# mdolab/dafoam

Hardware: AMD Instinct MI355X
Metric: adjoint_gmres_iterations_per_sec (higher is better)
Workload: dtype f64

## Files before the change

dafoam_amd/_capi.py:

```python
from __future__ import annotations

import ctypes as C
import os

import numpy as np

from .meshgen import BC_MIXED, FoamCase

_HERE = os.path.dirname(os.path.abspath(__file__))
LIB_PATH = os.environ.get("DAFOAM_AMD_LIB") or os.path.join(_HERE, "lib", "libdafoam_amd.so")

SOLVER_IDS = {"DASimpleFoam": 0, "DAScalarTransportFoam": 1, "DARhoSimpleFoam": 2, "DATurboFoam": 3, "DAHeatTransferFoam": 4}
PATCH_TYPES = {"patch": 0, "wall": 1, "symmetry": 2, "cyclic": 3}

c_double_p = C.POINTER(C.c_double)
c_int_p = C.POINTER(C.c_int)
c_ll_p = C.POINTER(C.c_longlong)


class das_case_t(C.Structure):
    _fields_ = [
        ("solver", C.c_int),
        ("n_points", C.c_int),
        ("n_faces", C.c_int),
# ... 231 lines not shown
    "das_set_coloring": (C.c_int, [_VP, c_int_p]),
    "das_debug_factor_block": (C.c_int, [C.c_int, c_ll_p, c_int_p, c_double_p, C.c_int, c_double_p, c_ll_p, c_int_p, c_int_p]),
    "das_debug_rcb": (C.c_int, [C.c_int, c_double_p, C.c_int, C.c_int, c_int_p]),
    "das_get_n_colors": (C.c_int, [_VP, C.c_int]),
    "das_get_con_nnz": (C.c_longlong, [_VP, C.c_int]),
    "das_get_con": (C.c_int, [_VP, C.c_int, c_ll_p, c_int_p]),
    "das_get_colors": (C.c_int, [_VP, C.c_int, c_int_p]),
    "das_calc_drdwt": (C.c_int, [_VP, C.c_int, C.c_int, C.POINTER(_VP)]),
    "das_mat_rows": (C.c_longlong, [_VP]),
    "das_mat_nnz": (C.c_longlong, [_VP]),
    "das_mat_export": (C.c_int, [_VP, c_ll_p, c_int_p, c_double_p]),
    "das_mat_mult": (C.c_int, [_VP, c_double_p, c_double_p]),
    "das_mat_create_from_csr": (C.c_int, [C.c_longlong, c_ll_p, c_int_p, c_double_p, C.POINTER(_VP)]),
    "das_mat_destroy": (None, [_VP]),
    "das_initialize_drdwt_matrix_free": (C.c_int, [_VP]),
    "das_destroy_drdwt_matrix_free": (C.c_int, [_VP]),
    "das_op_nnz": (C.c_longlong, [_VP]),
    "das_op_format_bytes": (C.c_longlong, [_VP]),
    "das_op_export": (C.c_int, [_VP, c_ll_p, c_int_p, c_double_p]),
    "das_calc_drdwold_t_psi": (C.c_int, [_VP, C.c_int, c_double_p, c_double_p]),
    "das_set_old_time_fields": (C.c_int, [_VP, c_double_p, c_double_p]),
    "das_calc_jac_vec_product": (C.c_int, [_VP, c_double_p, c_double_p]),
    "das_set_patch_value": (C.c_int, [_VP, c_int_p, C.c_int, C.c_char_p, c_double_p]),
    "das_get_patch_value": (C.c_int, [_VP, C.c_int, C.c_char_p, c_double_p]),
    "das_set_field": (C.c_int, [_VP, C.c_char_p, c_double_p]),
    "das_get_field": (C.c_int, [_VP, C.c_char_p, c_double_p]),
    "das_calc_dfield_product": (C.c_int, [_VP, C.c_char_p, C.c_char_p, C.c_char_p, c_double_p, c_double_p]),
    "das_calc_dvolcoord_product": (C.c_int, [_VP, C.c_char_p, C.c_char_p, c_double_p, c_double_p, c_double_p]),
    "das_point_influence_build": (C.c_int, [_VP, C.POINTER(C.c_int), C.POINTER(C.c_longlong)]),
    "das_point_influence_get": (C.c_int, [_VP, c_int_p, c_ll_p, c_int_p, c_double_p]),
    "das_debug_device_geometry": (C.c_int, [_VP, c_double_p, c_double_p, c_double_p]),
    "das_debug_strength_aggregates": (C.c_int, [_VP, C.c_int, c_int_p, C.POINTER(C.c_int)]),
    "das_calc_dbc_product": (C.c_int, [_VP, c_int_p, C.c_int, C.c_char_p, c_double_p, C.c_char_p, C.c_char_p, c_double_p, c_double_p]),
    "das_define_force_function": (C.c_int, [_VP, C.c_char_p, c_int_p, C.c_int, c_double_p, C.c_double]),
    "das_define_face_function": (C.c_int, [_VP, C.c_char_p, C.c_char_p, c_int_p, c_int_p, C.c_int, c_double_p, c_double_p, C.c_double, C.c_double]),
    "das_define_face_function_ex": (C.c_int, [_VP, C.c_char_p, C.c_char_p, c_int_p, c_int_p, C.c_int, c_double_p, c_double_p, C.c_double, C.c_double, C.c_int, C.c_double]),
    "das_define_location_function": (C.c_int, [_VP, C.c_char_p, C.c_char_p, c_int_p, C.c_int, c_double_p, c_double_p, C.c_double, C.c_int, C.c_double]),
    "das_define_patch_field_function": (C.c_int, [_VP, C.c_char_p, C.c_char_p, c_int_p, C.c_int, C.c_char_p, c_int_p, C.c_int, c_double_p, C.c_int, C.c_double, C.c_double]),
    "das_define_cell_function": (C.c_int, [_VP, C.c_char_p, C.c_char_p, c_int_p, C.c_int, C.c_char_p, c_int_p, C.c_int, c_double_p, C.c_int, C.c_double, C.c_double]),
    "das_calc_function": (C.c_int, [_VP, C.c_char_p, c_double_p]),
    "das_define_force_coupling": (C.c_int, [_VP, C.c_char_p, c_int_p, C.c_int, C.c_double]),
    "das_calc_force_coupling": (C.c_int, [_VP, C.c_char_p, c_double_p, C.c_int]),
    "das_define_thermal_coupling": (C.c_int, [_VP, C.c_char_p, c_int_p, C.c_int, C.c_int]),
    "das_calc_thermal_coupling": (C.c_int, [_VP, C.c_char_p, c_double_p, C.c_int]),
    "das_define_thermal_coupling_input": (C.c_int, [_VP, C.c_char_p, c_int_p, C.c_int, C.c_int]),
    "das_set_thermal_coupling_input": (C.c_int, [_VP, C.c_char_p, c_double_p, C.c_int]),
    "das_get_patch_mixed": (C.c_int, [_VP, C.c_int, c_double_p, c_double_p]),
    "das_calc_dthermal_coupling_product": (C.c_int, [_VP, C.c_char_p, C.c_char_p, C.c_char_p, c_double_p, c_double_p, C.c_int]),
    "das_define_heat_source": (C.c_int, [_VP, C.c_char_p, C.c_char_p, c_double_p, C.c_double, C.c_int]),
    "das_set_heat_source_pars": (C.c_int, [_VP, C.c_char_p, c_int_p, C.c_int, c_double_p]),
    "das_get_heat_source_info": (C.c_int, [_VP, C.c_char_p, c_double_p, c_double_p, c_double_p, c_int_p]),
    "das_get_heat_source_cells": (C.c_int, [_VP, C.c_char_p, c_int_p, C.c_int]),
    "das_get_fv_source": (C.c_int, [_VP, c_double_p]),
    "das_calc_dfvsourcepar_product": (C.c_int, [_VP, C.c_char_p, c_int_p, C.c_int, C.c_char_p, C.c_char_p, c_double_p, c_double_p]),
    "das_define_actuator_disk": (C.c_int, [_VP, C.c_char_p, C.c_char_p, c_double_p, C.c_char_p, C.c_double, C.c_int]),
    "das_set_actuator_disk_pars": (C.c_int, [_VP, C.c_char_p, c_int_p, C.c_int, c_double_p]),
    "das_get_actuator_disk_info": (C.c_int, [_VP, C.c_char_p, c_double_p, c_double_p, c_int_p]),
    "das_get_actuator_disk_cells": (C.c_int, [_VP, C.c_char_p, c_int_p, C.c_int]),
    "das_get_fv_source_vector": (C.c_int, [_VP, c_double_p]),
    "das_calc_dactuatordiskpar_product": (C.c_int, [_VP, C.c_char_p, c_int_p, C.c_int, C.c_char_p, C.c_char_p, c_double_p, c_double_p]),
    "das_get_input_size": (C.c_int, [_VP, C.c_char_p, C.c_char_p]),
    "das_get_output_size": (C.c_int, [_VP, C.c_char_p, C.c_char_p]),
    "das_calc_jac_t_vec_product": (
        C.c_int,
        [_VP, C.c_char_p, C.c_char_p, c_double_p, C.c_char_p, C.c_char_p, c_double_p, c_double_p],
    ),
    "das_drdwt_mult_device": (C.c_int, [_VP, _VP, _VP]),
    "das_create_ml_rksp_matrix_free": (C.c_int, [_VP, _VP, C.POINTER(_VP)]),
    "das_solve_linear_eqn": (C.c_int, [_VP, _VP, c_double_p, c_double_p]),
    "das_solve_linear_eqn_block": (C.c_int, [_VP, _VP, C.c_int, c_double_p, c_double_p, c_double_p, c_double_p]),
    "das_ksp_apply_pc": (C.c_int, [_VP, _VP, c_double_p, c_double_p]),
    "das_ksp_get_n_blocks": (C.c_int, [_VP]),
    "das_ksp_get_factor_nnz": (C.c_longlong, [_VP]),
    "das_ksp_get_n_ext": (C.c_longlong, [_VP]),
    "das_ksp_get_blocks": (C.c_int, [_VP, c_int_p, c_ll_p]),
    "das_pc_structure_build": (C.c_int, [_VP, c_int_p, c_ll_p, c_int_p, c_int_p]),
    "das_pc_structure_get": (C.c_int, [_VP, c_int_p, c_ll_p, c_int_p, c_int_p, c_int_p]),
    "das_ksp_get_pc_structure_sizes": (C.c_int, [_VP, c_int_p, c_ll_p, c_int_p]),
    "das_ksp_get_pc_structure": (C.c_int, [_VP, c_int_p, c_ll_p, c_int_p, c_int_p, c_int_p]),
    "das_ksp_get_info": (C.c_int, [_VP, c_int_p, c_double_p, c_double_p, c_double_p]),
    "das_ksp_get_history": (C.c_int, [_VP, c_double_p, C.c_int]),
    "das_ksp_get_cycle_lengths": (C.c_int, [_VP, c_int_p, C.c_int]),
    "das_ksp_get_basis_info": (C.c_int, [_VP, c_int_p, c_double_p, c_double_p]),
    "das_ksp_get_n_refine": (C.c_int, [_VP]),
    "das_set_dense_eig_callback": (C.c_int, [_VP]),
    "das_debug_gmres_dr_host": (C.c_int, [C.c_longlong, _VP, _VP, _VP, c_double_p, c_double_p, C.c_int, C.c_int, C.c_double, C.c_double, C.c_longlong, c_double_p, C.c_int,
                                          c_double_p, c_double_p]),
    "das_ksp_get_idr_info": (C.c_int, [_VP, c_int_p, c_int_p, c_int_p, c_int_p, c_int_p, c_double_p]),
    "das_ksp_get_poly_info": (C.c_int, [_VP, c_int_p, c_int_p, C.POINTER(C.c_longlong), C.POINTER(C.c_longlong), C.POINTER(C.c_longlong), c_int_p, c_int_p, c_int_p, c_double_p,
                                        c_int_p, c_double_p, c_double_p]),
    "das_debug_poly_roots": (C.c_int, [C.c_int, c_double_p, c_double_p, c_double_p]),
    "das_debug_poly_apply_host": (C.c_int, [C.c_longlong, _VP, _VP, _VP, C.c_int, c_double_p, c_double_p, c_double_p, c_double_p]),
    "das_debug_poly_step": (C.c_int, [C.c_longlong, C.c_int, C.c_int, C.c_int, C.c_double, C.c_double, C.c_longlong, C.c_longlong, c_double_p, c_double_p, c_double_p,
                                      c_double_p, c_double_p]),
    "das_debug_ksp_poly_apply": (C.c_int, [_VP, _VP, c_double_p, c_double_p]),
    "das_debug_idrs_host": (C.c_int, [C.c_longlong, _VP, _VP, _VP, c_double_p, c_double_p, C.c_int, C.c_int, C.c_double, C.c_double, C.c_longlong, c_double_p, C.c_int,
                                      c_double_p, c_double_p]),
    "das_debug_idr_cycle_host": (C.c_int, [C.c_longlong, _VP, _VP, _VP, c_double_p, c_double_p, C.c_int, C.c_int, c_double_p, c_double_p, c_double_p, c_double_p]),
    "das_debug_idr_shadow": (C.c_int, [C.c_longlong, C.c_int, C.c_longlong, C.c_int, C.c_int, c_double_p]),
    "das_debug_idr_combine": (C.c_int, [C.c_longlong, C.c_int, C.c_double, c_double_p, c_double_p, C.c_longlong, C.c_longlong, c_double_p, C.c_longlong, c_double_p,
                                        C.c_longlong]),
    "das_debug_idr_biortho_step": (C.c_int, [C.c_longlong, C.c_int, c_double_p, c_double_p, C.c_longlong, C.c_longlong, c_double_p, c_double_p, c_double_p, C.c_longlong,
                                             c_double_p]),
    "das_debug_idr_smooth_step": (C.c_int, [C.c_longlong, C.c_int, C.c_double, c_double_p, c_double_p, c_double_p, c_double_p, C.c_longlong, c_double_p, C.c_longlong,
                                            C.c_longlong, c_double_p]),
    "das_debug_gmres_dr_restart": (C.c_int, [C.c_int, C.c_int, c_double_p, c_double_p, c_double_p, c_double_p, c_double_p]),
    "das_debug_block_chol": (C.c_int, [C.c_int, c_double_p, c_double_p, c_double_p]),
    "das_debug_block_lsq": (C.c_int, [C.c_int, C.c_int, C.c_int, c_double_p, c_double_p, c_double_p, c_double_p, c_double_p, c_double_p]),
    "das_ksp_get_status": (C.c_int, [_VP, c_int_p, c_int_p, c_int_p, c_int_p]),
    "das_ksp_get_pc_stability": (C.c_int, [_VP, C.POINTER(C.c_double), c_int_p]),
    "das_ksp_get_pc_subdomains": (C.c_int, [_VP, c_int_p, c_double_p]),
    "das_ksp_get_pc_node_out": (C.c_int, [_VP, c_int_p]),
    "das_mesh_metrics": (C.c_int, [C.c_int, c_double_p, C.c_int, C.c_int, C.c_int, c_int_p, c_int_p, c_int_p, c_int_p, c_double_p, c_double_p, c_double_p, c_double_p, c_double_p]),
    "das_ksp_get_coarse": (C.c_int, [_VP, c_int_p]),
    "das_ksp_coarse_sparse_az_active": (C.c_int, [_VP]),
    "das_ksp_set_global_coarse": (C.c_int, [_VP, _VP, C.c_int, C.c_int, c_int_p]),
    "das_ksp_run_fixed_device": (C.c_int, [_VP, _VP, _VP, _VP, C.c_int]),
    "das_ksp_begin_device": (C.c_int, [_VP, _VP, _VP, _VP, C.c_int]),
    "das_ksp_advance": (C.c_int, [_VP, _VP, C.c_int]),
    "das_ksp_end": (C.c_int, [_VP, _VP]),
    "das_ksp_destroy": (None, [_VP]),
    "das_set_owned_mask": (C.c_int, [_VP, C.POINTER(C.c_ubyte)]),
    "das_comm_load_rccl": (C.c_int, []),
    "das_comm_unique_id": (C.c_int, [C.c_char_p]),
    "das_comm_init_rccl": (C.c_int, [_VP, C.c_int, C.c_int, C.c_char_p]),
    "das_comm_set_halo": (C.c_int, [_VP, C.c_int, c_int_p, c_ll_p, c_int_p, c_ll_p, c_int_p, C.c_longlong, c_int_p]),
    "das_set_exchange_cb": (C.c_int, [_VP, _VP, _VP]),
    "das_set_pc_overlap": (C.c_int, [_VP, C.POINTER(C.c_ubyte), C.c_int, c_ll_p, c_int_p, c_ll_p, c_int_p]),
    "das_set_gather_cb": (C.c_int, [_VP, _VP, _VP]),
    "das_comm_is_native": (C.c_int, [_VP]),
    "das_comm_reset": (C.c_int, [_VP]),
    "das_set_comm": (C.c_int, [_VP, _VP, _VP, _VP]),
    "das_set_stream": (C.c_int, [_VP, _VP]),
    "das_get_elapsed_clock_time": (C.c_double, [_VP]),
    "das_get_elapsed_cpu_time": (C.c_double, [_VP]),
    "das_timer_avg_ms": (C.c_double, [_VP, C.c_char_p]),
    "das_debug_orth_bench": (C.c_int, [C.c_longlong, C.c_int, C.c_int, C.c_int, C.c_int, C.c_int, C.POINTER(C.c_double), C.POINTER(C.c_double)]),
    "das_debug_orth_bench_split": (C.c_int, [C.c_longlong, C.c_int, C.c_int, C.c_int, C.c_int, C.c_int, C.c_int, C.c_int, C.POINTER(C.c_double), C.POINTER(C.c_double)]),
    "das_debug_set_orth_wide": (C.c_int, [C.c_int, C.POINTER(C.c_int)]),
    "das_debug_krylov_wide_eligible": (C.c_int, [C.c_longlong, C.c_int, C.c_longlong, C.POINTER(C.c_int), C.POINTER(C.c_int)]),
    "das_debug_krylov_dots2": (C.c_int, [C.c_longlong, C.c_int, C.c_int, _VP, C.c_longlong, c_double_p, c_double_p]),
    "das_debug_krylov_dcgs2_update": (C.c_int, [C.c_longlong, C.c_int, C.c_int, _VP, C.c_longlong, C.c_int, c_double_p, C.c_double, C.c_double, c_double_p]),
    "das_debug_krylov_multidot": (C.c_int, [C.c_longlong, C.c_int, C.c_int, _VP, C.c_longlong, c_double_p, c_double_p]),
    "das_debug_krylov_multiaxpy": (C.c_int, [C.c_longlong, C.c_int, C.c_int, _VP, C.c_longlong, c_double_p, C.c_int, _VP, C.c_longlong]),
    "das_debug_krylov_lincomb": (C.c_int, [C.c_longlong, C.c_int, C.c_int, _VP, C.c_longlong, c_double_p, c_double_p, C.c_longlong]),
    "das_debug_krylov_scale_to": (C.c_int, [C.c_longlong, C.c_double, C.c_int, _VP, _VP, C.c_longlong]),
    "das_debug_krylov_block_tn": (C.c_int, [C.c_longlong, C.c_int, C.c_int, c_double_p, C.c_longlong, C.c_longlong, c_double_p, C.c_longlong, c_double_p]),
    "das_debug_krylov_block_nn_sub": (C.c_int, [C.c_longlong, C.c_int, C.c_int, c_double_p, C.c_longlong, c_double_p, c_double_p, C.c_longlong]),
    "das_debug_krylov_block_right_mult": (C.c_int, [C.c_longlong, C.c_int, c_double_p, C.c_longlong, c_double_p]),
    "das_debug_krylov_block_lincomb": (C.c_int, [C.c_longlong, C.c_int, C.c_int, c_double_p, C.c_longlong, c_double_p, c_double_p, C.c_longlong]),
    "das_debug_krylov_block_spmm": (C.c_int, [C.c_longlong, C.c_int, c_ll_p, c_int_p, c_double_p, c_double_p, C.c_longlong, c_double_p, C.c_longlong]),
    "das_debug_bilu_factor": (C.c_int, [C.POINTER(das_bilu_debug_t), c_ll_p, c_ll_p, c_int_p, c_int_p, _VP, _VP, c_double_p, c_int_p]),
    "das_debug_bilu_apply": (C.c_int, [C.POINTER(das_bilu_debug_t), C.c_int, C.c_longlong, c_double_p, c_double_p, C.c_int, c_double_p, c_double_p, c_int_p, c_int_p]),
    "das_debug_graph_scan": (C.c_int, [C.c_longlong, c_int_p, c_ll_p, c_ll_p]),
    "das_debug_graph_transpose": (C.c_int, [C.c_longlong, c_ll_p, c_int_p, c_ll_p, c_int_p]),
    "das_debug_graph_nets": (C.c_int, [C.c_longlong, c_ll_p, c_int_p, C.c_longlong, c_ll_p, c_ll_p, c_int_p, c_int_p, C.POINTER(C.c_ubyte), c_ll_p]),
    "das_debug_graph_rows_gather": (C.c_int, [C.c_longlong, c_ll_p, C.c_longlong, c_ll_p, c_int_p, c_ll_p, c_int_p, C.c_longlong]),
    "das_debug_compact": (C.c_int, [C.c_longlong, c_ll_p, c_int_p, c_double_p, C.c_double, C.c_int, C.POINTER(C.c_ubyte), c_ll_p, c_int_p, c_double_p, c_ll_p]),
    "das_debug_vecpack": (C.c_int, [C.c_longlong, c_ll_p, c_int_p, c_double_p, C.c_longlong, C.c_longlong, c_int_p, c_ll_p, C.POINTER(C.c_ubyte), C.c_longlong, c_ll_p,
                                    c_double_p, c_double_p, C.c_longlong]),
    "das_debug_spmv_rows": (C.c_int, [C.c_longlong, c_int_p, C.c_longlong, c_ll_p, c_int_p, c_double_p, c_double_p, c_double_p, C.c_longlong]),
    "das_debug_coarse_assemble": (C.c_int, [C.c_int, C.c_longlong, C.c_longlong, C.c_longlong, c_ll_p, c_int_p, c_double_p, c_int_p, c_int_p, C.c_int, C.c_double,
                                            c_double_p]),
    "das_debug_coarse_invert": (C.c_int, [C.c_int, c_double_p, c_double_p, c_int_p]),
    "das_debug_coarse_correct": (C.c_int, [C.c_int, C.c_longlong, C.c_longlong, C.c_longlong, c_int_p, c_double_p, c_double_p, c_double_p, c_double_p, c_double_p,
                                           C.c_longlong, C.c_int]),
    "das_debug_coarse_az": (C.c_int, [C.c_int, C.c_longlong, c_ll_p, c_int_p, c_double_p, C.c_longlong, C.c_longlong, c_int_p, c_int_p, c_ll_p, c_int_p, c_double_p,
                                      C.c_longlong, c_ll_p, c_int_p, c_double_p, c_double_p, c_double_p, C.c_longlong]),
    "das_timer_count": (C.c_longlong, [_VP, C.c_char_p]),
    "das_timer_reset": (None, [_VP]),
    "das_timer_enable": (None, [_VP, C.c_int]),
}

_lib = None


def declared_symbols():
    return sorted(_SIGS)


def lib():
    global _lib
    if _lib is None:
        if not os.path.exists(LIB_PATH):
            raise ImportError(
                f"{LIB_PATH} not found: build the HIP extension first (python -c 'import __graft_entry__ as g; g.build()'). "
                "dafoam_amd has no CPU fallback."
            )
        L = C.CDLL(LIB_PATH)
        for name, (res, args) in _SIGS.items():
            fn = getattr(L, name)
            fn.restype = res
            fn.argtypes = args
        _lib = L
        _install_dense_eig(L)
    return _lib


_DENSE_EIG_FN = C.CFUNCTYPE(C.c_int, C.c_int, c_double_p, c_double_p, c_double_p, c_double_p, c_double_p)
_dense_eig_keepalive = []


def _install_dense_eig(L):

    def eig(m, A, wr, wi, vr, vi):
        try:
            G = np.ctypeslib.as_array(A, shape=(m * m,)).reshape(m, m)
            w, v = np.linalg.eig(G)
            np.ctypeslib.as_array(wr, shape=(m,))[:] = w.real
            np.ctypeslib.as_array(wi, shape=(m,))[:] = w.imag
            np.ctypeslib.as_array(vr, shape=(m * m,))[:] = np.ascontiguousarray(v.T.real).ravel()
            np.ctypeslib.as_array(vi, shape=(m * m,))[:] = np.ascontiguousarray(v.T.imag).ravel()
            return 0
        except Exception:
            return 1

    cb = _DENSE_EIG_FN(eig)
    _dense_eig_keepalive.append(cb)
    L.das_set_dense_eig_callback(C.cast(cb, C.c_void_p))


class DASError(RuntimeError):
    pass


def check(rc):
    if rc < 0:
        raise DASError(f"dafoam_amd error {rc}: {lib().das_last_error().decode()}")
    return rc


def dptr(a: np.ndarray):
    assert a.dtype == np.float64 and a.flags["C_CONTIGUOUS"]
    return a.ctypes.data_as(c_double_p)
```

dafoam_amd/csrc/das_bilu.hpp:

```cpp
#pragma once
#include <algorithm>
#include <cstdlib>
#include <numeric>

#include <omp.h>

#include "das_common.hpp"
#include "das_jaccon.hpp"

namespace das {

constexpr int BILU_NB = 8;
constexpr int BILU_NB2 = 64;
constexpr unsigned long long BILU_SENTINEL = 0xFFF7A5A5FFF7A5A5ull;
#ifndef BILU_WG
#define BILU_WG 512
#endif
#ifndef BILU_OCC
#define BILU_OCC 4
#endif
#ifndef BILU_XCD_TICKETS
#define BILU_XCD_TICKETS 1
#endif
constexpr int BILU_CTRL_STRIDE = 32;
// ... 283 lines not shown

__global__ __launch_bounds__(256) void k_bilu_scatter(long long n, const long long* __restrict__ rp, const int* __restrict__ ci,
                                                      const double* __restrict__ v, const int* __restrict__ unkNode,
                                                      const unsigned char* __restrict__ unkSlot, const long long* __restrict__ bptr,
                                                      const int* __restrict__ bcol, const unsigned char* __restrict__ late, double* __restrict__ bval,
                                                      unsigned long long* dropped, int transpose, double diagScale, long long shiftExLo,
                                                      long long shiftExHi, long long shiftEnd) {
    const long long row = (long long)blockIdx.x * 16 + (threadIdx.x >> 4);
    const int l16 = threadIdx.x & 15;
    if (row >= n) return;
    const int I0 = unkNode[row];
    if (I0 < 0) return;
    const int r0 = unkSlot[row];
    for (long long k = rp[row] + l16; k < rp[row + 1]; k += 16) {
        const int j = ci[k];
        const int J0 = unkNode[j];
        if (J0 < 0) continue;
        const int I = transpose ? J0 : I0, J = transpose ? I0 : J0;
        const int r = transpose ? unkSlot[j] : r0, c = transpose ? r0 : unkSlot[j];
        long long lo = bptr[I], hi = bptr[I + 1] - 1, e = -1;
        while (lo <= hi) {
            const long long mid = (lo + hi) >> 1;
            const int cm = bcol[mid];
            if (cm == J) { e = mid; break; }
            if (cm < J) lo = mid + 1; else hi = mid - 1;
        }
        if (e < 0) { if (!(late[I] && late[J])) atomicAdd(dropped, 1ull); continue; }
        const bool shifted = row < shiftEnd && !(row >= shiftExLo && row < shiftExHi);
        bval[e * BILU_NB2 + r * 8 + c] = (j == row && shifted) ? v[k] * diagScale : v[k];
    }
}
__global__ void k_bilu_pad_diag(int nNodes, const int* __restrict__ nodeUnk, const long long* __restrict__ bdiag, double* __restrict__ bval) {
    const long long i = (long long)blockIdx.x * blockDim.x + threadIdx.x;
    if (i >= (long long)nNodes * BILU_NB) return;
    if (nodeUnk[i] < 0) { const int k = (int)(i & 7); bval[bdiag[i >> 3] * BILU_NB2 + k * 8 + k] = 1.0; }
}

__device__ __forceinline__ double bilu_inverse8(double a, int lane, int* nshift) {
    const int r = lane >> 3, c = lane & 7;
    double b = (r == c) ? 1.0 : 0.0;
    for (int k = 0; k < 8; k++) {
        int pr = k;
        double best = -1.0;
        for (int rr = k; rr < 8; rr++) {
            const double t = fabs(__shfl(a, rr * 8 + k, 64));
            if (t > best) { best = t; pr = rr; }
        }
        const int src = (r == k) ? pr * 8 + c : (r == pr ? k * 8 + c : lane);
        a = __shfl(a, src, 64);
        b = __shfl(b, src, 64);
        double pv = __shfl(a, k * 8 + k, 64);
        if (!(fabs(pv) > 1e-300)) {
            pv = (pv < 0.0 ? -1.0 : 1.0) * 1e-12;
            if (lane == k * 9) a = pv;
            if (lane == 0) (*nshift)++;
        }
        const double rk = __shfl(a, k * 8 + c, 64) / pv;
        const double rkb = __shfl(b, k * 8 + c, 64) / pv;
        const double f = __shfl(a, r * 8 + k, 64);
        if (r == k) { a = rk; b = rkb; }
        else { a -= f * rk; b -= f * rkb; }
    }
    return b;
}

__global__ __launch_bounds__(256) void k_bilu_factor(int node0, int node1, const long long* __restrict__ bptr, const long long* __restrict__ bdiag,
                                                     const int* __restrict__ bcol, double* bval, double* invD, int* nshift) {
    const int lane = threadIdx.x & 63;
    const int p = node0 + blockIdx.x * 4 + (threadIdx.x >> 6);
    if (p >= node1) return;
    const int r = lane >> 3, c = lane & 7;
    const long long rb = bptr[p], rd = bdiag[p], re = bptr[p + 1];
    for (long long e = rb; e < rd; e++) {
        const int J = bcol[e];
        const double a = bval[e * BILU_NB2 + lane];
        double Lv = 0.0;
#pragma unroll
        for (int k = 0; k < 8; k++) Lv += __shfl(a, r * 8 + k, 64) * invD[(long long)J * BILU_NB2 + k * 8 + c];
        bval[e * BILU_NB2 + lane] = Lv;
        double Lrow[8];
#pragma unroll
        for (int k = 0; k < 8; k++) Lrow[k] = __shfl(Lv, r * 8 + k, 64);
        const long long je = bptr[J + 1];
        long long from = e + 1;
        for (long long f = bdiag[J] + 1; f < je; f++) {
            const int M = bcol[f];
            long long lo = from, hi = re - 1, pos = -1;
            while (lo <= hi) {
                const long long mid = (lo + hi) >> 1;
                const int cm = bcol[mid];
                if (cm == M) { pos = mid; break; }
                if (cm < M) lo = mid + 1; else hi = mid - 1;
            }
            if (pos < 0) { from = lo; continue; }
            from = pos + 1;
            double s = 0.0;
#pragma unroll
            for (int k = 0; k < 8; k++) s += Lrow[k] * bval[f * BILU_NB2 + k * 8 + c];
            bval[pos * BILU_NB2 + lane] -= s;
        }
    }
    int ns = 0;
    const double inv = bilu_inverse8(bval[rd * BILU_NB2 + lane], lane, &ns);
    invD[(long long)p * BILU_NB2 + lane] = inv;
    if (lane == 0 && ns) atomicAdd(nshift, ns);
}

template <class VT>
__global__ __launch_bounds__(256) void k_bilu_pack(int nNodes, const long long* __restrict__ bptr, const long long* __restrict__ bdiag,
                                                   const int* __restrict__ bcol, const double* __restrict__ bval, const long long* __restrict__ Lptr,
                                                   const long long* __restrict__ Uptr, int* __restrict__ Lcol, int* __restrict__ Ucol,
                                                   VT* __restrict__ Lval, VT* __restrict__ Uval) {
    const int lane = threadIdx.x & 63;
    const long long p = (long long)blockIdx.x * 4 + (threadIdx.x >> 6);
    if (p >= nNodes) return;
    const int r = lane >> 3, k = lane & 7;
    for (int t = 0; t < 2; t++) {
        const long long s0 = t == 0 ? bptr[p] : bdiag[p] + 1;
        const long long s1 = t == 0 ? bdiag[p] : bptr[p + 1];
        const int nE = (int)(s1 - s0);
        const long long d0 = t == 0 ? Lptr[p] : Uptr[nNodes - 1 - p];
        int* dcol = t == 0 ? Lcol : Ucol;
        VT* dval = t == 0 ? Lval : Uval;
        for (int a = 0; a < nE; a++) {
            const int pass = a >> 3, g = a & 7;
            const int nb = min(8, nE - 8 * pass);
            dval[(d0 + 8 * pass) * BILU_NB2 + (((r >> 1) * nb + g) * 8 + k) * 2 + (r & 1)] = (VT)bval[(s0 + a) * BILU_NB2 + lane];
            if (lane == 0) dcol[d0 + a] = bcol[s0 + a];
        }
    }
}

struct NodeILU {
    bool ready = false;
    long long n = 0;
    int nNodes = 0, nPrimary = 0, nLevels = 0, nshift = 0, maxRow = 0;
    std::vector<unsigned char> h_late;
    long long nnzB = 0, nL = 0, nU = 0;
    bool fp32 = false;
    double windowLevels = 3.0;
    int launchGrid = 0, launchSleep = 0, launchPerXcd = 0;
    std::vector<int> h_nodeUnk, h_bcol, h_lvlPtr, h_natural;
    std::vector<long long> h_bptr;
    DevBuf<int> nodeUnk, nodeOut, Lcol, Ucol;
    std::vector<int> h_nodeOut;
    DevBuf<long long> Lptr, Uptr;
    DevBuf<double> Lval, Uval, invD, y, z;
    DevBuf<float> Lvalf, Uvalf;
    DevBuf<unsigned> ctrl;
    DevBuf<double> ym, zm;
    int mS = 0;
    BiluView view;
    double t_struct = 0, t_scatter = 0, t_factor = 0, t_pack = 0;
    long long factor_bytes() const { return (nL + nU) * BILU_NB2 * (fp32 ? 4 : 8) + (long long)nNodes * BILU_NB2 * 8; }
};

inline std::vector<int> bilu_rcm_cells(const Mesh& m, const std::vector<char>& cellOwned, const double* startDir = nullptr) {
    const int nC = m.nC;
    std::vector<int> order, deg(nC, 0), queue;
    std::vector<char> seen(nC, 0);
    order.reserve(nC);
    for (int c = 0; c < nC; c++) for (int q = m.cc_ptr[c]; q < m.cc_ptr[c + 1]; q++) deg[c] += cellOwned[m.cc[q]] ? 1 : 0;
    auto bfs = [&](int start, std::vector<int>& out, std::vector<char>& mark) {
        const size_t first = out.size();
        out.push_back(start);
        mark[start] = 1;
        std::vector<int> nb;
        for (size_t head = first; head < out.size(); head++) {
            const int c = out[head];
            nb.clear();
            for (int q = m.cc_ptr[c]; q < m.cc_ptr[c + 1]; q++) { const int d = m.cc[q]; if (cellOwned[d] && !mark[d]) { mark[d] = 1; nb.push_back(d); } }
            std::sort(nb.begin(), nb.end(), [&](int a, int b) { return deg[a] < deg[b] || (deg[a] == deg[b] && a < b); });
            out.insert(out.end(), nb.begin(), nb.end());
        }
    };
    std::vector<char> tmpMark(nC, 0);
    std::vector<int> tmp;
    for (int c0 = 0; c0 < nC; c0++) {
        if (!cellOwned[c0] || seen[c0]) continue;
        int start = c0;
        if (startDir) {
            tmp.clear();
            bfs(c0, tmp, tmpMark);
            double best = 1e300;
            for (int c : tmp) {
                tmpMark[c] = 0;
                const double key = m.cg[c].C[0] * startDir[0] + m.cg[c].C[1] * startDir[1] + m.cg[c].C[2] * startDir[2];
                if (key < best) { best = key; start = c; }
            }
        } else {
            for (int sweep = 0; sweep < 2; sweep++) {
                tmp.clear();
                bfs(start, tmp, tmpMark);
                start = tmp.back();
                for (int c : tmp) tmpMark[c] = 0;
            }
        }
        bfs(start, order, seen);
    }
    std::reverse(order.begin(), order.end());
    return order;
}

inline void bilu_build_structure(const Mesh& m, const std::vector<StateDef>& states, long long n, const std::vector<unsigned char>& owned,
                                 const std::vector<char>& cellOwned, int reach, NodeILU& P, std::vector<int>& unkNode,
                                 std::vector<unsigned char>& unkSlot, std::vector<long long>& bptr, std::vector<long long>& bdiag,
                                 std::vector<int>& bcol, int nthr, int order = 0, const double* dir = nullptr) {
    const int nC = m.nC;
    std::vector<std::vector<int>> ownedFaces;
    bool hasFace = false;
    for (const StateDef& sd : states) if (sd.kind == KIND_FACE) hasFace = true;
    std::vector<int> of_ptr(nC + 1, 0), of;
    if (hasFace) {
        for (int f = 0; f < m.nF; f++) of_ptr[m.owner[f] + 1]++;
        for (int c = 0; c < nC; c++) of_ptr[c + 1] += of_ptr[c];
        of.resize(m.nF);
        std::vector<int> fill(of_ptr.begin(), of_ptr.end() - 1);
        for (int f = 0; f < m.nF; f++) of[fill[m.owner[f]]++] = f;
    }
    std::vector<int> nodeUnk0;
    std::vector<int> nodeCell_ptr{0}, nodeCell;
    std::vector<int> cellNode_ptr(nC + 1, 0), cellNode;
    nodeUnk0.reserve((size_t)nC * 9);
    std::vector<long long> tmp;
    int fillSlots = BILU_NB;
    auto is_owned = [&](long long g) { return owned.empty() || owned[g]; };
    std::vector<int> cellOrder;
    if (order == 1 || order == 2) cellOrder = bilu_rcm_cells(m, cellOwned);
    else { cellOrder.reserve(nC); for (int c = 0; c < nC; c++) if (cellOwned[c]) cellOrder.push_back(c); }
    if (order == 2 || order == 3) std::reverse(cellOrder.begin(), cellOrder.end());
    if (order == 6 || order == 7) {
        const double xdir[3] = {1.0, 0.0, 0.0};
        cellOrder = bilu_rcm_cells(m, cellOwned, dir ? dir : xdir);
        if (order == 6) std::reverse(cellOrder.begin(), cellOrder.end());
    }
    if (order == 4 || order == 5) {
        const double d0 = dir ? dir[0] : 1.0, d1 = dir ? dir[1] : 0.0, d2 = dir ? dir[2] : 0.0, sgn = order == 4 ? 1.0 : -1.0;
        std::vector<double> key(nC);
        for (int c = 0; c < nC; c++) key[c] = sgn * (m.cg[c].C[0] * d0 + m.cg[c].C[1] * d1 + m.cg[c].C[2] * d2);
        std::sort(cellOrder.begin(), cellOrder.end(), [&](int a, int b) { return key[a] < key[b] || (key[a] == key[b] && a < b); });
    }
    std::vector<std::pair<int, int>> cellNodePairs;
    std::vector<int> lateUnk, lateCell;
    for (int c : cellOrder) {
        tmp.clear();
        for (const StateDef& sd : states) {
            if (sd.kind == KIND_VEC) { for (int k = 0; k < 3; k++) if (is_owned(sd.offset + 3LL * c + k)) tmp.push_back(sd.offset + 3LL * c + k); }
            else if (sd.kind == KIND_SCL) { if (is_owned(sd.offset + c)) tmp.push_back(sd.offset + c); }
        }
        for (const StateDef& sd : states)
            if (sd.kind == KIND_FACE) for (int q = of_ptr[c]; q < of_ptr[c + 1]; q++) if (is_owned(sd.offset + of[q])) tmp.push_back(sd.offset + of[q]);
        const size_t mc = tmp.size();
        if (mc == 0) continue;
        const size_t mp = std::min<size_t>(mc, BILU_NB);
        if ((size_t)(BILU_NB - fillSlots) < mp) fillSlots = BILU_NB;
        if (fillSlots == BILU_NB) {
            nodeUnk0.insert(nodeUnk0.end(), BILU_NB, -1);
            nodeCell_ptr.push_back(nodeCell_ptr.back());
            fillSlots = 0;
        }
        const int node = (int)nodeCell_ptr.size() - 2;
        nodeCell.push_back(c);
        nodeCell_ptr[node + 1]++;
        cellNodePairs.push_back({c, node});
        for (size_t k = 0; k < mp; k++) nodeUnk0[(size_t)node * BILU_NB + fillSlots++] = (int)tmp[k];
        for (size_t k = mp; k < mc; k++) { lateUnk.push_back((int)tmp[k]); lateCell.push_back(c); }
    }
    const int nPrimary = (int)nodeCell_ptr.size() - 1;
    for (size_t k = 0; k < lateUnk.size();) {
        const int c = lateCell[k];
        nodeUnk0.insert(nodeUnk0.end(), BILU_NB, -1);
        nodeCell_ptr.push_back(nodeCell_ptr.back());
        const int node = (int)nodeCell_ptr.size() - 2;
        nodeCell.push_back(c);
        nodeCell_ptr[node + 1]++;
        cellNodePairs.push_back({c, node});
        for (int slot = 0; slot < BILU_NB && k < lateUnk.size() && lateCell[k] == c; slot++, k++) nodeUnk0[(size_t)node * BILU_NB + slot] = lateUnk[k];
    }
    const int nN = (int)nodeCell_ptr.size() - 1;
    DAS_CHECK(nN > 0, DAS_ERR_INTERNAL, "preconditioner: no owned unknowns");
    for (const auto& pr : cellNodePairs) cellNode_ptr[pr.first + 1]++;
    for (int c = 0; c < nC; c++) cellNode_ptr[c + 1] += cellNode_ptr[c];
    cellNode.resize(cellNodePairs.size());
    {
        std::vector<int> fill(cellNode_ptr.begin(), cellNode_ptr.end() - 1);
        for (const auto& pr : cellNodePairs) cellNode[fill[pr.first]++] = pr.second;
    }
    std::vector<long long> rptr(nN + 1, 0);
    std::vector<std::vector<int>> rows(nN);
#pragma omp parallel num_threads(nthr)
    {
        std::vector<int> cmark(nC, -1), nmark(nN, -1), cur, nxt;
#pragma omp for schedule(dynamic, 256)
        for (int I = 0; I < nN; I++) {
            std::vector<int>& row = rows[I];
            cur.clear();
            for (int q = nodeCell_ptr[I]; q < nodeCell_ptr[I + 1]; q++) { const int c = nodeCell[q]; cmark[c] = I; cur.push_back(c); }
            const bool lateI = I >= nPrimary;
            auto add_cell = [&](int c) {
                for (int q = cellNode_ptr[c]; q < cellNode_ptr[c + 1]; q++) {
                    const int J = cellNode[q];
                    if (lateI && J >= nPrimary && J != I) continue;
                    if (nmark[J] != I) { nmark[J] = I; row.push_back(J); }
                }
            };
            for (int c : cur) add_cell(c);
            for (int ring = 0; ring < reach; ring++) {
                nxt.clear();
                for (int c : cur)
                    for (int q = m.cc_ptr[c]; q < m.cc_ptr[c + 1]; q++) {
                        const int d = m.cc[q];
                        if (cmark[d] != I) { cmark[d] = I; nxt.push_back(d); if (cellOwned[d]) add_cell(d); }
                    }
                cur.swap(nxt);
            }
            std::sort(row.begin(), row.end());
        }
    }
    std::vector<int> level(nN, 0);
    int nLv = 0;
    for (int I = 0; I < nN; I++) {
        int l = 0;
        for (int J : rows[I]) { if (J >= I) break; l = std::max(l, level[J] + 1); }
        level[I] = l;
        nLv = std::max(nLv, l + 1);
    }
    std::vector<int> lvlPtr(nLv + 1, 0), pos(nN);
    for (int I = 0; I < nN; I++) lvlPtr[level[I] + 1]++;
    for (int l = 0; l < nLv; l++) lvlPtr[l + 1] += lvlPtr[l];
    {
        std::vector<int> fill(lvlPtr.begin(), lvlPtr.end() - 1);
        for (int I = 0; I < nN; I++) pos[I] = fill[level[I]]++;
    }
    std::vector<int> inv(nN);
    for (int I = 0; I < nN; I++) inv[pos[I]] = I;
    bptr.assign(nN + 1, 0);
    for (int p = 0; p < nN; p++) bptr[p + 1] = bptr[p] + (long long)rows[inv[p]].size();
    bcol.resize((size_t)bptr[nN]);
    bdiag.assign(nN, -1);
    int maxRow = 0;
#pragma omp parallel for schedule(static) reduction(max : maxRow) num_threads(nthr)
    for (int p = 0; p < nN; p++) {
        const std::vector<int>& row = rows[inv[p]];
        int* dst = bcol.data() + bptr[p];
        for (size_t k = 0; k < row.size(); k++) dst[k] = pos[row[k]];
        std::sort(dst, dst + row.size());
        bdiag[p] = bptr[p] + (std::lower_bound(dst, dst + row.size(), p) - dst);
        maxRow = std::max(maxRow, (int)row.size());
    }
    P.h_nodeUnk.assign((size_t)nN * BILU_NB, -1);
    unkNode.assign(n, -1);
    unkSlot.assign(n, 0);
    for (int p = 0; p < nN; p++)
        for (int k = 0; k < BILU_NB; k++) {
            const int gidx = nodeUnk0[(size_t)inv[p] * BILU_NB + k];
            P.h_nodeUnk[(size_t)p * BILU_NB + k] = gidx;
            if (gidx >= 0) { unkNode[gidx] = p; unkSlot[gidx] = (unsigned char)k; }
        }
    P.n = n; P.nNodes = nN; P.nLevels = nLv; P.nnzB = bptr[nN]; P.maxRow = maxRow; P.nPrimary = nPrimary;
    P.h_late.assign(nN, 0);
    for (int p = 0; p < nN; p++) P.h_late[p] = inv[p] >= nPrimary ? 1 : 0;
    P.h_bptr = bptr; P.h_bcol = bcol; P.h_lvlPtr = lvlPtr; P.h_natural = inv;
}

struct NodeILU;
inline void bilu_launch_shape(NodeILU& P, hipStream_t st);

struct BiluStructRef {
    const std::vector<long long>* bptr;
    const std::vector<long long>* bdiag;
    const std::vector<int>* bcol;
    std::vector<const std::vector<int>*> unkNode;
    std::vector<const std::vector<unsigned char>*> unkSlot;
};
inline void bilu_numeric(long long n, const BiluStructRef& S, bool fp32, long long An, const long long* d_rp, const int* d_ci, const double* d_av, hipStream_t st, NodeILU& P,
                         bool debug, bool transpose, double diagScale, long long shiftExLo, long long shiftExHi, long long shiftEnd, double t0);

inline std::vector<char> cells_of_mask(const Mesh& m, const std::vector<StateDef>& states, const std::vector<unsigned char>& mask) {
    std::vector<char> in(m.nC, 1);
    if (mask.empty()) return in;
    const StateDef& s0 = states[0];
    const int stride = s0.kind == KIND_VEC ? 3 : 1;
    for (int c = 0; c < m.nC; c++) in[c] = mask[s0.offset + (long long)stride * c] ? 1 : 0;
    return in;
}

inline void bilu_setup(const Mesh& m, const std::vector<StateDef>& states, long long n, const std::vector<unsigned char>& owned, int reach,
                       bool fp32, long long An, const long long* d_rp, const int* d_ci, const double* d_av, hipStream_t st, NodeILU& P,
                       bool debug, int nthr, int order, bool transpose = false, double diagScale = 1.0, long long shiftExLo = 0,
                       long long shiftExHi = 0, long long shiftEnd = (long long)1 << 62, const double* dir = nullptr) {
    const double t0 = wall_seconds();
    const std::vector<char> cellOwned = cells_of_mask(m, states, owned);
    std::vector<int> unkNode, bcol;
    std::vector<unsigned char> unkSlot;
    std::vector<long long> bptr, bdiag;
    bilu_build_structure(m, states, n, owned, cellOwned, reach, P, unkNode, unkSlot, bptr, bdiag, bcol, std::max(1, nthr), order, dir);
    BiluStructRef S{&bptr, &bdiag, &bcol, {&unkNode}, {&unkSlot}};
    bilu_numeric(n, S, fp32, An, d_rp, d_ci, d_av, st, P, debug, transpose, diagScale, shiftExLo, shiftExHi, shiftEnd, t0);
}

inline void bilu_numeric(long long n, const BiluStructRef& S, bool fp32, long long An, const long long* d_rp, const int* d_ci, const double* d_av, hipStream_t st, NodeILU& P,
                         bool debug, bool transpose, double diagScale, long long shiftExLo, long long shiftExHi, long long shiftEnd, double t0) {
    const int nN = P.nNodes;
    P.fp32 = fp32;
    P.nodeUnk.upload(P.h_nodeUnk);
    DevBuf<int> d_unkNode, d_bcol;
    DevBuf<unsigned char> d_unkSlot;
    DevBuf<long long> d_bptr, d_bdiag;
    const std::vector<int>& bcol = *S.bcol;
    const std::vector<long long>&bptr = *S.bptr, &bdiag = *S.bdiag;
    DevBuf<unsigned char> d_late;
    d_late.upload(P.h_late);
    d_bptr.upload(bptr); d_bdiag.upload(bdiag); d_bcol.upload(bcol);
    DevBuf<double> bval((size_t)P.nnzB * BILU_NB2);
    DevBuf<unsigned long long> d_dropped(1);
    DevBuf<int> d_nshift(1);
    DAS_HIP(hipMemsetAsync(bval.p, 0, bval.n * sizeof(double), st));
    DAS_HIP(hipMemsetAsync(d_dropped.p, 0, sizeof(unsigned long long), st));
    DAS_HIP(hipMemsetAsync(d_nshift.p, 0, sizeof(int), st));
    P.t_struct = wall_seconds() - t0;
    double t1 = wall_seconds();
    for (size_t q = 0; q < S.unkNode.size(); q++) {
        d_unkNode.upload(*S.unkNode[q]); d_unkSlot.upload(*S.unkSlot[q]);
        hipLaunchKernelGGL(k_bilu_scatter, dim3((unsigned)((An + 15) / 16)), dim3(256), 0, st, An, d_rp, d_ci, d_av, d_unkNode.p, d_unkSlot.p, d_bptr.p,
                           d_bcol.p, d_late.p, bval.p, d_dropped.p, transpose ? 1 : 0, diagScale, shiftExLo, shiftExHi, shiftEnd);
        DAS_HIP(hipStreamSynchronize(st));
    }
    hipLaunchKernelGGL(k_bilu_pad_diag, dim3((unsigned)(((long long)nN * BILU_NB + 255) / 256)), dim3(256), 0, st, nN, P.nodeUnk.p, d_bdiag.p, bval.p);
    DAS_HIP(hipGetLastError());
    unsigned long long dropped = 0;
    DAS_HIP(hipMemcpyAsync(&dropped, d_dropped.p, sizeof(dropped), hipMemcpyDeviceToHost, st));
    DAS_HIP(hipStreamSynchronize(st));
    DAS_CHECK(dropped == 0, DAS_ERR_INTERNAL, "preconditioner: " + std::to_string(dropped) + " matrix entries fall outside the node pattern (stencil reach too small)");
    P.t_scatter = wall_seconds() - t1;
    t1 = wall_seconds();
    P.invD.alloc((size_t)nN * BILU_NB2);
    for (int l = 0; l < P.nLevels; l++) {
        const int a = P.h_lvlPtr[l], bnd = P.h_lvlPtr[l + 1];
        if (bnd > a)
            hipLaunchKernelGGL(k_bilu_factor, dim3((unsigned)((bnd - a + 3) / 4)), dim3(256), 0, st, a, bnd, d_bptr.p, d_bdiag.p, d_bcol.p, bval.p, P.invD.p,
                               d_nshift.p);
    }
    DAS_HIP(hipGetLastError());
    DAS_HIP(hipMemcpyAsync(&P.nshift, d_nshift.p, sizeof(int), hipMemcpyDeviceToHost, st));
    DAS_HIP(hipStreamSynchronize(st));
    P.t_factor = wall_seconds() - t1;
    t1 = wall_seconds();
    std::vector<long long> Lptr(nN + 1, 0), Uptr(nN + 1, 0);
    for (int p = 0; p < nN; p++) Lptr[p + 1] = Lptr[p] + (bdiag[p] - bptr[p]);
    for (int q = 0; q < nN; q++) { const int p = nN - 1 - q; Uptr[q + 1] = Uptr[q] + (bptr[p + 1] - bdiag[p] - 1); }
    P.nL = Lptr[nN]; P.nU = Uptr[nN];
    P.Lptr.upload(Lptr); P.Uptr.upload(Uptr);
    P.Lcol.alloc(std::max<long long>(P.nL, 1)); P.Ucol.alloc(std::max<long long>(P.nU, 1));
    if (fp32) {
        P.Lvalf.alloc((size_t)std::max<long long>(P.nL, 1) * BILU_NB2); P.Uvalf.alloc((size_t)std::max<long long>(P.nU, 1) * BILU_NB2);
        P.Lval.release(); P.Uval.release();
        hipLaunchKernelGGL(k_bilu_pack<float>, dim3((unsigned)((nN + 3) / 4)), dim3(256), 0, st, nN, d_bptr.p, d_bdiag.p, d_bcol.p, bval.p, P.Lptr.p,
                           P.Uptr.p, P.Lcol.p, P.Ucol.p, P.Lvalf.p, P.Uvalf.p);
    } else {
        P.Lval.alloc((size_t)std::max<long long>(P.nL, 1) * BILU_NB2); P.Uval.alloc((size_t)std::max<long long>(P.nU, 1) * BILU_NB2);
        P.Lvalf.release(); P.Uvalf.release();
        hipLaunchKernelGGL(k_bilu_pack<double>, dim3((unsigned)((nN + 3) / 4)), dim3(256), 0, st, nN, d_bptr.p, d_bdiag.p, d_bcol.p, bval.p, P.Lptr.p,
                           P.Uptr.p, P.Lcol.p, P.Ucol.p, P.Lval.p, P.Uval.p);
    }
    DAS_HIP(hipGetLastError());
    P.y.alloc((size_t)nN * BILU_NB); P.z.alloc((size_t)nN * BILU_NB);
    P.ctrl.alloc(BILU_CTRL_SIZE);
    DAS_HIP(hipMemsetAsync(P.ctrl.p, 0, BILU_CTRL_SIZE * sizeof(unsigned), st));
    DAS_HIP(hipStreamSynchronize(st));
    P.t_pack = wall_seconds() - t1;
    P.view.nNodes = nN; P.view.nodeUnk = P.nodeUnk.p;
    if (!P.h_nodeOut.empty()) P.nodeOut.upload(P.h_nodeOut);
    P.view.nodeOut = P.h_nodeOut.empty() ? P.nodeUnk.p : P.nodeOut.p;
    P.view.ptr[0] = P.Lptr.p; P.view.ptr[1] = P.Uptr.p; P.view.col[0] = P.Lcol.p; P.view.col[1] = P.Ucol.p;
    P.view.val[0] = P.Lval.p; P.view.val[1] = P.Uval.p; P.view.valf[0] = P.Lvalf.p; P.view.valf[1] = P.Uvalf.p;
    P.view.invD = P.invD.p; P.view.y = P.y.p; P.view.z = P.z.p; P.view.ctrl = P.ctrl.p;
    bilu_launch_shape(P, st);
    P.ready = true;
    if (debug)
        fprintf(stderr, "[dafoam_amd] node-block ILU(0): %d nodes (%.3f slots/unknown), %lld blocks (%.1f per node, max %d), %d levels, %d shifted pivots, "
                        "factor %.2f GB%s; structure %.2f s, scatter %.3f s, factorise %.3f s, pack %.3f s\n", nN, (double)nN * BILU_NB / (double)n, P.nnzB,
                (double)P.nnzB / nN, P.maxRow, P.nLevels, P.nshift, P.factor_bytes() / 1e9, fp32 ? " (fp32)" : "", P.t_struct, P.t_scatter, P.t_factor,
                P.t_pack);
}

inline void bilu_setup_multi(const Mesh& m, const std::vector<StateDef>& states, long long n, const std::vector<const std::vector<unsigned char>*>& masks,
                             const std::vector<int>& orders, const std::vector<unsigned char>& subOf, int reach, bool fp32, long long An, const long long* d_rp,
                             const int* d_ci, const double* d_av, hipStream_t st, NodeILU& P, bool debug, int nthr, const double* dir) {
    const double t0 = wall_seconds();
    const int K = (int)masks.size();
    struct Blk { NodeILU S; std::vector<int> unkNode, bcol, newPos; std::vector<unsigned char> unkSlot; std::vector<long long> bptr, bdiag; };
    std::vector<Blk> B(K);
    int nLv = 0;
    long long nN = 0, nnzB = 0;
    for (int b = 0; b < K; b++) {
        const std::vector<unsigned char>& mask = *masks[b];
        const std::vector<char> cellOwned = cells_of_mask(m, states, mask);
        bilu_build_structure(m, states, n, mask, cellOwned, reach, B[b].S, B[b].unkNode, B[b].unkSlot, B[b].bptr, B[b].bdiag, B[b].bcol, std::max(1, nthr), orders[b], dir);
        nLv = std::max(nLv, B[b].S.nLevels);
        nN += B[b].S.nNodes;
        nnzB += B[b].S.nnzB;
    }
    DAS_CHECK(nN < (1LL << 31) && nnzB < (1LL << 40), DAS_ERR_INTERNAL, "multi-block preconditioner too large");
    std::vector<int> lvlPtr(nLv + 1, 0);
    for (int b = 0; b < K; b++) for (int l = 0; l < B[b].S.nLevels; l++) lvlPtr[l + 1] += B[b].S.h_lvlPtr[l + 1] - B[b].S.h_lvlPtr[l];
    for (int l = 0; l < nLv; l++) lvlPtr[l + 1] += lvlPtr[l];
    {
        std::vector<int> cursor(lvlPtr.begin(), lvlPtr.end() - 1);
        for (int b = 0; b < K; b++) {
            B[b].newPos.resize(B[b].S.nNodes);
            for (int l = 0; l < B[b].S.nLevels; l++) for (int p = B[b].S.h_lvlPtr[l]; p < B[b].S.h_lvlPtr[l + 1]; p++) B[b].newPos[p] = cursor[l]++;
        }
    }
    std::vector<long long> bptr(nN + 1, 0), bdiag(nN, -1);
    for (int b = 0; b < K; b++) for (int p = 0; p < B[b].S.nNodes; p++) bptr[B[b].newPos[p] + 1] = B[b].bptr[p + 1] - B[b].bptr[p];
    for (long long p = 0; p < nN; p++) bptr[p + 1] += bptr[p];
    std::vector<int> bcol((size_t)bptr[nN]);
    P = NodeILU();
    P.h_nodeUnk.assign((size_t)nN * BILU_NB, -1);
    P.h_nodeOut.assign((size_t)nN * BILU_NB, -1);
    P.h_late.assign(nN, 0);
    P.h_natural.assign(nN, 0);
    int maxRow = 0, nPrimary = 0;
    long long natOff = 0;
    for (int b = 0; b < K; b++) {
        Blk& Q = B[b];
#pragma omp parallel for schedule(static) num_threads(std::max(1, nthr))
        for (int p = 0; p < Q.S.nNodes; p++) {
            const long long np = Q.newPos[p];
            int* dst = bcol.data() + bptr[np];
            const long long r0 = Q.bptr[p], len = Q.bptr[p + 1] - r0;
            for (long long q = 0; q < len; q++) dst[q] = Q.newPos[Q.bcol[r0 + q]];
            bdiag[np] = bptr[np] + (Q.bdiag[p] - r0);
            for (int k = 0; k < BILU_NB; k++) {
                const int gi = Q.S.h_nodeUnk[(size_t)p * BILU_NB + k];
                P.h_nodeUnk[(size_t)np * BILU_NB + k] = gi;
                P.h_nodeOut[(size_t)np * BILU_NB + k] = (gi >= 0 && subOf[gi] == (unsigned char)b) ? gi : -1;
            }
            P.h_late[np] = Q.S.h_late[p];
            P.h_natural[np] = (int)(natOff + Q.S.h_natural[p]);
        }
        for (long long g = 0; g < n; g++) if (Q.unkNode[g] >= 0) Q.unkNode[g] = Q.newPos[Q.unkNode[g]];
        maxRow = std::max(maxRow, Q.S.maxRow);
        nPrimary += Q.S.nPrimary;
        natOff += Q.S.nNodes;
        Q.S = NodeILU();
        std::vector<int>().swap(Q.bcol);
        std::vector<long long>().swap(Q.bptr);
        std::vector<long long>().swap(Q.bdiag);
    }
    P.n = n; P.nNodes = (int)nN; P.nLevels = nLv; P.nnzB = bptr[nN]; P.maxRow = maxRow; P.nPrimary = nPrimary;
    P.h_bptr = bptr; P.h_bcol = bcol; P.h_lvlPtr = lvlPtr;
    BiluStructRef S{&bptr, &bdiag, &bcol, {}, {}};
    for (int b = 0; b < K; b++) { S.unkNode.push_back(&B[b].unkNode); S.unkSlot.push_back(&B[b].unkSlot); }
    bilu_numeric(n, S, fp32, An, d_rp, d_ci, d_av, st, P, debug, false, 1.0, 0, 0, (long long)1 << 62, t0);
}

__global__ void k_bilu_xcd_probe(unsigned* mask) {
    if (threadIdx.x == 0) atomicOr(mask, 1u << (__builtin_amdgcn_s_getreg((3 << 11) | 20) & 15u));
}
inline int bilu_xcd_probe(hipStream_t st) {
    static int cached = -1;
    if (cached >= 0) return cached;
    DevBuf<unsigned> mask(1);
    DAS_HIP(hipMemsetAsync(mask.p, 0, sizeof(unsigned), st));
    hipLaunchKernelGGL(k_bilu_xcd_probe, dim3(256), dim3(64), 0, st, mask.p);
    unsigned h = 0u;
    DAS_HIP(hipMemcpyAsync(&h, mask.p, sizeof(h), hipMemcpyDeviceToHost, st));
    DAS_HIP(hipStreamSynchronize(st));
    cached = (h == 0xFFu) ? 8 : 0;
    return cached;
}

inline void bilu_launch_shape(NodeILU& P, hipStream_t st) {
    int dev = 0, cus = 256;
    if (hipGetDevice(&dev) == hipSuccess) (void)hipDeviceGetAttribute(&cus, hipDeviceAttributeMultiprocessorCount, dev);
    const int waves = BILU_WG / 64;
    const double perLevel = (double)P.nNodes / std::max(1, P.nLevels);
    int grid = (int)std::min<double>(cus * 2.0 * (BILU_OCC * 4 / waves), std::max(8.0, P.windowLevels * perLevel / waves));
    int sleepReps = 0;
    if (const char* e = getenv("DAS_BILU_WGS")) grid = std::max(1, atoi(e));
    if (const char* e = getenv("DAS_BILU_SLEEP")) sleepReps = std::max(0, atoi(e));
    const long long tickets = ((long long)P.nNodes + waves - 1) / waves;
    grid = (int)std::min<long long>(grid, tickets + 1);
    int perXcd = (BILU_XCD_TICKETS && grid >= 64 && bilu_xcd_probe(st) == 8) ? 1 : 0;
    if (const char* e = getenv("DAS_BILU_XCD")) perXcd = (atoi(e) != 0 && grid >= 64 && bilu_xcd_probe(st) == 8) ? 1 : 0;
    P.launchGrid = grid; P.launchSleep = sleepReps; P.launchPerXcd = perXcd;
}

inline void bilu_apply(NodeILU& P, const double* b, double* out, hipStream_t st) {
    const long long nslots = (long long)P.nNodes * BILU_NB;
    hipLaunchKernelGGL(k_bilu_reset, dim3((unsigned)((nslots + 255) / 256)), dim3(256), 0, st, nslots, P.y.p, P.z.p, P.ctrl.p);
    const int grid = P.launchGrid, sl = P.launchSleep, px = P.launchPerXcd;
    if (P.fp32) {
        hipLaunchKernelGGL((k_bilu_sweep<float, false>), dim3(grid), dim3(BILU_WG), 0, st, P.view, b, out, sl, px);
        hipLaunchKernelGGL((k_bilu_sweep<float, true>), dim3(grid), dim3(BILU_WG), 0, st, P.view, b, out, sl, px);
    } else {
        hipLaunchKernelGGL((k_bilu_sweep<double, false>), dim3(grid), dim3(BILU_WG), 0, st, P.view, b, out, sl, px);
        hipLaunchKernelGGL((k_bilu_sweep<double, true>), dim3(grid), dim3(BILU_WG), 0, st, P.view, b, out, sl, px);
    }
}

template <int S>
inline void bilu_apply_multi_s(NodeILU& P, const double* b, double* out, long long ld, hipStream_t st) {
    const long long nslots = (long long)P.nNodes * BILU_NB * S;
    if (P.mS < S || P.ym.n < (size_t)nslots) { P.ym.alloc((size_t)P.nNodes * BILU_NB * 4); P.zm.alloc((size_t)P.nNodes * BILU_NB * 4); P.mS = 4; }
    hipLaunchKernelGGL(k_bilu_reset, dim3((unsigned)((nslots + 255) / 256)), dim3(256), 0, st, nslots, P.ym.p, P.zm.p, P.ctrl.p);
    const int grid = P.launchGrid, sl = P.launchSleep, px = P.launchPerXcd;
    if (P.fp32) {
        hipLaunchKernelGGL((k_bilu_sweep_m<float, false, S>), dim3(grid), dim3(BILU_WG), 0, st, P.view, P.ym.p, P.zm.p, b, out, ld, sl, px);
        hipLaunchKernelGGL((k_bilu_sweep_m<float, true, S>), dim3(grid), dim3(BILU_WG), 0, st, P.view, P.ym.p, P.zm.p, b, out, ld, sl, px);
    } else {
        hipLaunchKernelGGL((k_bilu_sweep_m<double, false, S>), dim3(grid), dim3(BILU_WG), 0, st, P.view, P.ym.p, P.zm.p, b, out, ld, sl, px);
        hipLaunchKernelGGL((k_bilu_sweep_m<double, true, S>), dim3(grid), dim3(BILU_WG), 0, st, P.view, P.ym.p, P.zm.p, b, out, ld, sl, px);
    }
}
inline void bilu_apply_multi(NodeILU& P, const double* b, double* out, long long ld, int nrhs, hipStream_t st) {
    int r = 0;
    for (; r + 4 <= nrhs; r += 4) bilu_apply_multi_s<4>(P, b + (long long)r * ld, out + (long long)r * ld, ld, st);
    for (; r + 2 <= nrhs; r += 2) bilu_apply_multi_s<2>(P, b + (long long)r * ld, out + (long long)r * ld, ld, st);
    for (; r < nrhs; r++) bilu_apply(P, b + (long long)r * ld, out + (long long)r * ld, st);
}

inline bool bilu_aborted(NodeILU& P, hipStream_t st) {
    unsigned c = 0u;
    DAS_HIP(hipMemcpyAsync(&c, P.ctrl.p + BILU_CTRL_ABORT, sizeof(c), hipMemcpyDeviceToHost, st));
    DAS_HIP(hipStreamSynchronize(st));
    return c != 0u;
}

inline void bilu_clear_abort(NodeILU& P, hipStream_t st) { DAS_HIP(hipMemsetAsync(P.ctrl.p + BILU_CTRL_ABORT, 0, sizeof(unsigned), st)); }

}
```

dafoam_amd/csrc/das_bilu_debug.hpp:

```cpp
#pragma once
#include "das_bilu.hpp"

namespace das {

static void bilu_debug_validate(const std::string& who, const das_bilu_debug_t& d) {
    const int nN = d.nNodes;
    auto bad = [&](bool cond, const char* what) { DAS_CHECK(!cond, DAS_ERR_ARG, who + ": " + what); };
    bad(d.bptr[0] != 0, "bptr[0] must be 0");
    for (int p = 0; p < nN; p++) bad(d.bptr[p + 1] < d.bptr[p], "bptr decreases");
    bad(d.bptr[nN] >= (1LL << 40), "too many blocks");
    bad(d.lvlPtr[0] != 0 || d.lvlPtr[d.nLevels] != nN, "lvlPtr must cover [0, nNodes]");
    for (int l = 0; l < d.nLevels; l++) bad(d.lvlPtr[l + 1] < d.lvlPtr[l], "lvlPtr decreases");
    std::vector<int> level(nN);
    for (int l = 0; l < d.nLevels; l++) for (int p = d.lvlPtr[l]; p < d.lvlPtr[l + 1]; p++) level[p] = l;
    for (int p = 0; p < nN; p++) {
        const long long rb = d.bptr[p], re = d.bptr[p + 1], rd = d.bdiag[p];
        bad(rd < rb || rd >= re, "bdiag outside its row");
        for (long long e = rb; e < re; e++) {
            const int J = d.bcol[e];
            bad(J < 0 || J >= nN, "block column out of range");
            bad(e > rb && d.bcol[e - 1] >= J, "block columns of a row must ascend");
        }
        bad(d.bcol[rd] != p, "bdiag does not point at the diagonal block");
    }
    for (int p = 0; p < nN; p++)
        for (long long e = d.bptr[p]; e < d.bptr[p + 1]; e++) {
            const int J = d.bcol[e];
            if (J == p) continue;
            const int* jb = d.bcol + d.bptr[J];
            const int* je = d.bcol + d.bptr[J + 1];
            bad(!std::binary_search(jb, je, p), "the node pattern is not symmetric");
            bad(J < p && level[J] >= level[p], "a dependency does not lie in an earlier level");
        }
    for (long long i = 0; i < (long long)nN * BILU_NB; i++) {
        bad(d.nodeUnk[i] < -1 || d.nodeUnk[i] >= d.n, "nodeUnk out of range");
        if (d.nodeOut) bad(d.nodeOut[i] < -1 || d.nodeOut[i] >= d.n, "nodeOut out of range");
    }
    for (long long i = 0; i < (long long)d.nMaps * d.An; i++) {
        bad(d.unkNode[i] < -1 || d.unkNode[i] >= nN, "unkNode out of range");
        bad(d.unkSlot[i] >= BILU_NB, "unkSlot must be below 8");
    }
    bad(d.rp[0] != 0, "rowptr[0] must be 0");
    for (long long i = 0; i < d.An; i++) bad(d.rp[i + 1] < d.rp[i], "rowptr decreases");
    const long long nnz = d.rp[d.An];
    bad(nnz > 0 && !(d.ci && d.val), "null pointer");
    for (long long k = 0; k < nnz; k++) bad(d.ci[k] < 0 || d.ci[k] >= d.An, "CSR column out of range");
}

static void bilu_debug_check(const std::string& who, const das_bilu_debug_t* d) {
    DAS_CHECK(d, DAS_ERR_ARG, who + ": null pointer");
    DAS_CHECK(d->nNodes > 0 && d->nLevels > 0 && d->nMaps > 0 && d->n > 0 && d->An > 0, DAS_ERR_ARG, who + ": sizes must be positive");
    DAS_CHECK(d->nNodes < (1 << 27) && d->An <= d->n && d->n < (1LL << 31), DAS_ERR_ARG, who + ": sizes out of range (An <= n < 2^31)");
    DAS_CHECK(d->nodeUnk && d->late && d->bptr && d->bdiag && d->bcol && d->lvlPtr && d->unkNode && d->unkSlot && d->rp, DAS_ERR_ARG, who + ": null pointer");
    DAS_CHECK((d->fp32 == 0 || d->fp32 == 1) && (d->transpose == 0 || d->transpose == 1), DAS_ERR_ARG, who + ": fp32 and transpose are 0 or 1");
    bilu_debug_validate(who, *d);
}

static void bilu_debug_setup(const das_bilu_debug_t& d, NodeILU& P) {
    const int nN = d.nNodes;
    const std::vector<long long> bptr(d.bptr, d.bptr + nN + 1), bdiag(d.bdiag, d.bdiag + nN);
    const std::vector<int> bcol(d.bcol, d.bcol + bptr[nN]);
    std::vector<std::vector<int>> unkNode(d.nMaps);
    std::vector<std::vector<unsigned char>> unkSlot(d.nMaps);
    BiluStructRef S{&bptr, &bdiag, &bcol, {}, {}};
    for (int q = 0; q < d.nMaps; q++) {
        unkNode[q].assign(d.unkNode + q * d.An, d.unkNode + (q + 1) * d.An);
        unkSlot[q].assign(d.unkSlot + q * d.An, d.unkSlot + (q + 1) * d.An);
    }
    for (int q = 0; q < d.nMaps; q++) { S.unkNode.push_back(&unkNode[q]); S.unkSlot.push_back(&unkSlot[q]); }
    P.n = d.n; P.nNodes = nN; P.nLevels = d.nLevels; P.nnzB = bptr[nN]; P.nPrimary = nN;
    for (int p = 0; p < nN; p++) P.maxRow = std::max(P.maxRow, (int)(bptr[p + 1] - bptr[p]));
    P.h_nodeUnk.assign(d.nodeUnk, d.nodeUnk + (size_t)nN * BILU_NB);
    if (d.nodeOut) P.h_nodeOut.assign(d.nodeOut, d.nodeOut + (size_t)nN * BILU_NB);
    P.h_late.assign(d.late, d.late + nN);
    P.h_lvlPtr.assign(d.lvlPtr, d.lvlPtr + d.nLevels + 1);
    P.h_bptr = bptr; P.h_bcol = bcol;
    const size_t nnz = (size_t)d.rp[d.An];
    DevBuf<long long> d_rp(d.An + 1);
    DevBuf<int> d_ci(std::max<size_t>(nnz, 1));
    DevBuf<double> d_av(std::max<size_t>(nnz, 1));
    d_rp.upload(d.rp, (size_t)d.An + 1); d_ci.upload(d.ci, nnz); d_av.upload(d.val, nnz);
    bilu_numeric(d.n, S, d.fp32 != 0, d.An, d_rp.p, d_ci.p, d_av.p, 0, P, false, d.transpose != 0, d.diagScale, d.shiftExLo, d.shiftExHi, d.shiftEnd, wall_seconds());
}

static void debug_bilu_factor(const das_bilu_debug_t& d, long long* Lptr, long long* Uptr, int* Lcol, int* Ucol, void* Lval, void* Uval, double* invD, int* nshift) {
    NodeILU P;
    bilu_debug_setup(d, P);
    const size_t nN = (size_t)d.nNodes;
    P.Lptr.download(Lptr, nN + 1); P.Uptr.download(Uptr, nN + 1);
    P.Lcol.download(Lcol, (size_t)P.nL); P.Ucol.download(Ucol, (size_t)P.nU);
    if (d.fp32) { P.Lvalf.download((float*)Lval, (size_t)P.nL * BILU_NB2); P.Uvalf.download((float*)Uval, (size_t)P.nU * BILU_NB2); }
    else { P.Lval.download((double*)Lval, (size_t)P.nL * BILU_NB2); P.Uval.download((double*)Uval, (size_t)P.nU * BILU_NB2); }
    P.invD.download(invD, nN * BILU_NB2);
    *nshift = P.nshift;
}

static int bilu_debug_last_group(int nrhs) { return (nrhs & 1) ? 1 : ((nrhs & 3) == 2 ? 2 : 4); }

static void debug_bilu_apply(const das_bilu_debug_t& d, int nrhs, long long ld, const double* b, double* out, int twice, double* y, double* z, int* abortFlag,
                             int* info) {
    NodeILU P;
    bilu_debug_setup(d, P);
    const size_t len = (size_t)nrhs * ld;
    DevBuf<double> db(len), dout(len);
    db.upload(b, len);
    for (int rep = 0; rep < (twice ? 2 : 1); rep++) {
        dout.upload(out, len);
        if (nrhs == 1) bilu_apply(P, db.p, dout.p, 0);
        else bilu_apply_multi(P, db.p, dout.p, ld, nrhs, 0);
        DAS_HIP(hipGetLastError());
        DAS_HIP(hipStreamSynchronize(0));
    }
    dout.download(out, len);
    const int S = bilu_debug_last_group(nrhs);
    const size_t nw = (size_t)d.nNodes * BILU_NB * S;
    (S == 1 ? P.y : P.ym).download(y, nw);
    (S == 1 ? P.z : P.zm).download(z, nw);
    *abortFlag = bilu_aborted(P, 0) ? 1 : 0;
    info[0] = P.launchGrid; info[1] = P.launchSleep; info[2] = P.launchPerXcd; info[3] = bilu_xcd_probe(0);
}

}
```

dafoam_amd/csrc/das_device.hip:

```cpp
#include <algorithm>
#include <cmath>
#include <ctime>
#include <functional>
#include <numeric>
#include <thread>

#include "das_case.hpp"
#include "das_jaccon.hpp"
#include "das_bilu.hpp"
#include "das_rcb.hpp"
#include "das_comm.hpp"
#include "das_krylov.hpp"
#include "das_gmres_host.hpp"
#include "das_block.hpp"
#include "das_krylov_debug.hpp"
#include "das_idr.hpp"
#include "das_idr_debug.hpp"
#include "das_poly.hpp"
#include "das_poly_debug.hpp"
#include "das_bilu_debug.hpp"
#include "das_graph_debug.hpp"
#include "das_coarse.hpp"
#include "das_coarse_debug.hpp"
#include "das_color.hpp"
// ... 467 lines not shown
            sok[d] = ee < lvl[lq + 1];
            const int ec = ee < eend ? ee : eend - 1;
            sv[d].load(bv, ec);
            sr[d] = br[ec];
#ifndef PC_EXP_NOBARRIER
            __syncthreads();
#endif
        }
    }
}

template <bool USE_LDS>
__global__ __launch_bounds__(PC_THREADS) void k_ras_apply(PCView P, const double* __restrict__ b, double* __restrict__ out, int maxLev) {
    extern __shared__ double xs[];
    const int blk = blockIdx.x;
    const long long o0 = P.boff[blk];
    const int nloc = (int)(P.boff[blk + 1] - o0);
    int* lvl = (int*)xs;
    double* xlds = xs + ((maxLev + 2 * PC_PF + 4) >> 1);
    double* xw = USE_LDS ? xlds : P.xglob + o0;
    for (int i = threadIdx.x; i < nloc; i += PC_THREADS) xw[i] = b[P.gidx[o0 + i]];
    __syncthreads();
    if (P.factor32) ras_sweep<USE_LDS, float>(P.svalf[0], P.srowcol[0], P.slev[0], P.slevOff[0][blk], P.slevOff[0][blk + 1], xw, lvl);
    else ras_sweep<USE_LDS, double>(P.sval[0], P.srowcol[0], P.slev[0], P.slevOff[0][blk], P.slevOff[0][blk + 1], xw, lvl);
    for (int i = threadIdx.x; i < nloc; i += PC_THREADS) xw[i] *= P.invd[o0 + i];
    __syncthreads();
    if (P.factor32) ras_sweep<USE_LDS, float>(P.svalf[1], P.srowcol[1], P.slev[1], P.slevOff[1][blk], P.slevOff[1][blk + 1], xw, lvl);
    else ras_sweep<USE_LDS, double>(P.sval[1], P.srowcol[1], P.slev[1], P.slevOff[1][blk], P.slevOff[1][blk + 1], xw, lvl);
    for (int i = threadIdx.x; i < nloc; i += PC_THREADS) {
        int g = P.gout[o0 + i];
        if (g >= 0) out[g] = xw[i];
    }
}

struct Mat {
    long long n = 0, nnz = 0;
    DevBuf<long long> rowptr;
    DevBuf<int> col;
    DevBuf<double> val;
    VecPack vp;
};

struct KernelTimer {
    struct Rec { double ms = 0; long long cnt = 0; std::vector<std::pair<hipEvent_t, hipEvent_t>> pending; };
    std::map<std::string, Rec> recs;
    bool on = false;
    std::vector<hipEvent_t> pool;
    hipEvent_t get() {
        if (!pool.empty()) { hipEvent_t e = pool.back(); pool.pop_back(); return e; }
        hipEvent_t e;
        DAS_HIP(hipEventCreate(&e));
        return e;
    }
    void begin(const char* name, hipStream_t st, hipEvent_t& a) {
        if (!on) return;
        a = get();
        DAS_HIP(hipEventRecord(a, st));
    }
    void end(const char* name, hipStream_t st, hipEvent_t a) {
        if (!on) return;
        hipEvent_t b = get();
        DAS_HIP(hipEventRecord(b, st));
        recs[name].pending.push_back({a, b});
    }
    void resolve() {
        for (auto& kv : recs) {
            for (auto& pr : kv.second.pending) {
                DAS_HIP(hipEventSynchronize(pr.second));
                float ms = 0;
                DAS_HIP(hipEventElapsedTime(&ms, pr.first, pr.second));
                kv.second.ms += ms;
                kv.second.cnt++;
                pool.push_back(pr.first);
                pool.push_back(pr.second);
            }
            kv.second.pending.clear();
        }
    }
    void reset() { resolve(); for (auto& kv : recs) { kv.second.ms = 0; kv.second.cnt = 0; } }
};

struct ConDev {
    bool ready = false;
    bool onDevice = false;
    DevBuf<long long> t_rowptr;
    DevBuf<int> cl_cols;
    DevBuf<int> t_col;
};

struct BlockILU {
    long long n = 0, next = 0;
    int nBlocks = 0;
    long long fnnz = 0;
    int maxLocal = 0;
    DevBuf<long long> boff, slev[2], slevOff[2];
    DevBuf<int> gidx, gout;
    DevBuf<unsigned> srowcol[2];
    DevBuf<double> sval[2], invd, xw;
    DevBuf<float> svalf[2];
    bool factor32 = false;
    PCView view;
    int maxLevels = 0;
    bool useLDS = false;
    double setup_seconds = 0;
    std::vector<int> h_core_perm;
    std::vector<long long> h_core_off;
};

}

using namespace das;

struct das_mat {
    Mat m;
};

struct das_ksp {
    das_mat* pcmat = nullptr;
    BlockILU pc;
    NodeILU bilu;
    bool useBilu = false;
    bool pcTranspose = false;
    double pcDiagScale = 1.0;
    long long shiftExLo = 0, shiftExHi = 0, shiftEnd = (long long)1 << 62;
    struct CoarsePC {
        bool active = false, deflated = false;
        bool global = false;
        int nagg = 0;
        int naggG = 0, aggOff = 0;
        long long off = 0, N = 0;
        DevBuf<int> agg;
        DevBuf<int> aggRow;
        DevBuf<int> cells, cellsAll;
        DevBuf<long long> aptr, aptrAll;
        DevBuf<double> Einv, t, u, c, rr;
        std::vector<int> h_agg;
        DevBuf<long long> azPtr;
        DevBuf<int> azAgg;
        DevBuf<double> azVal;
        long long azOpId = -1;
        long long azEpoch = -1, azNnz = 0;
        bool azReady = false, azFailed = false;
    } coarse;
    int restart = 0;
    VmBuf<double> V;
    long long Vn = 0;
    bool vf32 = false;
    bool split = false;
    DevBuf<double> ustage;
    DevBuf<double> w, z, r, xdev, bdev, partial, hdev, rich_r, rich_d;
    int nSub = 1;
    std::vector<int> subOrder;
    std::vector<double> subEst;
    int pcOrder = -1;
    int pcOrderUsed = -1;
    double pcStability = -1.0;
    bool rasOverlap = false;
    DevBuf<double> pcin;
    std::unique_ptr<struct GmresRun> run;
    std::unique_ptr<struct BlockWork> block;
    int polyD = 0;
    std::unique_ptr<struct PolyWork> poly;
    std::unique_ptr<struct IdrWork> idr;
    std::vector<double> block_res0, block_res;
    int iters = 0, nrefine = 0, reason = 0, nBreakdown = 0;
    double res0 = 0, res = 0, seconds = 0;
    std::vector<double> hist;
    std::vector<int> cycleLens;
};

struct das_solver {
    Mesh mesh;
    CaseParams cp;
    Options opt;
    int device = -1;
    bool inited = false;
    long long n = 0;
    Stencil st_full, st_pc;
    JacCon con_full, con_pc;
    std::vector<int> colors;
    int nColors = 0;
    bool colored = false;
    DevBuf<FaceGeom> d_fg;
    DevBuf<CellGeom> d_cg;
    DevBuf<int> d_cf_ptr, d_cf_face, d_cf_other, d_owner, d_neigh, d_bpatch, d_cyc;
    DevBuf<PatchBC> d_bc;
    DevBuf<double> d_mixed;
    DevBuf<double> d_phiF, d_Told;
    DevMesh dm;
    DevBuf<double> d_W, d_R, d_R0, d_Wp, d_scale, d_tmp1, d_tmp2;
    DevBuf<int> d_colors;
    std::vector<double> h_W, h_scale;
    ResWork<double> wk;
    ResWork<Dual<1>> wk1;
    DevBuf<Dual<1>> d_Wd, d_Rd;
    ConDev cd[2];
    std::unique_ptr<das_mat> op;
    std::vector<double> op_states;
    long long op_geom = -1;
    struct FaceFn {
        int kind = DAS_FN_FORCE;
        bool ratio = false;
        double gammaFn = 1.4, RFn = 287.0;
        std::vector<int> faces;
        std::vector<unsigned char> group;
        std::vector<double> w0, dir;
        DevBuf<int> d_faces;
        DevBuf<unsigned char> d_group;
        DevBuf<double> d_w0, d_weff, d_dir, d_fv;
        bool uploaded = false;
        bool isMoment = false;
        double vecA[3] = {0, 0, 0}, vecB[3] = {0, 0, 0}, scale = 1.0;
        long long geomVersion = -1;
        bool refVar = false, geoWeight = false, hasData = true;
        double ref = 0.0;
        int ncomp = 1;
        bool byUnitArea = true, ks = false;
        double coeffKS = 1.0, loc[6] = {1, 0, 0, 0, 0, 0};
        DevBuf<double> d_ks, d_kpart;
        double pRef = 0.0;
        FaceFnView view(const double* w) const {
            return FaceFnView{d_faces.p, d_group.p, w, dir.empty() ? nullptr : d_dir.p, (int)faces.size(), kind, gammaFn, RFn,
                              {loc[0], loc[1], loc[2], loc[3], loc[4], loc[5]}, pRef};
        }
    };
    std::map<std::string, FaceFn> functions;
    struct ForceCoupling {
        std::vector<int> patches;
        int nOut = 0;
        std::vector<int> ptPtr, ptSlot;
        std::vector<int> fcPtr, fcPt;
        DevBuf<int> d_ptPtr, d_ptSlot, d_fcPtr, d_fcPt;
        DevBuf<double> d_ff, d_out, d_seeds;
        FaceFn fn;
        bool uploaded = false;
    };
    std::map<std::string, ForceCoupling> forceCouplings;
    struct ThermalCoupling {
        std::vector<int> patches;
        DevBuf<double> d_out, d_seeds;
        FaceFn fn;
        bool uploaded = false;
        std::vector<double> in;
    };
    std::map<std::string, ThermalCoupling> thermalCouplings, thermalInputs;
    struct CellFn {
        bool variance = false, square = false, multiplyVol = true, divByTotalVol = false, refVar = false, geoWeight = false, hasData = true;
        bool field = false;
        double scale = 1.0, ref = 0.0;
        double coef = 0.0, totalVol = 1.0;
        long long geomVersion = -1;
        std::vector<int> cell;
        std::vector<long long> idx;
        std::vector<double> data;
        DevBuf<int> d_cell;
        DevBuf<long long> d_idx;
        DevBuf<double> d_data, d_part, d_unit;
        bool uploaded = false;
        CellFnView view() const {
            return CellFnView{(long long)cell.size(), d_cell.p, d_idx.p, data.empty() ? nullptr : d_data.p, (int)square, (int)multiplyVol};
        }
    };
    std::map<std::string, CellFn> cellFunctions;
    struct HeatSource {
        int kind = DAS_HS_CYLINDERSMOOTH;
        double pars[9] = {0, 0, 0, 0, 0, 0, 0, 0, 0};
        double eps = 0.0;
        int snapCell = -1;
        std::vector<int> members;
        DevBuf<unsigned char> d_member;
        double volumeTotal = 0.0;
    };
    std::map<std::string, HeatSource> heatSources;
    DevBuf<double> d_src, d_hsVt;
    DevBuf<Dual<1>> d_hsPart, d_hsVtD;
    double hsSourceTotal = 0.0;
    struct ActuatorDisk {
        int smooth = 1, adjustThrust = 0;
        double pars[13] = {0, 0, 0, 0, 0, 0, 0, 0, 0, 0, 0, 0, 0};
        double eps = 0.0, rotSign = 1.0;
        std::vector<int> members;
        DevBuf<unsigned char> d_member;
        double scale = 0.0, thrustSum = 0.0, torqueSum = 0.0, unitThrust = 0.0;
    };
    std::map<std::string, ActuatorDisk> actuatorDisks;
    DevBuf<double> d_src3, d_adSums;
    DevBuf<Dual<1>> d_adPart, d_adD;
    DevBuf<int> d_adBad;
    int colorRounds = 0;
    DevBuf<double> d_betaFI, d_dBetaFI;
    long long geomVersion = 0;
    struct VolCoord {
        PointInfluence inf;
        bool built = false, uploaded = false;
        double relStep = 0.0;
        long long hGeom = -1;
        DevBuf<long long> d_ptr;
        DevBuf<int> d_cells, d_cpoints, d_face_ptr, d_face_pts, d_bad, d_fnPtr, d_fnIdx;
        DevBuf<double> d_h, d_X0, d_X, d_Rp, d_Rm, d_seeds, d_tc, d_out, d_fvp, d_fvm;
        DevBuf<FaceGeom> d_fg0;
        DevBuf<CellGeom> d_cg0;
        double buildSeconds = 0.0, seconds = 0.0;
    } vc;
    long long opEpoch = 0, op_epoch = -1;
    long long nGlobalCells = 0;
    hipStream_t stream = nullptr;
// ... 422 lines not shown
                lrp.assign(nl + 1, 0);
                lci.clear();
                lv.clear();
                for (int p = 0; p < nl; p++) {
                    int g = F.gidx[p];
                    row.clear();
                    for (long long q = rp[g]; q < rp[g + 1]; q++) {
                        int lc = loc[ci[q]];
                        if (lc >= 0) row.push_back({lc, av[q]});
                    }
                    std::sort(row.begin(), row.end());
                    for (auto& e : row) { lci.push_back(e.first); lv.push_back(e.second); }
                    lrp[p + 1] = (long long)lci.size();
                }
                for (int p = 0; p < nl; p++) loc[F.gidx[p]] = -1;
                factor_local(nl, lrp, lci, lv, lfill, F, where, lev, nullptr);
                F.nnzLU = (long long)F.fci.size();
                std::vector<long long>().swap(F.frp); std::vector<long long>().swap(F.fdiag); std::vector<int>().swap(F.fci);
                std::vector<double>().swap(F.fv); std::vector<int>().swap(F.Lrows); std::vector<int>().swap(F.Urows);
            } catch (const std::exception& e) {
#pragma omp critical
                err = e.what();
            }
        }
    }
    DAS_CHECK(err.empty(), DAS_ERR_INTERNAL, "block ILU setup failed: " + err);
    const double t_fact = wall_seconds();
    BlockILU& P = k->pc;
    std::vector<long long> boff(nB + 1, 0), eoff[2], loff[2], slev[2], slevOff[2];
    long long next = 0, fnnz = 0;
    int maxLocal = 0, maxLv = 0, nshift = 0;
    for (int t = 0; t < 2; t++) { eoff[t].assign(nB + 1, 0); loff[t].assign(nB + 1, 0); }
    P.h_core_off.assign(1, 0);
    for (int b = 0; b < nB; b++) {
        const BlockFactor& F = BF[b];
        const int nl = (int)F.gidx.size();
        boff[b + 1] = boff[b] + nl;
        maxLocal = std::max(maxLocal, nl);
        nshift += F.nshift;
        fnnz += F.nnzLU;
        long long ncore = 0;
        for (int g : F.gout) ncore += g >= 0 ? 1 : 0;
        P.h_core_off.push_back(P.h_core_off.back() + ncore);
        for (int t = 0; t < 2; t++) {
            eoff[t][b + 1] = eoff[t][b] + (long long)F.sval[t].size();
            loff[t][b + 1] = loff[t][b] + (long long)F.slev[t].size();
            maxLv = std::max<int>(maxLv, (int)F.slev[t].size() - 1);
        }
    }
    next = boff[nB];
    std::vector<int> gidx(next), gout(next);
    std::vector<double> invd(next);
    P.h_core_perm.assign(P.h_core_off.back(), 0);
    for (int t = 0; t < 2; t++) { slev[t].resize(loff[t][nB]); slevOff[t] = loff[t]; }
#pragma omp parallel for schedule(dynamic, 1) num_threads(das::host_threads())
    for (int b = 0; b < nB; b++) {
        BlockFactor& F = BF[b];
        std::copy(F.gidx.begin(), F.gidx.end(), gidx.begin() + boff[b]);
        std::copy(F.gout.begin(), F.gout.end(), gout.begin() + boff[b]);
        std::copy(F.invd.begin(), F.invd.end(), invd.begin() + boff[b]);
        long long pc = P.h_core_off[b];
        for (int g : F.gout) if (g >= 0) P.h_core_perm[pc++] = g;
        for (int t = 0; t < 2; t++)
            for (size_t q = 0; q < F.slev[t].size(); q++) slev[t][loff[t][b] + q] = eoff[t][b] + F.slev[t][q];
    }
    DAS_CHECK((long long)P.h_core_perm.size() == nOwnedStates, DAS_ERR_INTERNAL, "block cores do not cover all owned states exactly once");
    P.n = n; P.next = next; P.nBlocks = nB; P.fnnz = fnnz; P.maxLevels = maxLv; P.maxLocal = maxLocal;
    P.boff.upload(boff); P.gidx.upload(gidx); P.gout.upload(gout); P.invd.upload(invd);
    P.factor32 = s->opt.geti("amd.pcFactorFP32") != 0;
    for (int t = 0; t < 2; t++) {
        const size_t tot = (size_t)eoff[t][nB];
        if (P.factor32) { P.svalf[t].alloc(tot); P.sval[t].release(); }
        else { P.sval[t].alloc(tot); P.svalf[t].release(); }
        P.srowcol[t].alloc(tot);
        P.slev[t].upload(slev[t]); P.slevOff[t].upload(slevOff[t]);
    }
    {
        std::vector<float> f32;
        for (int b = 0; b < nB; b++) {
            BlockFactor& F = BF[b];
            for (int t = 0; t < 2; t++) {
                const size_t cnt = F.sval[t].size();
                if (!cnt) continue;
                if (P.factor32) {
                    f32.assign(F.sval[t].begin(), F.sval[t].end());
                    DAS_HIP(hipMemcpy(P.svalf[t].p + eoff[t][b], f32.data(), cnt * sizeof(float), hipMemcpyHostToDevice));
                } else {
                    DAS_HIP(hipMemcpy(P.sval[t].p + eoff[t][b], F.sval[t].data(), cnt * sizeof(double), hipMemcpyHostToDevice));
                }
                DAS_HIP(hipMemcpy(P.srowcol[t].p + eoff[t][b], F.src[t].data(), cnt * sizeof(unsigned), hipMemcpyHostToDevice));
            }
            F = BlockFactor();
        }
    }
    P.useLDS = (size_t)maxLocal * sizeof(double) + (size_t)(maxLv + 2 * PC_PF + 8) * sizeof(int) + 16 <= 160 * 1024;
    if (!P.useLDS) P.xw.alloc(next);
    else DAS_HIP(hipFuncSetAttribute((const void*)k_ras_apply<true>, hipFuncAttributeMaxDynamicSharedMemorySize, 160 * 1024));
    P.view.nBlocks = nB; P.view.boff = P.boff.p; P.view.gidx = P.gidx.p; P.view.gout = P.gout.p; P.view.invd = P.invd.p;
    P.view.factor32 = P.factor32 ? 1 : 0;
    for (int t = 0; t < 2; t++) { P.view.sval[t] = P.sval[t].p; P.view.svalf[t] = P.svalf[t].p; P.view.srowcol[t] = P.srowcol[t].p; P.view.slev[t] = P.slev[t].p; P.view.slevOff[t] = P.slevOff[t].p; }
    P.view.xglob = P.xw.p;
    P.setup_seconds = wall_seconds() - t0;
    if (s->opt.geti("debug"))
        fprintf(stderr, "[dafoam_amd] RAS(overlap %d)+ILU(%d): %d blocks, n_ext=%lld (%.2fx), nnz(LU)=%lld, max block %d unknowns (%s), max levels %d, "
                        "%d shifted pivots, %.2f s (download+partition %.2f, factorise %.2f, streams+upload %.2f)\n", overlap, lfill, nB, next,
                (double)next / n, fnnz, maxLocal, P.useLDS ? "LDS" : "global", maxLv, nshift, P.setup_seconds, t_prep - t0, t_fact - t_prep,
                wall_seconds() - t_fact);
}

static int pc_stencil_reach(das_solver* s) {
    ensure_coloring(s);
    int reach = 0;
    for (size_t b = 0; b < s->st_pc.states.size(); b++)
        for (size_t lv = 0; lv < s->st_pc.levels[b].size(); lv++) {
            const unsigned mask = s->st_pc.levels[b][lv];
            if (!mask) continue;
            bool faceState = false;
            for (size_t q = 0; q < s->st_pc.states.size(); q++) if ((mask >> q & 1u) && s->st_pc.states[q].kind == KIND_FACE) faceState = true;
            reach = std::max<int>(reach, (int)lv + (faceState ? 1 : 0) + (s->st_pc.states[b].kind == KIND_FACE ? 1 : 0));
        }
    return reach;
}

static bool pc_ordering_rcm(das_solver* s) {
    const std::string& o = s->opt.gets("adjEqnOption.jacMatReOrdering");
    DAS_CHECK(o == "natural" || o == "rcm", DAS_ERR_ARG, "adjEqnOption.jacMatReOrdering \"" + o + "\" is not implemented (natural | rcm)");
    return o == "rcm";
}

static void pc_flow_direction(das_solver* s, double* dir) {
    dir[0] = 1.0; dir[1] = 0.0; dir[2] = 0.0;
    if (!s->st_full.states.empty() && s->st_full.states[0].kind == KIND_VEC && s->h_W.size() == (size_t)s->n) {
        const StateDef& u = s->st_full.states[0];
        double m[3] = {0, 0, 0};
        for (long long c = 0; c < u.size / 3; c++) for (int q = 0; q < 3; q++) m[q] += s->h_W[u.offset + 3 * c + q];
        const double nm = std::sqrt(m[0] * m[0] + m[1] * m[1] + m[2] * m[2]);
        if (nm > 0.0) for (int q = 0; q < 3; q++) dir[q] = m[q] / nm;
    }
}

static const std::vector<unsigned char>& pc_mask(das_solver* s, das_ksp* k) { return (s->pcMask.empty() || k->pcTranspose) ? s->owned : s->pcMask; }
static int pc_configured_order(das_solver* s, das_ksp* k) { return k->pcOrder >= 0 ? k->pcOrder : (pc_ordering_rcm(s) ? 1 : 0); }
static bool pc_order_is_deep(int levels, int nodes) { return (double)levels > 30.0 * std::cbrt((double)std::max(1, nodes)); }
static const char* rank_label() { return getenv("RANK") ? getenv("RANK") : "0"; }

struct BiluInputs {
    const Mat& A;
    int reach, nthr;
    bool fp32, debug;
    double dir[3];
    BiluInputs(das_solver* s, das_ksp* k)
        : A(k->pcmat->m), reach(pc_stencil_reach(s)), nthr(pc_setup_threads(s)), fp32(s->opt.geti("amd.pcFactorFP32") != 0), debug(s->opt.geti("debug") != 0) { pc_flow_direction(s, dir); }
};
static void factorise_node_ilu(das_solver* s, das_ksp* k, NodeILU& P, const std::vector<unsigned char>& mask, int order) {
    const BiluInputs in(s, k);
    bilu_setup(s->mesh, s->st_full.states, s->n, mask, in.reach, in.fp32, in.A.n, in.A.rowptr.p, in.A.col.p, in.A.val.p, s->stream,
               P, in.debug, in.nthr, order, k->pcTranspose, k->pcDiagScale, k->shiftExLo, k->shiftExHi, k->shiftEnd, in.dir);
}
static void pc_finish_bilu(das_solver* s, das_ksp* k, double t0, int nBlocks, bool rasOverlap) {
    k->useBilu = true;
    k->rasOverlap = rasOverlap;
    if (k->rasOverlap && k->pcin.n != (size_t)s->n) k->pcin.alloc(s->n);
    k->pc.setup_seconds = wall_seconds() - t0;
    k->pc.nBlocks = nBlocks;
    k->pc.fnnz = (k->bilu.nL + k->bilu.nU + k->bilu.nNodes) * (long long)BILU_NB2;
    k->pc.next = (long long)k->bilu.nNodes * BILU_NB;
}

static double pc_stability_estimate(das_solver* s, das_ksp* k, NodeILU& F, const std::vector<unsigned char>& mask) {
    const long long n = s->n;
    const Mat& P = k->pcmat->m;
    std::vector<double> e(n), z(n);
    DevBuf<double> de(n), dw(n), dz(n);
    double est = 0.0;
    long long worst = -1;
    for (int trial = 0; trial < 2; trial++) {
        for (long long i = 0; i < n; i++) {
            const bool in = mask.empty() || mask[i];
            unsigned long long hsh = (unsigned long long)i * 0x9E3779B97F4A7C15ull;
            hsh ^= hsh >> 29;
            e[i] = !in ? 0.0 : (trial == 0 ? 1.0 : ((hsh & 1ull) ? 1.0 : -1.0));
        }
        de.upload(e);
        hipLaunchKernelGGL(k_spmv_wave, SPMV_GRID(P.n), dim3(256), 0, s->stream, P.n, P.rowptr.p, P.col.p, P.val.p, (const double*)de.p, dw.p);
        dz.zero();
        bilu_apply(F, dw.p, dz.p, s->stream);
        DAS_HIP(hipStreamSynchronize(s->stream));
        z = dz.to_host();
        const int* nu = F.h_nodeUnk.data();
        for (size_t q = 0; q < F.h_nodeUnk.size(); q++) {
            const int gi = nu[q];
            if (gi < 0) continue;
            const double d = std::fabs(z[gi] - e[gi]);
            if (d > est || d != d) worst = gi;
            est = (d > est || d != d) ? (d != d ? 1e300 : d) : est;
        }
    }
    if (worst >= 0 && getenv("DAS_PC_STAB")) {
        for (const StateDef& sd : s->st_full.states) {
            if (worst < sd.offset || worst >= sd.offset + sd.size) continue;
            const long long ent = (worst - sd.offset) / (sd.kind == KIND_VEC ? 3 : 1);
            const double* C = sd.kind == KIND_FACE ? s->mesh.fg[ent].Cf : s->mesh.cg[ent].C;
            fprintf(stderr, "[dafoam_amd] rank %s: worst entry of the stability test: state %s entity %lld at (%.4g %.4g %.4g)%s\n", rank_label(),
                    sd.name.c_str(), ent, C[0], C[1], C[2], (!s->owned.empty() && !s->owned[worst]) ? " (overlap ring)" : "");
        }
    }
    return est;
}

static void choose_order_and_factorise(das_solver* s, das_ksp* k, NodeILU& F, const std::vector<unsigned char>& mask, bool pickMin, int& orderUsed, double& estimate,
                                       bool earlyAccept = true) {
    const int configured = pc_configured_order(s, k);
    const double limit = s->opt.getd("amd.pcStabilityLimit");
    if (!(limit > 0.0)) {
        F = NodeILU();
        factorise_node_ilu(s, k, F, mask, configured);
        orderUsed = -1; estimate = -1.0;
        return;
    }
    std::vector<int> cand{configured};
    {
        std::string lst = s->opt.gets("amd.pcOrderCandidates");
        if (getenv("DAS_BILU_ORDER_LIST")) { lst = getenv("DAS_BILU_ORDER_LIST"); cand.clear(); }
        for (size_t q = 0; q < lst.size(); q++)
            if (lst[q] >= '0' && lst[q] <= '7') { const int o = lst[q] - '0'; if (std::find(cand.begin(), cand.end(), o) == cand.end()) cand.push_back(o); }
        if (cand.empty()) cand.push_back(configured);
    }
    if (getenv("DAS_BILU_PICK_MIN")) pickMin = atoi(getenv("DAS_BILU_PICK_MIN")) != 0;
    const double good = s->opt.getd("amd.pcStabilityGood");
    struct Cand { int o; double est; int levels; };
    std::vector<Cand> seen;
    int last = -1;
    for (size_t attempt = 0; attempt < cand.size(); attempt++) {
        const int o = cand[attempt];
        F = NodeILU();
        factorise_node_ilu(s, k, F, mask, o);
        const double est = pc_stability_estimate(s, k, F, mask);
        last = o;
        seen.push_back({o, est, F.nLevels});
        if (s->opt.geti("debug") || getenv("DAS_PC_STAB") || (est > limit && !pickMin))
            fprintf(stderr, "[dafoam_amd] rank %s: preconditioner stability estimate max|(LU)^-1 P e - e| = %.3e with elimination order %d, %d levels (limit %.1e)%s\n",
                    rank_label(), est, o, F.nLevels, limit, (est > limit && !pickMin) ? ": unstable, trying another order" : "");
        const bool deep = pc_order_is_deep(F.nLevels, F.nNodes);
        if (est <= limit && (!pickMin || (earlyAccept && est <= good && !deep))) break;
    }
    bool anyOk = false;
    for (const Cand& c : seen) anyOk = anyOk || c.est <= limit;
    int minLv = 1 << 30;
    for (const Cand& c : seen) if (!anyOk || c.est <= limit) minLv = std::min(minLv, c.levels);
    int best = seen.back().o;
    double bestEst = 1e300;
    if (!pickMin && seen.back().est <= limit) bestEst = seen.back().est;
    else
        for (const Cand& c : seen)
            if ((!anyOk || c.est <= limit) && (double)c.levels <= 1.5 * minLv && c.est < bestEst) { best = c.o; bestEst = c.est; }
    if (last != best) {
        F = NodeILU();
        factorise_node_ilu(s, k, F, mask, best);
    }
    if (bestEst > limit)
        fprintf(stderr, "[dafoam_amd] rank %s: no elimination order passes the stability limit; keeping order %d (estimate %.3e)\n", rank_label(), best, bestEst);
    orderUsed = best; estimate = bestEst;
}

static void setup_node_ilu(das_solver* s, das_ksp* k, bool byEstimate) {
    const double t0 = wall_seconds();
    if (byEstimate) {
        choose_order_and_factorise(s, k, k->bilu, pc_mask(s, k), !s->owned.empty(), k->pcOrderUsed, k->pcStability,  s->owned.empty());
        if (k->pcOrderUsed >= 0) k->pcOrder = k->pcOrderUsed;
    } else {
        factorise_node_ilu(s, k, k->bilu, pc_mask(s, k), pc_configured_order(s, k));
    }
    pc_finish_bilu(s, k, t0, 1, !s->pcMask.empty() && !k->pcTranspose && s->halo.ovActive);
}

static long long pc_subdomain_count(das_solver* s) {
    long long K = s->opt.geti("amd.pcSubdomains");
    if (!s->owned.empty()) return 1;
    if (K < 0) K = s->mesh.nC >= 1000000 ? 4 : 1;
    return std::max<long long>(1, std::min<long long>(K, 16));
}

template <class Fn>
static void for_each_unknown_with_cell(das_solver* s, Fn fn) {
    const Mesh& m = s->mesh;
    for (const StateDef& sd : s->st_full.states) {
        if (sd.kind == KIND_VEC) { for (int c = 0; c < m.nC; c++) for (int q = 0; q < 3; q++) fn(sd.offset + 3LL * c + q, c); }
        else if (sd.kind == KIND_SCL) { for (int c = 0; c < m.nC; c++) fn(sd.offset + c, c); }
        else { for (long long f = 0; f < m.nF; f++) fn(sd.offset + f, m.owner[f]); }
    }
}

static bool setup_subdomain_ilus(das_solver* s, das_ksp* k, int K) {
    const double t0 = wall_seconds();
    const Mesh& m = s->mesh;
    const long long N = m.nC, n = s->n;
    std::vector<int> cells(N), blockOf(N, 0);
    std::iota(cells.begin(), cells.end(), 0);
    rcb_parts(cells, [&](int c, int d) { return m.cg[c].C[d]; }, K, blockOf);
    std::vector<unsigned char> subOf(n, 0);
    for_each_unknown_with_cell(s, [&](long long g, int c) { subOf[g] = (unsigned char)blockOf[c]; });
    const int overlap = (int)std::max<long long>(0, s->opt.geti("adjEqnOption.asmOverlap"));
    std::vector<std::vector<unsigned char>> masks(K);
    k->subOrder.assign(K, -1);
    k->subEst.assign(K, -1.0);
    for (int b = 0; b < K; b++) {
        std::vector<unsigned char> cellIn(N, 0), grown;
        for (long long c = 0; c < N; c++) cellIn[c] = blockOf[c] == b;
        for (int ring = 0; ring < overlap; ring++) {
            grown = cellIn;
            for (long long c = 0; c < N; c++) if (cellIn[c]) for (int q = m.cc_ptr[c]; q < m.cc_ptr[c + 1]; q++) grown[m.cc[q]] = 1;
            cellIn.swap(grown);
        }
        masks[b].assign(n, 0);
        for_each_unknown_with_cell(s, [&](long long g, int c) { masks[b][g] = cellIn[c]; });
        NodeILU F;
        choose_order_and_factorise(s, k, F, masks[b], true, k->subOrder[b], k->subEst[b]);
        if (k->subOrder[b] < 0) k->subOrder[b] = pc_configured_order(s, k);
        if (s->opt.geti("debug") || getenv("DAS_PC_STAB"))
            fprintf(stderr, "[dafoam_amd] sub-domain %d of %d: %d nodes, %d levels, elimination order %d, stability estimate %.3e\n", b, K, F.nNodes, F.nLevels, k->subOrder[b], k->subEst[b]);
        if (pc_order_is_deep(F.nLevels, F.nNodes) && s->opt.geti("amd.pcSubdomains") < 0) {
            fprintf(stderr, "[dafoam_amd] sub-domain %d of %d needs %d dependency levels for %d nodes: the blocks do not suit this mesh, one factorisation instead "
                            "(amd.pcSubdomains K > 1 forces the blocks)\n", b, K, F.nLevels, F.nNodes);
            k->subOrder.clear(); k->subEst.clear();
            return false;
        }
    }
    {
        const BiluInputs in(s, k);
        std::vector<const std::vector<unsigned char>*> mp;
        for (int b = 0; b < K; b++) mp.push_back(&masks[b]);
        k->bilu = NodeILU();
        bilu_setup_multi(s->mesh, s->st_full.states, n, mp, k->subOrder, subOf, in.reach, in.fp32, in.A.n, in.A.rowptr.p, in.A.col.p, in.A.val.p, s->stream, k->bilu,
                         in.debug, in.nthr, in.dir);
    }
    k->nSub = K;
    k->pcOrderUsed = k->subOrder[0];
    k->pcStability = 0.0;
    for (double e : k->subEst) k->pcStability = std::max(k->pcStability, e);
    pc_finish_bilu(s, k, t0, K, false);
    if (s->opt.geti("debug") || getenv("DAS_PC_STAB"))
        fprintf(stderr, "[dafoam_amd] %d sub-domains merged: %d nodes, %d levels (%.0f nodes per level)\n", K, k->bilu.nNodes, k->bilu.nLevels, (double)k->bilu.nNodes / std::max(1, k->bilu.nLevels));
    return true;
}

static void coarse_build_operator(das_solver* s, das_ksp* k, int naggG, int aggOff, const std::vector<int>& aggRowG) {
    das_ksp::CoarsePC& C = k->coarse;
    C.active = false;
    DAS_CHECK(naggG >= C.nagg && naggG <= 2048, DAS_ERR_ARG, "coarse space: at most 2048 aggregates in total (dense inverse)");
    const long long N = C.N;
    std::vector<int> aggOwn(N, -1);
    for (long long c = 0; c < N; c++) if (C.h_agg[c] >= 0) aggOwn[c] = aggOff + C.h_agg[c];
    std::vector<long long> aptrAll;
    std::vector<int> cellsAll;
    coarse_sort_cells(N, naggG, aggRowG.data(), aptrAll, cellsAll);
    C.naggG = naggG; C.aggOff = aggOff; C.global = naggG > C.nagg;
    C.azOpId = -1; C.azReady = false;
    C.agg.upload(aggOwn); C.aggRow.upload(aggRowG); C.cellsAll.upload(cellsAll); C.aptrAll.upload(aptrAll);
    DevBuf<double> E((size_t)naggG * naggG);
    const Mat& P = k->pcmat->m;
    coarse_assemble(naggG, C.aptrAll.p, C.cellsAll.p, N, C.off, P.rowptr.p, P.col.p, P.val.p, k->pcTranspose ? C.aggRow.p : C.agg.p, E.p, k->pcTranspose ? 1 : 0,
                    (C.off < k->shiftEnd && !(C.off >= k->shiftExLo && C.off < k->shiftExHi)) ? k->pcDiagScale : 1.0, s->stream);
    if (C.global) {
        DAS_CHECK(!k->pcTranspose, DAS_ERR_ARG, "global coarse space: adjoint preconditioner only");
        rank_allreduce(s, E.p, naggG * naggG, s->stream);
    }
    {
        if (C.Einv.n < (size_t)naggG * naggG) C.Einv.alloc((size_t)naggG * naggG);
        DevBuf<int> sing(1);
        if (coarse_invert(naggG, E.p, C.Einv.p, sing.p, s->stream)) return;
    }
    C.t.alloc(naggG); C.u.alloc(naggG);
    C.active = true;
}

static void setup_coarse(das_solver* s, das_ksp* k) {
    das_ksp::CoarsePC& C = k->coarse;
    C.active = false;
    long long want = s->opt.geti("amd.pcCoarseAggregates");
    if (want == 0) return;
    const std::string field = s->opt.gets("amd.pcCoarseField");
    const StateDef* sd = nullptr;
    for (const StateDef& q : s->st_full.states) if (q.name == field && q.kind == KIND_SCL) sd = &q;
    if (!sd) return;
    const Mesh& m = s->mesh;
    const long long N = m.nC;
    std::vector<int> owned;
    owned.reserve(N);
    for (long long c = 0; c < N; c++) if (s->owned.empty() || s->owned[sd->offset + c]) owned.push_back((int)c);
    if (owned.size() < 64) return;
    if (want < 0) want = std::min<long long>(1024, std::max<long long>(16, (long long)owned.size() / 2048));
    int nagg = (int)std::min<long long>(want, std::min<long long>(2048, (long long)owned.size() / 4));
    if (nagg < 2) return;
    std::vector<int> agg(N, -1);
    const bool byStrength = s->opt.gets("amd.pcCoarseAggregation") == "strength";
    DAS_CHECK(byStrength || s->opt.gets("amd.pcCoarseAggregation") == "rcb", DAS_ERR_ARG, "amd.pcCoarseAggregation: rcb | strength");
    if (byStrength) {
        std::vector<unsigned char> mask;
        if (!s->owned.empty()) { mask.resize(N); for (long long c = 0; c < N; c++) mask[c] = s->owned[sd->offset + c]; }
        nagg = strength_aggregates(m, s->owned.empty() ? nullptr : &mask, nagg, agg);
        if (nagg < 2) return;
    } else {
        rcb_parts(owned, [&](int c, int d) { return m.cg[c].C[d]; }, nagg, agg);
    }
    std::vector<long long> aptr;
    std::vector<int> cells;
    coarse_sort_cells(N, nagg, agg.data(), aptr, cells);
    C.nagg = nagg; C.off = sd->offset; C.N = N; C.h_agg = agg;
    C.cells.upload(cells); C.aptr.upload(aptr);
    C.deflated = s->opt.gets("amd.pcCoarseMode") == "deflated";
    if (C.deflated) { C.c.alloc(s->n); C.rr.alloc(s->n); }
    coarse_build_operator(s, k, nagg, 0, agg);
    if (C.active && s->opt.geti("debug")) fprintf(stderr, "[dafoam_amd] coarse space: %d aggregates on field %s (%s)\n", nagg, field.c_str(), C.deflated ? "deflated" : "additive");
}
static void coarse_solve(das_solver* s, das_ksp* k, const double* r) {
    das_ksp::CoarsePC& C = k->coarse;
    if (C.global) DAS_HIP(hipMemsetAsync(C.t.p, 0, (size_t)C.naggG * sizeof(double), s->stream));
    coarse_restrict_solve(C.nagg, C.aptr.p, C.cells.p, C.off, r, C.naggG, C.aggOff, C.Einv.p, C.t.p, C.u.p, s->stream,
                          [&] { if (C.global) rank_allreduce(s, C.t.p, C.naggG, s->stream); });
}

static void pc_apply(das_solver* s, das_ksp* k, const double* b, double* x) {
    hipEvent_t ev = nullptr;
    s->timer.begin("pc", s->stream, ev);
    if (k->useBilu) {
        if (k->rasOverlap) {
            DAS_HIP(hipMemcpyAsync(k->pcin.p, b, (size_t)s->n * sizeof(double), hipMemcpyDeviceToDevice, s->stream));
            s->halo.gather_overlap(k->pcin.p, s->stream);
            bilu_apply(k->bilu, k->pcin.p, x, s->stream);
            s->halo.zero_overlap(x, s->stream);
        } else {
            bilu_apply(k->bilu, b, x, s->stream);
        }
        s->timer.end("pc", s->stream, ev);
        return;
    }
    const int mlv = k->pc.maxLevels;
    const size_t lvlBytes = (size_t)((mlv + 2 * PC_PF + 4) >> 1) * sizeof(double);
    if (k->pc.useLDS)
        hipLaunchKernelGGL(k_ras_apply<true>, dim3(k->pc.nBlocks), dim3(PC_THREADS), lvlBytes + (size_t)k->pc.maxLocal * sizeof(double), s->stream,
                           k->pc.view, b, x, mlv);
    else
        hipLaunchKernelGGL(k_ras_apply<false>, dim3(k->pc.nBlocks), dim3(PC_THREADS), lvlBytes, s->stream, k->pc.view, b, x, mlv);
    s->timer.end("pc", s->stream, ev);
}

static void gmres_ws(das_solver* s, das_ksp* k, int polyD = 0) {
    const long long n = s->n;
    long long restart = std::min<long long>(s->opt.geti("adjEqnOption.gmresRestart"), s->opt.geti("adjEqnOption.gmresMaxIters"));
    k->polyD = polyD;
    if (polyD > 0) restart = std::min<long long>(s->opt.geti("adjEqnOption.gmresRestart"), (std::max<long long>(s->opt.geti("adjEqnOption.gmresMaxIters"), 1) + polyD - 1) / polyD + polyD);
    const long long budget = s->opt.geti_or("amd.maxKrylovBytes", (long long)(32.0 * 1024 * 1024 * 1024));
    const long long nr = (n + 3) / 4 * 4;
    const long long maxVec = std::max<long long>(3, budget / (8 * nr));
    restart = std::max<long long>(1, std::min<long long>(restart, maxVec - 2));
    long long wantVec = std::max<long long>(restart + 2, std::min<long long>(maxVec, 1002));
    if ((size_t)wantVec * (size_t)nr * sizeof(double) < ((size_t)4 << 30) || getenv("DAS_NO_VMM") || polyD > 0) wantVec = restart + 2;
    if (k->V.n < (size_t)((restart + 2) * nr) || k->Vn != n) {
        k->V.reserve((size_t)(wantVec * nr));
        k->Vn = n;
    }
    {
        const std::string prec = s->opt.gets_or("amd.krylovBasisPrecision", "auto");
        DAS_CHECK(prec == "auto" || prec == "fp64" || prec == "fp32" || prec == "split", DAS_ERR_ARG, "amd.krylovBasisPrecision: auto | fp64 | split | fp32");
        const bool eligible = s->opt.geti("adjEqnOption.useMGSO") == 0 && !s->fwd.on;
        const bool dcgs2 = s->opt.gets("amd.gmresOrthogonalization") == "dcgs2" && s->opt.geti("adjEqnOption.useMGSO") == 0;
        bool big = (size_t)(restart + 2) * (size_t)n * 8 >= ((size_t)1 << 30);
        big = rank_any(s, big);
        k->split = eligible && (prec == "split" || (prec == "auto" && dcgs2 && big));
        k->vf32 = k->split || (eligible && prec == "fp32");
        if (k->vf32 && k->ustage.n != (size_t)n) k->ustage.alloc(n);
    }
    if (k->restart != restart || k->w.n != (size_t)n) {
        k->restart = (int)restart;
        k->w.alloc(n); k->z.alloc(n); k->r.alloc(n); k->xdev.alloc(n); k->bdev.alloc(n);
        k->z.zero();
        k->partial.alloc(std::max<size_t>(multidot_partial_size(n, (int)restart + 1), multidot2_partial_size(n, (int)restart + 2)));
        k->hdev.alloc(4 * (restart + 3));
    }
}
static inline long long basis_n4(das_solver* s) { return (s->n + 3) / 4 * 4; }
static inline long long basis_ld(das_solver* s, das_ksp* k) { return k->split ? 2 * basis_n4(s) : (k->vf32 ? basis_n4(s) : s->n); }
static inline bool gmres_map_basis(das_solver* s, das_ksp* k, long long nvec) {
    const long long per = basis_ld(s, k) / (k->vf32 ? 2 : 1);
    const long long ahead = k->polyD > 0 ? std::min<long long>(nvec + 64, (long long)k->restart + 2) : nvec + 64;
    k->V.request((size_t)(ahead * per));
    return k->V.try_ensure((size_t)(nvec * per));
}
template <class VT>
static inline VT* basis_slot(das_solver* s, das_ksp* k, long long j) { return reinterpret_cast<VT*>(k->V.p) + j * basis_ld(s, k); }
static inline float* basis_lo(das_solver* s, das_ksp* k, long long j) { return k->split ? reinterpret_cast<float*>(k->V.p) + j * basis_ld(s, k) + basis_n4(s) : nullptr; }

template <class VT>
static void multidot_dev(das_solver* s, das_ksp* k, const VT* Vbase, int m, const double* w, double* dev_out) {
    launch_multidot<VT>(s->stream, s->n, m, Vbase, basis_ld(s, k), w, k->partial.p, dev_out);
// ... 4330 lines not shown
    g_orth_wide = on ? 1 : 0;
    return DAS_OK;
}
int das_debug_krylov_wide_eligible(long long n, int fmt, long long ld, int* dots, int* update) {
    DAS_TRY
    DAS_CHECK(dots && update, DAS_ERR_ARG, "das_debug_krylov_wide_eligible: null pointer");
    const float* base = reinterpret_cast<const float*>((uintptr_t)1 << 20);
    const bool f = fmt == KRY_FP32 || fmt == KRY_SPLIT;
    *dots = (f && g_orth_wide && orth_wide_ok(n, base, nullptr, ld, base + ld, base)) ? 1 : 0;
    *update = (f && g_orth_wide && orth_wide_ok(n, base, fmt == KRY_SPLIT ? base + n : nullptr, ld, nullptr, base)) ? 1 : 0;
    return DAS_OK;
    DAS_CATCH
}

int das_debug_krylov_dots2(long long n, int K, int fmt, const void* V, long long ld, const double* v, double* out) {
    DAS_TRY
    krylov_check_basis("das_debug_krylov_dots2", n, K, fmt, V, ld);
    DAS_CHECK(v && out, DAS_ERR_ARG, "das_debug_krylov_dots2: null pointer");
    if (fmt == KRY_FP64) debug_krylov_dots2<double>(n, K, V, ld, v, out);
    else debug_krylov_dots2<float>(n, K, V, ld, v, out);
    return DAS_OK;
    DAS_CATCH
}
int das_debug_krylov_dcgs2_update(long long n, int j, int fmt, void* V, long long ld, int nslots, const double* sc, double gamma, double ralpha,
                                  const double* v) {
    DAS_TRY
    DAS_CHECK(j >= 0, DAS_ERR_ARG, "das_debug_krylov_dcgs2_update: j must not be negative");
    krylov_check_basis("das_debug_krylov_dcgs2_update", n, nslots, fmt, V, ld);
    DAS_CHECK(nslots >= j + 2, DAS_ERR_ARG, "das_debug_krylov_dcgs2_update: the basis needs slots 0 .. j + 1");
    DAS_CHECK(v && (sc || j == 0), DAS_ERR_ARG, "das_debug_krylov_dcgs2_update: null pointer");
    if (fmt == KRY_FP64) debug_krylov_dcgs2_update<double>(n, j, false, V, ld, nslots, sc, gamma, ralpha, v);
    else debug_krylov_dcgs2_update<float>(n, j, fmt == KRY_SPLIT, V, ld, nslots, sc, gamma, ralpha, v);
    return DAS_OK;
    DAS_CATCH
}
int das_debug_krylov_multidot(long long n, int m, int fmt, const void* V, long long ld, const double* w, double* out) {
    DAS_TRY
    DAS_CHECK(m >= 0, DAS_ERR_ARG, "das_debug_krylov_multidot: m must not be negative");
    krylov_check_basis("das_debug_krylov_multidot", n, std::max(m, 1), fmt, m > 0 ? V : (const void*)w, ld);
    DAS_CHECK(w && out, DAS_ERR_ARG, "das_debug_krylov_multidot: null pointer");
    if (fmt == KRY_FP64) debug_krylov_multidot<double>(n, m, V, ld, w, out);
    else debug_krylov_multidot<float>(n, m, V, ld, w, out);
    return DAS_OK;
    DAS_CATCH
}
int das_debug_krylov_multiaxpy(long long n, int m, int fmt, const void* V, long long ld, const double* h, int wfloat, void* w, long long wlen) {
    DAS_TRY
    krylov_check_basis("das_debug_krylov_multiaxpy", n, m, fmt, V, ld);
    DAS_CHECK(h && w, DAS_ERR_ARG, "das_debug_krylov_multiaxpy: null pointer");
    DAS_CHECK(wlen >= n, DAS_ERR_ARG, "das_debug_krylov_multiaxpy: w shorter than n");
    DAS_CHECK(!wfloat || fmt == KRY_FP32, DAS_ERR_ARG, "das_debug_krylov_multiaxpy: a float w goes with the fp32 basis only");
    if (fmt == KRY_FP64) debug_krylov_multiaxpy<double, double>(n, m, false, V, ld, h, w, wlen);
    else if (wfloat) debug_krylov_multiaxpy<float, float>(n, m, false, V, ld, h, w, wlen);
    else debug_krylov_multiaxpy<float, double>(n, m, fmt == KRY_SPLIT, V, ld, h, w, wlen);
    return DAS_OK;
    DAS_CATCH
}
int das_debug_krylov_lincomb(long long n, int m, int fmt, const void* V, long long ld, const double* c, double* y, long long ylen) {
    DAS_TRY
    krylov_check_basis("das_debug_krylov_lincomb", n, m, fmt, V, ld);
    DAS_CHECK(c && y, DAS_ERR_ARG, "das_debug_krylov_lincomb: null pointer");
    DAS_CHECK(ylen >= n, DAS_ERR_ARG, "das_debug_krylov_lincomb: y shorter than n");
    if (fmt == KRY_FP64) debug_krylov_lincomb<double>(n, m, false, V, ld, c, y, ylen);
    else debug_krylov_lincomb<float>(n, m, fmt == KRY_SPLIT, V, ld, c, y, ylen);
    return DAS_OK;
    DAS_CATCH
}
int das_debug_krylov_scale_to(long long n, double a, int use, const void* x, void* y, long long ylen) {
    DAS_TRY
    DAS_CHECK(n > 0, DAS_ERR_ARG, "das_debug_krylov_scale_to: n must be positive");
    DAS_CHECK(use >= 0 && use <= 4, DAS_ERR_ARG, "das_debug_krylov_scale_to: use is 0 (double -> double), 1 (double -> float), 2 (double -> split), 3 (split -> double) or 4 (float -> double)");
    DAS_CHECK(x && y, DAS_ERR_ARG, "das_debug_krylov_scale_to: null pointer");
    DAS_CHECK(ylen >= (use == 2 ? 2 * n : n), DAS_ERR_ARG, "das_debug_krylov_scale_to: y shorter than n (split: 2 n)");
    if (use == 0) debug_krylov_scale_to<double, double>(n, a, false, false, x, y, ylen);
    else if (use == 1) debug_krylov_scale_to<double, float>(n, a, false, false, x, y, ylen);
    else if (use == 2) debug_krylov_scale_to<double, float>(n, a, false, true, x, y, ylen);
    else if (use == 3) debug_krylov_scale_to<float, double>(n, a, true, false, x, y, ylen);
    else debug_krylov_scale_to<float, double>(n, a, false, false, x, y, ylen);
    return DAS_OK;
    DAS_CATCH
}
int das_debug_krylov_block_tn(long long n, int K, int s, const double* V, long long ldv, long long voff, const double* W, long long ldw, double* C) {
    DAS_TRY
    krylov_check_block("das_debug_krylov_block_tn", n, K, s);
    DAS_CHECK(V && W && C, DAS_ERR_ARG, "das_debug_krylov_block_tn: null pointer");
    DAS_CHECK(ldv >= n && ldw >= n && voff >= 0, DAS_ERR_ARG, "das_debug_krylov_block_tn: leading dimension below n or negative offset");
    debug_krylov_block_tn(n, K, s, V, ldv, voff, W, ldw, C);
    return DAS_OK;
    DAS_CATCH
}
int das_debug_krylov_block_nn_sub(long long n, int K, int s, const double* V, long long ldv, const double* C, double* W, long long ldw) {
    DAS_TRY
    krylov_check_block("das_debug_krylov_block_nn_sub", n, K, s);
    DAS_CHECK(V && W && C, DAS_ERR_ARG, "das_debug_krylov_block_nn_sub: null pointer");
    DAS_CHECK(ldv >= n && ldw >= n, DAS_ERR_ARG, "das_debug_krylov_block_nn_sub: leading dimension below n");
    debug_krylov_block_nn_sub(n, K, s, V, ldv, C, W, ldw);
    return DAS_OK;
    DAS_CATCH
}
int das_debug_krylov_block_right_mult(long long n, int s, double* W, long long ldw, const double* T) {
    DAS_TRY
    krylov_check_block("das_debug_krylov_block_right_mult", n, 1, s);
    DAS_CHECK(W && T, DAS_ERR_ARG, "das_debug_krylov_block_right_mult: null pointer");
    DAS_CHECK(ldw >= n, DAS_ERR_ARG, "das_debug_krylov_block_right_mult: leading dimension below n");
    debug_krylov_block_right_mult(n, s, W, ldw, T);
    return DAS_OK;
    DAS_CATCH
}
int das_debug_krylov_block_lincomb(long long n, int K, int s, const double* V, long long ldv, const double* C, double* Y, long long ldy) {
    DAS_TRY
    krylov_check_block("das_debug_krylov_block_lincomb", n, K, s);
    DAS_CHECK(V && C && Y, DAS_ERR_ARG, "das_debug_krylov_block_lincomb: null pointer");
    DAS_CHECK(ldv >= n && ldy >= n, DAS_ERR_ARG, "das_debug_krylov_block_lincomb: leading dimension below n");
    debug_krylov_block_lincomb(n, K, s, V, ldv, C, Y, ldy);
    return DAS_OK;
    DAS_CATCH
}
int das_debug_krylov_block_spmm(long long n, int s, const long long* rp, const int* ci, const double* val, const double* X, long long ldx, double* Y,
                                long long ldy) {
    DAS_TRY
    krylov_check_block("das_debug_krylov_block_spmm", n, 1, s);
    DAS_CHECK(rp && X && Y, DAS_ERR_ARG, "das_debug_krylov_block_spmm: null pointer");
    DAS_CHECK(ldx >= n && ldy >= n, DAS_ERR_ARG, "das_debug_krylov_block_spmm: leading dimension below n");
    DAS_CHECK(rp[0] == 0, DAS_ERR_ARG, "das_debug_krylov_block_spmm: rowptr[0] must be 0");
    for (long long i = 0; i < n; i++) DAS_CHECK(rp[i + 1] >= rp[i], DAS_ERR_ARG, "das_debug_krylov_block_spmm: rowptr decreases");
    const long long nnz = rp[n];
    DAS_CHECK(nnz == 0 || (ci && val), DAS_ERR_ARG, "das_debug_krylov_block_spmm: null pointer");
    for (long long k = 0; k < nnz; k++) DAS_CHECK(ci[k] >= 0 && ci[k] < n, DAS_ERR_ARG, "das_debug_krylov_block_spmm: column index out of range");
    debug_krylov_block_spmm(n, s, rp, ci, val, X, ldx, Y, ldy);
    return DAS_OK;
    DAS_CATCH
}

int das_debug_bilu_factor(const das_bilu_debug_t* in, long long* Lptr, long long* Uptr, int* Lcol, int* Ucol, void* Lval, void* Uval, double* invD,
                          int* nshift) {
    DAS_TRY
    bilu_debug_check("das_debug_bilu_factor", in);
    DAS_CHECK(Lptr && Uptr && Lcol && Ucol && Lval && Uval && invD && nshift, DAS_ERR_ARG, "das_debug_bilu_factor: null pointer");
    debug_bilu_factor(*in, Lptr, Uptr, Lcol, Ucol, Lval, Uval, invD, nshift);
    return DAS_OK;
    DAS_CATCH
}
int das_debug_bilu_apply(const das_bilu_debug_t* in, int nrhs, long long ld, const double* b, double* out, int twice, double* y, double* z,
                         int* abortFlag, int* info) {
    DAS_TRY
    bilu_debug_check("das_debug_bilu_apply", in);
    DAS_CHECK(nrhs >= 1 && nrhs <= 8, DAS_ERR_ARG, "das_debug_bilu_apply: 1 to 8 right-hand sides");
    DAS_CHECK(ld >= in->n, DAS_ERR_ARG, "das_debug_bilu_apply: leading dimension below n");
    DAS_CHECK(b && out && y && z && abortFlag && info, DAS_ERR_ARG, "das_debug_bilu_apply: null pointer");
    debug_bilu_apply(*in, nrhs, ld, b, out, twice, y, z, abortFlag, info);
    return DAS_OK;
    DAS_CATCH
}

#define DAS_GRAPH_DEVICE(who) DAS_CHECK(das_device_count() > 0, DAS_ERR_NO_DEVICE, std::string(who) + ": no HIP device visible")
int das_debug_graph_scan(long long n, const int* cnt, long long* out, long long* total) {
    DAS_TRY
    const std::string who = "das_debug_graph_scan";
    graph_check_sizes(who, n);
    DAS_CHECK(cnt && out && total, DAS_ERR_ARG, who + ": null pointer");
    for (long long i = 0; i < n; i++) DAS_CHECK(cnt[i] >= 0, DAS_ERR_ARG, who + ": negative count");
    DAS_GRAPH_DEVICE(who);
    debug_graph_scan(n, cnt, out, total);
    return DAS_OK;
    DAS_CATCH
}
int das_debug_graph_transpose(long long n, const long long* rowptr, const int* col, long long* trp, int* tcol) {
    DAS_TRY
    const std::string who = "das_debug_graph_transpose";
    graph_check_sizes(who, n);
    DAS_CHECK(rowptr && col && trp && tcol, DAS_ERR_ARG, who + ": null pointer");
    graph_check_csr(who, n, rowptr, col, n, true);
    DAS_CHECK(rowptr[n] > 0, DAS_ERR_ARG, who + ": a pattern without entries");
    DAS_GRAPH_DEVICE(who);
    debug_graph_transpose(n, rowptr, col, trp, tcol);
    return DAS_OK;
    DAS_CATCH
}
int das_debug_graph_nets(long long n, const long long* rowptr, const int* col, long long nKeep, const long long* keep, long long* cptr, int* crow, int* cpos,
                         unsigned char* isStart, long long* total) {
    DAS_TRY
    const std::string who = "das_debug_graph_nets";
    graph_check_sizes(who, n);
    DAS_CHECK(rowptr && col && cptr && crow && cpos && isStart && total && (keep || nKeep == 0), DAS_ERR_ARG, who + ": null pointer");
    graph_check_csr(who, n, rowptr, col, n, true);
    DAS_CHECK(rowptr[n] > 0, DAS_ERR_ARG, who + ": a pattern without entries");
    DAS_CHECK(nKeep >= 0 && nKeep <= n, DAS_ERR_ARG, who + ": nKeep outside [0, n]");
    {
        std::vector<unsigned char> seen((size_t)n, 0);
        for (long long q = 0; q < nKeep; q++) {
            DAS_CHECK(keep[q] >= 0 && keep[q] < n, DAS_ERR_ARG, who + ": kept row out of range");
            DAS_CHECK(!seen[keep[q]], DAS_ERR_ARG, who + ": kept row repeated");
            seen[keep[q]] = 1;
        }
    }
    DAS_GRAPH_DEVICE(who);
    debug_graph_nets(n, rowptr, col, nKeep, keep, cptr, crow, cpos, isStart, total);
    return DAS_OK;
    DAS_CATCH
}
int das_debug_graph_rows_gather(long long nSel, const long long* rows, long long n, const long long* rowptr, const int* col, const long long* dst, int* out,
                                long long outLen) {
    DAS_TRY
    const std::string who = "das_debug_graph_rows_gather";
    graph_check_sizes(who, n);
    DAS_CHECK(nSel > 0 && outLen > 0, DAS_ERR_ARG, who + ": sizes must be positive");
    DAS_CHECK(rows && rowptr && dst && out, DAS_ERR_ARG, who + ": null pointer");
    graph_check_csr(who, n, rowptr, col, n, false);
    for (long long q = 0; q < nSel; q++) {
        DAS_CHECK(rows[q] >= 0 && rows[q] < n, DAS_ERR_ARG, who + ": row index out of range");
        DAS_CHECK(dst[q] >= 0 && dst[q] <= outLen - (rowptr[rows[q] + 1] - rowptr[rows[q]]), DAS_ERR_ARG, who + ": a gathered row does not fit into out");
    }
    DAS_GRAPH_DEVICE(who);
    debug_graph_rows_gather(nSel, rows, n, rowptr, col, dst, out, outLen);
    return DAS_OK;
    DAS_CATCH
}
int das_debug_compact(long long n, const long long* rowptr, const int* col, const double* vals, double bound, int useBound, const unsigned char* owned,
                      long long* nrp, int* nci, double* nv, long long* nnzOut) {
    DAS_TRY
    const std::string who = "das_debug_compact";
    graph_check_sizes(who, n);
    DAS_CHECK(rowptr && nrp && nci && nv && nnzOut, DAS_ERR_ARG, who + ": null pointer");
    DAS_CHECK(useBound == 0 || useBound == 1, DAS_ERR_ARG, who + ": useBound is 0 or 1");
    graph_check_csr(who, n, rowptr, col, n, false);
    DAS_CHECK(rowptr[n] == 0 || vals, DAS_ERR_ARG, who + ": null pointer");
    DAS_GRAPH_DEVICE(who);
    debug_compact(n, rowptr, col, vals, bound, useBound != 0, owned, nrp, nci, nv, nnzOut);
    return DAS_OK;
    DAS_CATCH
}
int das_debug_vecpack(long long n, const long long* rowptr, const int* col, const double* vals, long long row0, long long nG, int* built, long long* cptr,
                      unsigned char* data, long long dataCap, long long* nChunks, const double* x, double* y, long long ylen) {
    DAS_TRY
    const std::string who = "das_debug_vecpack";
    graph_check_sizes(who, n);
    DAS_CHECK(nG > 0, DAS_ERR_ARG, who + ": sizes must be positive");
    DAS_CHECK(rowptr && built && cptr && data && nChunks && (!x || y), DAS_ERR_ARG, who + ": null pointer");
    DAS_CHECK(row0 >= 0 && nG <= n && row0 <= n - 3 * nG, DAS_ERR_ARG, who + ": the group rows [row0, row0 + 3 nG) do not lie in [0, n)");
    DAS_CHECK(!x || ylen >= n, DAS_ERR_ARG, who + ": y shorter than n");
    graph_check_csr(who, n, rowptr, col, n, false);
    DAS_CHECK(rowptr[n] == 0 || vals, DAS_ERR_ARG, who + ": null pointer");
    long long need = 0;
    for (long long g = 0; g < nG; g++) need += (rowptr[row0 + 3 * g + 1] - rowptr[row0 + 3 * g] + VP_CHUNK - 1) / VP_CHUNK;
    DAS_CHECK(dataCap >= need * VP_CHUNK_BYTES, DAS_ERR_ARG, who + ": data holds fewer bytes than the chunks of the group rows");
    DAS_GRAPH_DEVICE(who);
    debug_vecpack(n, rowptr, col, vals, row0, nG, built, cptr, data, nChunks, x, y, ylen);
    return DAS_OK;
    DAS_CATCH
}
int das_debug_spmv_rows(long long nrows, const int* rows, long long n, const long long* rowptr, const int* col, const double* vals, const double* x, double* buf,
                        long long buflen) {
    DAS_TRY
    const std::string who = "das_debug_spmv_rows";
    graph_check_sizes(who, n);
    DAS_CHECK(nrows > 0, DAS_ERR_ARG, who + ": sizes must be positive");
    DAS_CHECK(rows && rowptr && x && buf, DAS_ERR_ARG, who + ": null pointer");
    DAS_CHECK(buflen >= nrows, DAS_ERR_ARG, who + ": buf shorter than nrows");
    graph_check_csr(who, n, rowptr, col, n, false);
    DAS_CHECK(rowptr[n] == 0 || vals, DAS_ERR_ARG, who + ": null pointer");
    for (long long k = 0; k < nrows; k++) DAS_CHECK(rows[k] >= 0 && rows[k] < n, DAS_ERR_ARG, who + ": row index out of range");
    DAS_GRAPH_DEVICE(who);
    debug_spmv_rows(nrows, rows, n, rowptr, col, vals, x, buf, buflen);
    return DAS_OK;
    DAS_CATCH
}
int das_debug_coarse_assemble(int nagg, long long N, long long off, long long n, const long long* rowptr, const int* col, const double* vals, const int* aggRow,
                              const int* aggCol, int transpose, double diagScale, double* E) {
    DAS_TRY
    const std::string who = "das_debug_coarse_assemble";
    coarse_check_nagg(who, nagg);
    coarse_check_field(who, N, off, n);
    DAS_CHECK(rowptr && aggRow && aggCol && E, DAS_ERR_ARG, who + ": null pointer");
    DAS_CHECK(transpose == 0 || transpose == 1, DAS_ERR_ARG, who + ": transpose is 0 or 1");
    graph_check_csr(who, n, rowptr, col, n, false);
    DAS_CHECK(rowptr[n] == 0 || vals, DAS_ERR_ARG, who + ": null pointer");
    coarse_check_agg(who, N, nagg, aggRow);
    coarse_check_agg(who, N, nagg, aggCol);
    DAS_GRAPH_DEVICE(who);
    debug_coarse_assemble(nagg, N, off, n, rowptr, col, vals, aggRow, aggCol, transpose, diagScale, E);
    return DAS_OK;
    DAS_CATCH
}
int das_debug_coarse_invert(int n, const double* Ein, double* Inv, int* singular) {
    DAS_TRY
    const std::string who = "das_debug_coarse_invert";
    DAS_CHECK(n >= 1 && n <= COARSE_MAX_AGG, DAS_ERR_ARG, who + ": n outside 1 .. 2048");
    DAS_CHECK(Ein && Inv && singular, DAS_ERR_ARG, who + ": null pointer");
    DAS_GRAPH_DEVICE(who);
    debug_coarse_invert(n, Ein, Inv, singular);
    return DAS_OK;
    DAS_CATCH
}
int das_debug_coarse_correct(int nagg, long long N, long long off, long long n, const int* agg, const double* Einv, const double* r, double* t, double* u, double* y,
                             long long ylen, int set) {
    DAS_TRY
    const std::string who = "das_debug_coarse_correct";
    coarse_check_nagg(who, nagg);
    coarse_check_field(who, N, off, n);
    DAS_CHECK(Einv && r && t && u && y, DAS_ERR_ARG, who + ": null pointer");
    DAS_CHECK(ylen >= n && ylen < (1LL << 31), DAS_ERR_ARG, who + ": y shorter than n");
    DAS_CHECK(set == 0 || set == 1, DAS_ERR_ARG, who + ": set is 0 or 1");
    coarse_check_agg(who, N, nagg, agg);
    DAS_GRAPH_DEVICE(who);
    debug_coarse_correct(nagg, N, off, n, agg, Einv, r, t, u, y, ylen, set);
    return DAS_OK;
// ... 48 lines not shown
```

include/dafoam_amd.h:

```cpp
#ifndef DAFOAM_AMD_H
#define DAFOAM_AMD_H

#ifdef __cplusplus
extern "C" {
#endif

#define DAS_OK 0
#define DAS_ERR_ARG -1
#define DAS_ERR_NO_DEVICE -2
#define DAS_ERR_HIP -3
#define DAS_ERR_STATE -4
#define DAS_ERR_INTERNAL -5

#define DAS_SOLVER_SIMPLEFOAM 0
#define DAS_SOLVER_SCALARTRANSPORTFOAM 1
#define DAS_SOLVER_RHOSIMPLEFOAM 2
#define DAS_SOLVER_TURBOFOAM 3
#define DAS_SOLVER_HEATTRANSFERFOAM 4
#define DAS_IS_COMPRESSIBLE(s) ((s) == DAS_SOLVER_RHOSIMPLEFOAM || (s) == DAS_SOLVER_TURBOFOAM)

#define DAS_PATCH_PATCH 0
#define DAS_PATCH_WALL 1
#define DAS_PATCH_SYMMETRY 2
#define DAS_PATCH_CYCLIC 3
// ... 145 lines not shown
int das_define_patch_field_function(das_solver_t* s, const char* name, const char* type, const int* patch_ids, int npatch, const char* var,
                                    const int* comps, int ncomp, const double* data, int flags, double scale, double ref);
int das_define_cell_function(das_solver_t* s, const char* name, const char* type, const int* cells, int ncells, const char* var, const int* comps,
                             int ncomp, const double* data, int flags, double scale, double ref);
int das_calc_function(das_solver_t* s, const char* name, double* value);
int das_define_force_coupling(das_solver_t* s, const char* name, const int* patch_ids, int npatch, double pRef);
int das_calc_force_coupling(das_solver_t* s, const char* name, double* out, int n);
int das_define_thermal_coupling(das_solver_t* s, const char* name, const int* patch_ids, int npatch, int flags);
int das_calc_thermal_coupling(das_solver_t* s, const char* name, double* out, int n);
int das_define_thermal_coupling_input(das_solver_t* s, const char* name, const int* patch_ids, int npatch, int flags);
int das_set_thermal_coupling_input(das_solver_t* s, const char* name, const double* in, int n);
int das_get_patch_mixed(das_solver_t* s, int patch, double* refValue, double* valueFraction);
int das_calc_dthermal_coupling_product(das_solver_t* s, const char* inputName, const char* outputName, const char* outputType, const double* seeds,
                                       double* product, int n);

int das_define_heat_source(das_solver_t* s, const char* name, const char* kind, const double* pars, double eps, int snapCenter2Cell);
int das_set_heat_source_pars(das_solver_t* s, const char* name, const int* indices, int n, const double* values);
int das_get_heat_source_info(das_solver_t* s, const char* name, double* pars9, double* volumeTotal, double* sourceTotal, int* snappedCell);
int das_get_heat_source_cells(das_solver_t* s, const char* name, int* cells, int cap);
int das_get_fv_source(das_solver_t* s, double* out);
int das_calc_dfvsourcepar_product(das_solver_t* s, const char* name, const int* indices, int n, const char* outputName, const char* outputType,
                                  const double* seeds, double* product);

int das_define_actuator_disk(das_solver_t* s, const char* name, const char* kind, const double* pars, const char* rotDir, double eps, int adjustThrust);
int das_set_actuator_disk_pars(das_solver_t* s, const char* name, const int* indices, int n, const double* values);
int das_get_actuator_disk_info(das_solver_t* s, const char* name, double* pars13, double* info4, int* nCells);
int das_get_actuator_disk_cells(das_solver_t* s, const char* name, int* cells, int cap);
int das_get_fv_source_vector(das_solver_t* s, double* out);
int das_calc_dactuatordiskpar_product(das_solver_t* s, const char* name, const int* indices, int n, const char* outputName, const char* outputType,
                                      const double* seeds, double* product);

int das_get_input_size(das_solver_t* s, const char* inputName, const char* inputType);
int das_get_output_size(das_solver_t* s, const char* outputName, const char* outputType);
int das_calc_jac_t_vec_product(das_solver_t* s, const char* inputName, const char* inputType, const double* inputs,
                               const char* outputName, const char* outputType, const double* seeds, double* product);
int das_drdwt_mult_device(das_solver_t* s, const double* d_x, double* d_y);

int das_create_ml_rksp_matrix_free(das_solver_t* s, das_mat_t* pc, das_ksp_t** ksp);
int das_solve_linear_eqn(das_solver_t* s, das_ksp_t* ksp, const double* rhs, double* sol);
int das_solve_linear_eqn_block(das_solver_t* s, das_ksp_t* ksp, int nrhs, const double* rhs, double* sol, double* res0, double* res);
int das_ksp_apply_pc(das_solver_t* s, das_ksp_t* ksp, const double* x, double* y);
int das_ksp_get_n_blocks(das_ksp_t* ksp);
long long das_ksp_get_factor_nnz(das_ksp_t* ksp);
long long das_ksp_get_n_ext(das_ksp_t* ksp);
int das_ksp_get_blocks(das_ksp_t* ksp, int* perm, long long* block_off);
int das_pc_structure_build(das_solver_t* s, int* nNodes, long long* nBlocks, int* nLevels, int* reach);
int das_pc_structure_get(das_solver_t* s, int* nodeUnk, long long* bptr, int* bcol, int* lvlPtr, int* natural);
int das_ksp_get_pc_structure_sizes(das_ksp_t* ksp, int* nNodes, long long* nBlocks, int* nLevels);
int das_ksp_get_pc_structure(das_ksp_t* ksp, int* nodeUnk, long long* bptr, int* bcol, int* lvlPtr, int* natural);
int das_ksp_get_pc_node_out(das_ksp_t* ksp, int* nodeOut);
int das_ksp_get_info(das_ksp_t* ksp, int* iters, double* res0, double* res, double* seconds);
int das_ksp_get_history(das_ksp_t* ksp, double* hist, int cap);
int das_ksp_get_basis_info(das_ksp_t* ksp, int* fp32, double* mappedBytes, double* bytesPerVector);
int das_ksp_get_cycle_lengths(das_ksp_t* ksp, int* lens, int cap);
int das_ksp_get_n_refine(das_ksp_t* ksp);
int das_set_dense_eig_callback(void* fn);
int das_debug_gmres_dr_restart(int m, int kwant, const double* Hbar, const double* rvec, double* P1, double* Hnew, double* cnew);
int das_debug_block_chol(int sv, const double* G, double* L, double* T);
int das_debug_block_lsq(int sv, int m, int ncols, const double* S0, const double* Hc, const double* Hc2, const double* S, double* Y, double* res);
int das_debug_gmres_dr_host(long long n, void* A, void* M, void* user, const double* b, double* x, int m, int kdef, double rtol, double atol,
                            long long maxIts, double* hist, int histCap, double* info4, double* res2);
int das_ksp_get_idr_info(das_ksp_t* ksp, int* s, int* cycles, int* restarts, int* breakdowns, int* workVectors, double* workBytes);
int das_debug_idrs_host(long long n, void* A, void* M, void* user, const double* b, double* x, int s, int seed, double rtol, double atol, long long maxIts,
                        double* hist, int histCap, double* info4, double* res2);
int das_debug_idr_cycle_host(long long n, void* A, void* M, void* user, const double* b, double* x, int s, int seed, double* r, double* P, double* G,
                             double* U);
int das_debug_idr_shadow(long long n, int s, long long ld, int seed, int device, double* P);
int das_debug_idr_combine(long long n, int m, double a, const double* x, double* V, long long ld, long long vlen, const double* c, long long yoff, double* y,
                          long long ylen);
int das_debug_idr_biortho_step(long long n, int k, double* G, double* U, long long ld, long long glen, const double* coef, double* r, double* x,
                               long long vlen, double* rr);
int das_debug_idr_smooth_step(long long n, int s, double omega, double* r, const double* t, double* x, const double* z, long long vlen, double* P,
                              long long ld, long long plen, double* out);
int das_ksp_get_poly_info(das_ksp_t* ksp, int* degree, int* nComplexPairs, long long* products, long long* columns, long long* generatingColumns, int* generated,
                          int* fallback, int* workVectors, double* workBytes, int* nRoots, double* re, double* im);
int das_debug_poly_roots(int d, const double* Hbar, double* re, double* im);
int das_debug_poly_apply_host(long long n, void* A, void* M, void* user, int nroots, const double* re, const double* im, const double* v, double* out);
int das_debug_poly_step(long long n, int kind, int first, int last, double re, double im, long long off, long long len, double* v, double* w, double* prod, double* poly,
                        double* tmp);
int das_debug_ksp_poly_apply(das_solver_t* s, das_ksp_t* ksp, const double* v, double* out);
int das_ksp_get_status(das_ksp_t* ksp, int* reason, int* nBreakdown, int* nSweepGrid, int* sweepPerXcd);
int das_ksp_get_pc_stability(das_ksp_t* ksp, double* estimate, int* orderUsed);
int das_ksp_get_pc_subdomains(das_ksp_t* ksp, int* orders, double* estimates);
int das_ksp_get_coarse(das_ksp_t* ksp, int* aggOfCell);
int das_ksp_coarse_sparse_az_active(das_ksp_t* ksp);
int das_ksp_set_global_coarse(das_solver_t* s, das_ksp_t* ksp, int naggGlobal, int aggOffset, const int* aggRowGlobal);
int das_ksp_run_fixed_device(das_solver_t* s, das_ksp_t* ksp, const double* d_rhs, double* d_sol, int iters);
int das_ksp_begin_device(das_solver_t* s, das_ksp_t* ksp, const double* d_rhs, double* d_sol, int fixed);
int das_ksp_advance(das_solver_t* s, das_ksp_t* ksp, int iters);
int das_ksp_end(das_solver_t* s, das_ksp_t* ksp);
void das_ksp_destroy(das_ksp_t* k);

typedef void (*das_halo_cb)(double* d_vec, void* user);
typedef void (*das_allreduce_cb)(double* d_buf, int n, void* user);
int das_set_owned_mask(das_solver_t* s, const unsigned char* owned );
int das_set_comm(das_solver_t* s, das_halo_cb halo, das_allreduce_cb allreduce, void* user);
int das_comm_load_rccl(void);
typedef void (*das_exchange_cb)(double* d_send, double* d_recv, void* user);
int das_comm_unique_id(char* out128);
int das_comm_init_rccl(das_solver_t* s, int rank, int world, const char* id128);
int das_comm_set_halo(das_solver_t* s, int npeers, const int* peers, const long long* sendOff, const int* sendIdx, const long long* recvOff,
                      const int* recvIdx, long long nGhost, const int* ghostIdx);
int das_set_exchange_cb(das_solver_t* s, das_exchange_cb cb, void* user);
int das_set_pc_overlap(das_solver_t* s, const unsigned char* pcMask , int npeers, const long long* ovSendOff, const int* ovSendIdx,
                       const long long* ovRecvOff, const int* ovRecvIdx);
int das_set_gather_cb(das_solver_t* s, das_exchange_cb cb, void* user);
int das_comm_is_native(das_solver_t* s);
int das_comm_reset(das_solver_t* s);
int das_set_stream(das_solver_t* s, void* hip_stream);

double das_get_elapsed_clock_time(das_solver_t* s);
double das_get_elapsed_cpu_time(das_solver_t* s);
double das_timer_avg_ms(das_solver_t* s, const char* name);
int das_debug_orth_bench(long long n, int K, int reps, int rows, int unroll, int rpt, double* ms_dots, double* ms_update);
int das_debug_orth_bench_split(long long n, int K, int reps, int fmt, int variant, int rows, int unroll, int rpt, double* ms_dots, double* ms_update);
int das_debug_set_orth_wide(int on, int* previous);
int das_debug_krylov_wide_eligible(long long n, int fmt, long long ld, int* dots, int* update);
int das_debug_krylov_dots2(long long n, int K, int fmt, const void* V, long long ld, const double* v, double* out);
int das_debug_krylov_dcgs2_update(long long n, int j, int fmt, void* V, long long ld, int nslots, const double* sc, double gamma, double ralpha,
                                  const double* v);
int das_debug_krylov_multidot(long long n, int m, int fmt, const void* V, long long ld, const double* w, double* out);
int das_debug_krylov_multiaxpy(long long n, int m, int fmt, const void* V, long long ld, const double* h, int wfloat, void* w, long long wlen);
int das_debug_krylov_lincomb(long long n, int m, int fmt, const void* V, long long ld, const double* c, double* y, long long ylen);
int das_debug_krylov_scale_to(long long n, double a, int use, const void* x, void* y, long long ylen);
int das_debug_krylov_block_tn(long long n, int K, int s, const double* V, long long ldv, long long voff, const double* W, long long ldw, double* C);
int das_debug_krylov_block_nn_sub(long long n, int K, int s, const double* V, long long ldv, const double* C, double* W, long long ldw);
int das_debug_krylov_block_right_mult(long long n, int s, double* W, long long ldw, const double* T);
int das_debug_krylov_block_lincomb(long long n, int K, int s, const double* V, long long ldv, const double* C, double* Y, long long ldy);
int das_debug_krylov_block_spmm(long long n, int s, const long long* rowptr, const int* colidx, const double* vals, const double* X, long long ldx,
                                double* Y, long long ldy);
typedef struct {
    int nNodes, nLevels, nMaps;
    int fp32, transpose;
    long long n, An;
    const int* nodeUnk;
    const int* nodeOut;
    const unsigned char* late;
    const long long* bptr;
    const long long* bdiag;
    const int* bcol;
    const int* lvlPtr;
    const int* unkNode;
    const unsigned char* unkSlot;
    const long long* rp;
    const int* ci;
    const double* val;
    double diagScale;
    long long shiftExLo, shiftExHi, shiftEnd;
} das_bilu_debug_t;
int das_debug_bilu_factor(const das_bilu_debug_t* in, long long* Lptr, long long* Uptr, int* Lcol, int* Ucol, void* Lval, void* Uval, double* invD,
                          int* nshift);
int das_debug_bilu_apply(const das_bilu_debug_t* in, int nrhs, long long ld, const double* b, double* out, int twice, double* y, double* z,
                         int* abortFlag, int* info);
int das_debug_graph_scan(long long n, const int* cnt, long long* out, long long* total);
int das_debug_graph_transpose(long long n, const long long* rowptr, const int* col, long long* trp, int* tcol);
int das_debug_graph_nets(long long n, const long long* rowptr, const int* col, long long nKeep, const long long* keep, long long* cptr, int* crow, int* cpos,
                         unsigned char* isStart, long long* total);
int das_debug_graph_rows_gather(long long nSel, const long long* rows, long long n, const long long* rowptr, const int* col, const long long* dst, int* out,
                                long long outLen);
int das_debug_compact(long long n, const long long* rowptr, const int* col, const double* vals, double bound, int useBound, const unsigned char* owned,
                      long long* nrp, int* nci, double* nv, long long* nnzOut);
int das_debug_vecpack(long long n, const long long* rowptr, const int* col, const double* vals, long long row0, long long nG, int* built, long long* cptr,
                      unsigned char* data, long long dataCap, long long* nChunks, const double* x, double* y, long long ylen);
int das_debug_spmv_rows(long long nrows, const int* rows, long long n, const long long* rowptr, const int* col, const double* vals, const double* x, double* buf,
                        long long buflen);
int das_debug_coarse_assemble(int nagg, long long N, long long off, long long n, const long long* rowptr, const int* col, const double* vals, const int* aggRow,
                              const int* aggCol, int transpose, double diagScale, double* E);
int das_debug_coarse_invert(int n, const double* Ein, double* Inv, int* singular);
int das_debug_coarse_correct(int nagg, long long N, long long off, long long n, const int* agg, const double* Einv, const double* r, double* t, double* u, double* y,
                             long long ylen, int set);
int das_debug_coarse_az(int nagg, long long n, const long long* rowptr, const int* col, const double* vals, long long N, long long off, const int* agg, int* cnt,
                        long long* ptr, int* oa, double* ov, long long cap, long long* nnz, int* overflow, const double* u, const double* v, double* out,
                        long long outlen);
long long das_timer_count(das_solver_t* s, const char* name);
void das_timer_reset(das_solver_t* s);
void das_timer_enable(das_solver_t* s, int on);

#ifdef __cplusplus
}
#endif
#endif
```

Measured before the change: 43.91.

## Reuse sub-domain ILU factors in merge instead of refactorising the whole matrix

The multi-subdomain block ILU set-up now keeps each sub-domain's factorisation and merges the packed factors on the device with copy kernels (rows, columns, inverse diagonals), instead of rebuilding structure and refactorising the merged matrix. Scratch buffers for scatter and the stability estimate are reused across order candidates, and the best candidate factor is kept so it need not be refactorised. An environment switch restores the old rebuild path, and per-phase timing and memory diagnostics are added. This targets preconditioner set-up cost, not the per-iteration GMRES kernels, so it affects the iteration rate only if set-up time is counted; holding several factors at once raises peak device memory.

After: 43.84. About the same (-0.2%).

```diff
diff --git a/dafoam_amd/_capi.py b/dafoam_amd/_capi.py
--- a/dafoam_amd/_capi.py
+++ b/dafoam_amd/_capi.py
@@ -407,6 +407,7 @@
     "das_debug_krylov_block_spmm": (C.c_int, [C.c_longlong, C.c_int, c_ll_p, c_int_p, c_double_p, c_double_p, C.c_longlong, c_double_p, C.c_longlong]),
     "das_debug_bilu_factor": (C.c_int, [C.POINTER(das_bilu_debug_t), c_ll_p, c_ll_p, c_int_p, c_int_p, _VP, _VP, c_double_p, c_int_p]),
     "das_debug_bilu_apply": (C.c_int, [C.POINTER(das_bilu_debug_t), C.c_int, C.c_longlong, c_double_p, c_double_p, C.c_int, c_double_p, c_double_p, c_int_p, c_int_p]),
+    "das_debug_bilu_stab_max": (C.c_int, [C.c_longlong, C.c_longlong, c_int_p, c_double_p, c_double_p, c_double_p, c_ll_p]),
     "das_debug_graph_scan": (C.c_int, [C.c_longlong, c_int_p, c_ll_p, c_ll_p]),
     "das_debug_graph_transpose": (C.c_int, [C.c_longlong, c_ll_p, c_int_p, c_ll_p, c_int_p]),
     "das_debug_graph_nets": (C.c_int, [C.c_longlong, c_ll_p, c_int_p, C.c_longlong, c_ll_p, c_ll_p, c_int_p, c_int_p, C.POINTER(C.c_ubyte), c_ll_p]),
diff --git a/dafoam_amd/csrc/das_bilu.hpp b/dafoam_amd/csrc/das_bilu.hpp
--- a/dafoam_amd/csrc/das_bilu.hpp
+++ b/dafoam_amd/csrc/das_bilu.hpp
@@ -459,6 +459,7 @@
     int mS = 0;
     BiluView view;
     double t_struct = 0, t_scatter = 0, t_factor = 0, t_pack = 0;
+    double gbPeak = 0;
     long long factor_bytes() const { return (nL + nU) * BILU_NB2 * (fp32 ? 4 : 8) + (long long)nNodes * BILU_NB2 * 8; }
 };
 
@@ -673,6 +674,19 @@
 struct NodeILU;
 inline void bilu_launch_shape(NodeILU& P, hipStream_t st);
 
+struct BiluStabPart { double val; long long q, nanq; };
+
+struct BiluSetupWork {
+    DevBuf<double> bval, e, w, z;
+    DevBuf<unsigned char> mask;
+    DevBuf<BiluStabPart> part;
+};
+inline double bilu_device_gb_in_use() {
+    size_t fr = 0, tot = 0;
+    if (hipMemGetInfo(&fr, &tot) != hipSuccess) { (void)hipGetLastError(); return -1.0; }
+    return (double)(tot - fr) / 1e9;
+}
+
 struct BiluStructRef {
     const std::vector<long long>* bptr;
     const std::vector<long long>* bdiag;
@@ -681,7 +695,8 @@
     std::vector<const std::vector<unsigned char>*> unkSlot;
 };
 inline void bilu_numeric(long long n, const BiluStructRef& S, bool fp32, long long An, const long long* d_rp, const int* d_ci, const double* d_av, hipStream_t st, NodeILU& P,
-                         bool debug, bool transpose, double diagScale, long long shiftExLo, long long shiftExHi, long long shiftEnd, double t0);
+                         bool debug, bool transpose, double diagScale, long long shiftExLo, long long shiftExHi, long long shiftEnd, double t0,
+                         BiluSetupWork* W = nullptr);
 
 inline std::vector<char> cells_of_mask(const Mesh& m, const std::vector<StateDef>& states, const std::vector<unsigned char>& mask) {
     std::vector<char> in(m.nC, 1);
@@ -695,7 +710,7 @@
 inline void bilu_setup(const Mesh& m, const std::vector<StateDef>& states, long long n, const std::vector<unsigned char>& owned, int reach,
                        bool fp32, long long An, const long long* d_rp, const int* d_ci, const double* d_av, hipStream_t st, NodeILU& P,
                        bool debug, int nthr, int order, bool transpose = false, double diagScale = 1.0, long long shiftExLo = 0,
-                       long long shiftExHi = 0, long long shiftEnd = (long long)1 << 62, const double* dir = nullptr) {
+                       long long shiftExHi = 0, long long shiftEnd = (long long)1 << 62, const double* dir = nullptr, BiluSetupWork* W = nullptr) {
     const double t0 = wall_seconds();
     const std::vector<char> cellOwned = cells_of_mask(m, states, owned);
     std::vector<int> unkNode, bcol;
@@ -703,11 +718,27 @@
     std::vector<long long> bptr, bdiag;
     bilu_build_structure(m, states, n, owned, cellOwned, reach, P, unkNode, unkSlot, bptr, bdiag, bcol, std::max(1, nthr), order, dir);
     BiluStructRef S{&bptr, &bdiag, &bcol, {&unkNode}, {&unkSlot}};
-    bilu_numeric(n, S, fp32, An, d_rp, d_ci, d_av, st, P, debug, transpose, diagScale, shiftExLo, shiftExHi, shiftEnd, t0);
+    bilu_numeric(n, S, fp32, An, d_rp, d_ci, d_av, st, P, debug, transpose, diagScale, shiftExLo, shiftExHi, shiftEnd, t0, W);
+}
+
+inline void bilu_finish(NodeILU& P, hipStream_t st) {
+    const int nN = P.nNodes;
+    P.y.alloc((size_t)nN * BILU_NB); P.z.alloc((size_t)nN * BILU_NB);
+    P.ctrl.alloc(BILU_CTRL_SIZE);
+    DAS_HIP(hipMemsetAsync(P.ctrl.p, 0, BILU_CTRL_SIZE * sizeof(unsigned), st));
+    DAS_HIP(hipStreamSynchronize(st));
+    P.view.nNodes = nN; P.view.nodeUnk = P.nodeUnk.p;
+    if (!P.h_nodeOut.empty()) P.nodeOut.upload(P.h_nodeOut);
+    P.view.nodeOut = P.h_nodeOut.empty() ? P.nodeUnk.p : P.nodeOut.p;
+    P.view.ptr[0] = P.Lptr.p; P.view.ptr[1] = P.Uptr.p; P.view.col[0] = P.Lcol.p; P.view.col[1] = P.Ucol.p;
+    P.view.val[0] = P.Lval.p; P.view.val[1] = P.Uval.p; P.view.valf[0] = P.Lvalf.p; P.view.valf[1] = P.Uvalf.p;
+    P.view.invD = P.invD.p; P.view.y = P.y.p; P.view.z = P.z.p; P.view.ctrl = P.ctrl.p;
+    bilu_launch_shape(P, st);
+    P.ready = true;
 }
 
 inline void bilu_numeric(long long n, const BiluStructRef& S, bool fp32, long long An, const long long* d_rp, const int* d_ci, const double* d_av, hipStream_t st, NodeILU& P,
-                         bool debug, bool transpose, double diagScale, long long shiftExLo, long long shiftExHi, long long shiftEnd, double t0) {
+                         bool debug, bool transpose, double diagScale, long long shiftExLo, long long shiftExHi, long long shiftEnd, double t0, BiluSetupWork* W) {
     const int nN = P.nNodes;
     P.fp32 = fp32;
     P.nodeUnk.upload(P.h_nodeUnk);
@@ -719,10 +750,14 @@
     DevBuf<unsigned char> d_late;
     d_late.upload(P.h_late);
     d_bptr.upload(bptr); d_bdiag.upload(bdiag); d_bcol.upload(bcol);
-    DevBuf<double> bval((size_t)P.nnzB * BILU_NB2);
+    const size_t nbval = (size_t)P.nnzB * BILU_NB2;
+    DevBuf<double> bvalOwn;
+    if (!W) bvalOwn.alloc(nbval);
+    else if (W->bval.n < nbval) W->bval.alloc(nbval);
+    double* const bval = W ? W->bval.p : bvalOwn.p;
     DevBuf<unsigned long long> d_dropped(1);
     DevBuf<int> d_nshift(1);
-    DAS_HIP(hipMemsetAsync(bval.p, 0, bval.n * sizeof(double), st));
+    DAS_HIP(hipMemsetAsync(bval, 0, nbval * sizeof(double), st));
     DAS_HIP(hipMemsetAsync(d_dropped.p, 0, sizeof(unsigned long long), st));
     DAS_HIP(hipMemsetAsync(d_nshift.p, 0, sizeof(int), st));
     P.t_struct = wall_seconds() - t0;
@@ -730,10 +765,10 @@
     for (size_t q = 0; q < S.unkNode.size(); q++) {
         d_unkNode.upload(*S.unkNode[q]); d_unkSlot.upload(*S.unkSlot[q]);
         hipLaunchKernelGGL(k_bilu_scatter, dim3((unsigned)((An + 15) / 16)), dim3(256), 0, st, An, d_rp, d_ci, d_av, d_unkNode.p, d_unkSlot.p, d_bptr.p,
-                           d_bcol.p, d_late.p, bval.p, d_dropped.p, transpose ? 1 : 0, diagScale, shiftExLo, shiftExHi, shiftEnd);
+                           d_bcol.p, d_late.p, bval, d_dropped.p, transpose ? 1 : 0, diagScale, shiftExLo, shiftExHi, shiftEnd);
         DAS_HIP(hipStreamSynchronize(st));
     }
-    hipLaunchKernelGGL(k_bilu_pad_diag, dim3((unsigned)(((long long)nN * BILU_NB + 255) / 256)), dim3(256), 0, st, nN, P.nodeUnk.p, d_bdiag.p, bval.p);
+    hipLaunchKernelGGL(k_bilu_pad_diag, dim3((unsigned)(((long long)nN * BILU_NB + 255) / 256)), dim3(256), 0, st, nN, P.nodeUnk.p, d_bdiag.p, bval);
     DAS_HIP(hipGetLastError());
     unsigned long long dropped = 0;
     DAS_HIP(hipMemcpyAsync(&dropped, d_dropped.p, sizeof(dropped), hipMemcpyDeviceToHost, st));
@@ -745,7 +780,7 @@
     for (int l = 0; l < P.nLevels; l++) {
         const int a = P.h_lvlPtr[l], bnd = P.h_lvlPtr[l + 1];
         if (bnd > a)
-            hipLaunchKernelGGL(k_bilu_factor, dim3((unsigned)((bnd - a + 3) / 4)), dim3(256), 0, st, a, bnd, d_bptr.p, d_bdiag.p, d_bcol.p, bval.p, P.invD.p,
+            hipLaunchKernelGGL(k_bilu_factor, dim3((unsigned)((bnd - a + 3) / 4)), dim3(256), 0, st, a, bnd, d_bptr.p, d_bdiag.p, d_bcol.p, bval, P.invD.p,
                                d_nshift.p);
     }
     DAS_HIP(hipGetLastError());
@@ -762,28 +797,18 @@
     if (fp32) {
         P.Lvalf.alloc((size_t)std::max<long long>(P.nL, 1) * BILU_NB2); P.Uvalf.alloc((size_t)std::max<long long>(P.nU, 1) * BILU_NB2);
         P.Lval.release(); P.Uval.release();
-        hipLaunchKernelGGL(k_bilu_pack<float>, dim3((unsigned)((nN + 3) / 4)), dim3(256), 0, st, nN, d_bptr.p, d_bdiag.p, d_bcol.p, bval.p, P.Lptr.p,
+        hipLaunchKernelGGL(k_bilu_pack<float>, dim3((unsigned)((nN + 3) / 4)), dim3(256), 0, st, nN, d_bptr.p, d_bdiag.p, d_bcol.p, bval, P.Lptr.p,
                            P.Uptr.p, P.Lcol.p, P.Ucol.p, P.Lvalf.p, P.Uvalf.p);
     } else {
         P.Lval.alloc((size_t)std::max<long long>(P.nL, 1) * BILU_NB2); P.Uval.alloc((size_t)std::max<long long>(P.nU, 1) * BILU_NB2);
         P.Lvalf.release(); P.Uvalf.release();
-        hipLaunchKernelGGL(k_bilu_pack<double>, dim3((unsigned)((nN + 3) / 4)), dim3(256), 0, st, nN, d_bptr.p, d_bdiag.p, d_bcol.p, bval.p, P.Lptr.p,
+        hipLaunchKernelGGL(k_bilu_pack<double>, dim3((unsigned)((nN + 3) / 4)), dim3(256), 0, st, nN, d_bptr.p, d_bdiag.p, d_bcol.p, bval, P.Lptr.p,
                            P.Uptr.p, P.Lcol.p, P.Ucol.p, P.Lval.p, P.Uval.p);
     }
     DAS_HIP(hipGetLastError());
-    P.y.alloc((size_t)nN * BILU_NB); P.z.alloc((size_t)nN * BILU_NB);
-    P.ctrl.alloc(BILU_CTRL_SIZE);
-    DAS_HIP(hipMemsetAsync(P.ctrl.p, 0, BILU_CTRL_SIZE * sizeof(unsigned), st));
-    DAS_HIP(hipStreamSynchronize(st));
+    bilu_finish(P, st);
     P.t_pack = wall_seconds() - t1;
-    P.view.nNodes = nN; P.view.nodeUnk = P.nodeUnk.p;
-    if (!P.h_nodeOut.empty()) P.nodeOut.upload(P.h_nodeOut);
-    P.view.nodeOut = P.h_nodeOut.empty() ? P.nodeUnk.p : P.nodeOut.p;
-    P.view.ptr[0] = P.Lptr.p; P.view.ptr[1] = P.Uptr.p; P.view.col[0] = P.Lcol.p; P.view.col[1] = P.Ucol.p;
-    P.view.val[0] = P.Lval.p; P.view.val[1] = P.Uval.p; P.view.valf[0] = P.Lvalf.p; P.view.valf[1] = P.Uvalf.p;
-    P.view.invD = P.invD.p; P.view.y = P.y.p; P.view.z = P.z.p; P.view.ctrl = P.ctrl.p;
-    bilu_launch_shape(P, st);
-    P.ready = true;
+    P.gbPeak = (debug || getenv("DAS_PC_STAB")) ? bilu_device_gb_in_use() : 0.0;
     if (debug)
         fprintf(stderr, "[dafoam_amd] node-block ILU(0): %d nodes (%.3f slots/unknown), %lld blocks (%.1f per node, max %d), %d levels, %d shifted pivots, "
                         "factor %.2f GB%s; structure %.2f s, scatter %.3f s, factorise %.3f s, pack %.3f s\n", nN, (double)nN * BILU_NB / (double)n, P.nnzB,
@@ -791,19 +816,14 @@
                 P.t_pack);
 }
 
-inline void bilu_setup_multi(const Mesh& m, const std::vector<StateDef>& states, long long n, const std::vector<const std::vector<unsigned char>*>& masks,
-                             const std::vector<int>& orders, const std::vector<unsigned char>& subOf, int reach, bool fp32, long long An, const long long* d_rp,
-                             const int* d_ci, const double* d_av, hipStream_t st, NodeILU& P, bool debug, int nthr, const double* dir) {
-    const double t0 = wall_seconds();
-    const int K = (int)masks.size();
-    struct Blk { NodeILU S; std::vector<int> unkNode, bcol, newPos; std::vector<unsigned char> unkSlot; std::vector<long long> bptr, bdiag; };
-    std::vector<Blk> B(K);
+struct BiluBlock { NodeILU S; std::vector<int> unkNode, bcol, newPos; std::vector<unsigned char> unkSlot; std::vector<long long> bptr, bdiag; };
+
+inline void bilu_merge_structure(long long n, std::vector<BiluBlock>& B, const std::vector<unsigned char>& subOf, int nthr, NodeILU& P,
+                                 std::vector<long long>& bptr, std::vector<long long>& bdiag, std::vector<int>& bcol) {
+    const int K = (int)B.size();
     int nLv = 0;
     long long nN = 0, nnzB = 0;
     for (int b = 0; b < K; b++) {
-        const std::vector<unsigned char>& mask = *masks[b];
-        const std::vector<char> cellOwned = cells_of_mask(m, states, mask);
-        bilu_build_structure(m, states, n, mask, cellOwned, reach, B[b].S, B[b].unkNode, B[b].unkSlot, B[b].bptr, B[b].bdiag, B[b].bcol, std::max(1, nthr), orders[b], dir);
         nLv = std::max(nLv, B[b].S.nLevels);
         nN += B[b].S.nNodes;
         nnzB += B[b].S.nnzB;
@@ -819,10 +839,11 @@
             for (int l = 0; l < B[b].S.nLevels; l++) for (int p = B[b].S.h_lvlPtr[l]; p < B[b].S.h_lvlPtr[l + 1]; p++) B[b].newPos[p] = cursor[l]++;
         }
     }
-    std::vector<long long> bptr(nN + 1, 0), bdiag(nN, -1);
+    bptr.assign(nN + 1, 0);
+    bdiag.assign(nN, -1);
     for (int b = 0; b < K; b++) for (int p = 0; p < B[b].S.nNodes; p++) bptr[B[b].newPos[p] + 1] = B[b].bptr[p + 1] - B[b].bptr[p];
     for (long long p = 0; p < nN; p++) bptr[p + 1] += bptr[p];
-    std::vector<int> bcol((size_t)bptr[nN]);
+    bcol.assign((size_t)bptr[nN], 0);
     P = NodeILU();
     P.h_nodeUnk.assign((size_t)nN * BILU_NB, -1);
     P.h_nodeOut.assign((size_t)nN * BILU_NB, -1);
@@ -831,7 +852,7 @@
     int maxRow = 0, nPrimary = 0;
     long long natOff = 0;
     for (int b = 0; b < K; b++) {
-        Blk& Q = B[b];
+        BiluBlock& Q = B[b];
 #pragma omp parallel for schedule(static) num_threads(std::max(1, nthr))
         for (int p = 0; p < Q.S.nNodes; p++) {
             const long long np = Q.newPos[p];
@@ -847,20 +868,133 @@
             P.h_late[np] = Q.S.h_late[p];
             P.h_natural[np] = (int)(natOff + Q.S.h_natural[p]);
         }
-        for (long long g = 0; g < n; g++) if (Q.unkNode[g] >= 0) Q.unkNode[g] = Q.newPos[Q.unkNode[g]];
+        if (!Q.unkNode.empty()) for (long long g = 0; g < n; g++) if (Q.unkNode[g] >= 0) Q.unkNode[g] = Q.newPos[Q.unkNode[g]];
         maxRow = std::max(maxRow, Q.S.maxRow);
         nPrimary += Q.S.nPrimary;
         natOff += Q.S.nNodes;
-        Q.S = NodeILU();
         std::vector<int>().swap(Q.bcol);
         std::vector<long long>().swap(Q.bptr);
         std::vector<long long>().swap(Q.bdiag);
     }
     P.n = n; P.nNodes = (int)nN; P.nLevels = nLv; P.nnzB = bptr[nN]; P.maxRow = maxRow; P.nPrimary = nPrimary;
     P.h_bptr = bptr; P.h_bcol = bcol; P.h_lvlPtr = lvlPtr;
+}
+
+inline void bilu_setup_multi(const Mesh& m, const std::vector<StateDef>& states, long long n, const std::vector<const std::vector<unsigned char>*>& masks,
+                             const std::vector<int>& orders, const std::vector<unsigned char>& subOf, int reach, bool fp32, long long An, const long long* d_rp,
+                             const int* d_ci, const double* d_av, hipStream_t st, NodeILU& P, bool debug, int nthr, const double* dir) {
+    const double t0 = wall_seconds();
+    const int K = (int)masks.size();
+    std::vector<BiluBlock> B(K);
+    for (int b = 0; b < K; b++) {
+        const std::vector<unsigned char>& mask = *masks[b];
+        const std::vector<char> cellOwned = cells_of_mask(m, states, mask);
+        bilu_build_structure(m, states, n, mask, cellOwned, reach, B[b].S, B[b].unkNode, B[b].unkSlot, B[b].bptr, B[b].bdiag, B[b].bcol, std::max(1, nthr), orders[b], dir);
+    }
+    std::vector<long long> bptr, bdiag;
+    std::vector<int> bcol;
+    bilu_merge_structure(n, B, subOf, nthr, P, bptr, bdiag, bcol);
+    for (int b = 0; b < K; b++) B[b].S = NodeILU();
     BiluStructRef S{&bptr, &bdiag, &bcol, {}, {}};
     for (int b = 0; b < K; b++) { S.unkNode.push_back(&B[b].unkNode); S.unkSlot.push_back(&B[b].unkSlot); }
     bilu_numeric(n, S, fp32, An, d_rp, d_ci, d_av, st, P, debug, false, 1.0, 0, 0, (long long)1 << 62, t0);
+}
+
+template <class VT>
+__global__ void __launch_bounds__(256) k_bilu_merge_rows(int nNb, int nNm, int lower, const int* __restrict__ newPos, const long long* __restrict__ sptr,
+                                                         const int* __restrict__ scol, const VT* __restrict__ sval, const long long* __restrict__ dptr,
+                                                         int* __restrict__ dcol, VT* __restrict__ dval) {
+    const int lane = threadIdx.x & 63;
+    const long long p = (long long)blockIdx.x * 4 + (threadIdx.x >> 6);
+    if (p >= nNb) return;
+    const int np = newPos[p];
+    const long long sr = lower ? p : nNb - 1 - p, dr = lower ? np : nNm - 1 - np;
+    const long long s0 = sptr[sr], nE = sptr[sr + 1] - s0, d0 = dptr[dr];
+    for (long long a = lane; a < nE; a += 64) dcol[d0 + a] = newPos[scol[s0 + a]];
+    for (long long a = lane; a < nE * BILU_NB2; a += 64) dval[d0 * BILU_NB2 + a] = sval[s0 * BILU_NB2 + a];
+}
+__global__ void k_bilu_merge_invd(long long nNb, const int* __restrict__ newPos, const double* __restrict__ src, double* __restrict__ dst) {
+    const long long i = (long long)blockIdx.x * 256 + threadIdx.x;
+    if (i < nNb * BILU_NB2) dst[(long long)newPos[i / BILU_NB2] * BILU_NB2 + (i % BILU_NB2)] = src[i];
+}
+
+inline void bilu_merge_blocks(long long n, std::vector<NodeILU>& F, const std::vector<unsigned char>& subOf, bool fp32, hipStream_t st, NodeILU& P, bool debug,
+                              int nthr) {
+    const double t0 = wall_seconds();
+    const int K = (int)F.size();
+    std::vector<BiluBlock> B(K);
+    for (int b = 0; b < K; b++) {
+        BiluBlock& Q = B[b];
+        Q.S = std::move(F[b]);
+        DAS_CHECK(Q.S.ready && Q.S.fp32 == fp32 && Q.S.n == n, DAS_ERR_INTERNAL, "multi-block preconditioner: a block has no factor to merge");
+        Q.bptr.swap(Q.S.h_bptr);
+        Q.bcol.swap(Q.S.h_bcol);
+        Q.bdiag.resize(Q.S.nNodes);
+#pragma omp parallel for schedule(static) num_threads(std::max(1, nthr))
+        for (int p = 0; p < Q.S.nNodes; p++) {
+            const int* row = Q.bcol.data() + Q.bptr[p];
+            Q.bdiag[p] = Q.bptr[p] + (std::lower_bound(row, row + (Q.bptr[p + 1] - Q.bptr[p]), p) - row);
+        }
+    }
+    F.clear();
+    std::vector<long long> bptr, bdiag;
+    std::vector<int> bcol;
+    bilu_merge_structure(n, B, subOf, nthr, P, bptr, bdiag, bcol);
+    const int nN = P.nNodes;
+    P.fp32 = fp32;
+    P.t_struct = wall_seconds() - t0;
+    const double t1 = wall_seconds();
+    std::vector<long long> Lptr(nN + 1, 0), Uptr(nN + 1, 0);
+    for (int p = 0; p < nN; p++) Lptr[p + 1] = Lptr[p] + (bdiag[p] - bptr[p]);
+    for (int q = 0; q < nN; q++) { const int p = nN - 1 - q; Uptr[q + 1] = Uptr[q] + (bptr[p + 1] - bdiag[p] - 1); }
+    P.nL = Lptr[nN]; P.nU = Uptr[nN];
+    long long nLb = 0, nUb = 0;
+    for (int b = 0; b < K; b++) { nLb += B[b].S.nL; nUb += B[b].S.nU; P.nshift += B[b].S.nshift; }
+    DAS_CHECK(nLb == P.nL && nUb == P.nU, DAS_ERR_INTERNAL, "multi-block preconditioner: the merged streams do not have the blocks' sizes");
+    std::vector<long long>().swap(bptr); std::vector<long long>().swap(bdiag); std::vector<int>().swap(bcol);
+    P.Lptr.upload(Lptr); P.Uptr.upload(Uptr);
+    P.nodeUnk.upload(P.h_nodeUnk);
+    std::vector<DevBuf<int>> d_newPos(K);
+    for (int b = 0; b < K; b++) d_newPos[b].upload(B[b].newPos);
+    const bool measure = debug || getenv("DAS_PC_STAB");
+    for (int lower = 1; lower >= 0; lower--) {
+        const size_t nE = (size_t)std::max<long long>(lower ? P.nL : P.nU, 1);
+        DevBuf<int>& dcol = lower ? P.Lcol : P.Ucol;
+        dcol.alloc(nE);
+        if (fp32) (lower ? P.Lvalf : P.Uvalf).alloc(nE * BILU_NB2);
+        else (lower ? P.Lval : P.Uval).alloc(nE * BILU_NB2);
+        if (measure) P.gbPeak = std::max(P.gbPeak, bilu_device_gb_in_use());
+        for (int b = 0; b < K; b++) {
+            NodeILU& S = B[b].S;
+            const dim3 grid((unsigned)((S.nNodes + 3) / 4));
+            if (fp32)
+                hipLaunchKernelGGL(k_bilu_merge_rows<float>, grid, dim3(256), 0, st, S.nNodes, nN, lower, d_newPos[b].p, (lower ? S.Lptr : S.Uptr).p, (lower ? S.Lcol : S.Ucol).p,
+                                   (lower ? S.Lvalf : S.Uvalf).p, (lower ? P.Lptr : P.Uptr).p, dcol.p, (lower ? P.Lvalf : P.Uvalf).p);
+            else
+                hipLaunchKernelGGL(k_bilu_merge_rows<double>, grid, dim3(256), 0, st, S.nNodes, nN, lower, d_newPos[b].p, (lower ? S.Lptr : S.Uptr).p, (lower ? S.Lcol : S.Ucol).p,
+                                   (lower ? S.Lval : S.Uval).p, (lower ? P.Lptr : P.Uptr).p, dcol.p, (lower ? P.Lval : P.Uval).p);
+            DAS_HIP(hipGetLastError());
+            DAS_HIP(hipStreamSynchronize(st));
+            (lower ? S.Lptr : S.Uptr).release(); (lower ? S.Lcol : S.Ucol).release();
+            (lower ? S.Lval : S.Uval).release(); (lower ? S.Lvalf : S.Uvalf).release();
+        }
+    }
+    P.invD.alloc((size_t)nN * BILU_NB2);
+    if (measure) P.gbPeak = std::max(P.gbPeak, bilu_device_gb_in_use());
+    for (int b = 0; b < K; b++) {
+        NodeILU& S = B[b].S;
+        const long long cnt = (long long)S.nNodes * BILU_NB2;
+        hipLaunchKernelGGL(k_bilu_merge_invd, dim3((unsigned)((cnt + 255) / 256)), dim3(256), 0, st, (long long)S.nNodes, d_newPos[b].p, S.invD.p, P.invD.p);
+        DAS_HIP(hipGetLastError());
+        DAS_HIP(hipStreamSynchronize(st));
+        S = NodeILU();
+    }
+    bilu_finish(P, st);
+    P.t_pack = wall_seconds() - t1;
+    if (debug)
+        fprintf(stderr, "[dafoam_amd] node-block ILU(0): %d blocks merged: %d nodes, %lld blocks (%.1f per node, max %d), %d levels, %d shifted pivots, factor %.2f GB%s; "
+                        "structure %.2f s, copy %.3f s\n", K, nN, P.nnzB, (double)P.nnzB / nN, P.maxRow, P.nLevels, P.nshift, P.factor_bytes() / 1e9, fp32 ? " (fp32)" : "",
+                P.t_struct, P.t_pack);
 }
 
 __global__ void k_bilu_xcd_probe(unsigned* mask) {
@@ -938,4 +1072,67 @@
 
 inline void bilu_clear_abort(NodeILU& P, hipStream_t st) { DAS_HIP(hipMemsetAsync(P.ctrl.p + BILU_CTRL_ABORT, 0, sizeof(unsigned), st)); }
 
-}
+__global__ void k_bilu_stab_trial(long long n, const unsigned char* __restrict__ mask, int trial, double* __restrict__ e) {
+    for (long long i = (long long)blockIdx.x * 256 + threadIdx.x; i < n; i += (long long)gridDim.x * 256) {
+        const bool in = !mask || mask[i];
+        unsigned long long hsh = (unsigned long long)i * 0x9E3779B97F4A7C15ull;
+        hsh ^= hsh >> 29;
+        e[i] = !in ? 0.0 : (trial == 0 ? 1.0 : ((hsh & 1ull) ? 1.0 : -1.0));
+    }
+}
+
+__device__ inline void bilu_stab_combine(BiluStabPart& a, const BiluStabPart& b) {
+    if (b.val > a.val || (b.val == a.val && b.q >= 0 && (a.q < 0 || b.q < a.q))) { a.val = b.val; a.q = b.q; }
+    a.nanq = a.nanq > b.nanq ? a.nanq : b.nanq;
+}
+__device__ inline void bilu_stab_block_reduce(BiluStabPart mine, BiluStabPart* out) {
+    __shared__ BiluStabPart sh[256];
+    sh[threadIdx.x] = mine;
+    __syncthreads();
+    for (int w = 128; w > 0; w >>= 1) {
+        if ((int)threadIdx.x < w) bilu_stab_combine(sh[threadIdx.x], sh[threadIdx.x + w]);
+        __syncthreads();
+    }
+    if (threadIdx.x == 0) *out = sh[0];
+}
+__global__ void __launch_bounds__(256) k_bilu_stab_max(long long nslots, long long qlo, const int* __restrict__ nodeUnk, const double* __restrict__ z,
+                                                       const double* __restrict__ e, BiluStabPart* __restrict__ part) {
+    BiluStabPart m{-1.0, -1, -1};
+    for (long long q = qlo + (long long)blockIdx.x * 256 + threadIdx.x; q < nslots; q += (long long)gridDim.x * 256) {
+        const int gi = nodeUnk[q];
+        if (gi < 0) continue;
+        const double d = fabs(z[gi] - e[gi]);
+        if (d != d) m.nanq = q;
+        else if (d > m.val) { m.val = d; m.q = q; }
+    }
+    bilu_stab_block_reduce(m, part + blockIdx.x);
+}
+__global__ void __launch_bounds__(256) k_bilu_stab_final(int nparts, BiluStabPart* part) {
+    BiluStabPart m{-1.0, -1, -1};
+    for (int i = threadIdx.x; i < nparts; i += 256) bilu_stab_combine(m, part[i]);
+    bilu_stab_block_reduce(m, part);
+}
+
+inline void bilu_stab_reduce(long long nslots, const int* d_nodeUnk, const double* d_z, const double* d_e, DevBuf<BiluStabPart>& part, hipStream_t st, double& est,
+                             long long& slot) {
+    const int grid = (int)std::max<long long>(1, std::min<long long>(1024, (nslots + 255) / 256));
+    if (part.n < (size_t)grid) part.alloc(1024);
+    auto scan_from = [&](long long qlo) {
+        BiluStabPart h{-1.0, -1, -1};
+        hipLaunchKernelGGL(k_bilu_stab_max, dim3(grid), dim3(256), 0, st, nslots, qlo, d_nodeUnk, d_z, d_e, part.p);
+        hipLaunchKernelGGL(k_bilu_stab_final, dim3(1), dim3(256), 0, st, grid, part.p);
+        DAS_HIP(hipGetLastError());
+        DAS_HIP(hipMemcpyAsync(&h, part.p, sizeof(h), hipMemcpyDeviceToHost, st));
+        DAS_HIP(hipStreamSynchronize(st));
+        return h;
+    };
+    BiluStabPart h = scan_from(0);
+    if (h.nanq >= 0) {
+        est = 1e300;
+        slot = h.nanq;
+        h = scan_from(h.nanq + 1);
+    }
+    if (h.val > est) { est = h.val; slot = h.q; }
+}
+
+}
diff --git a/dafoam_amd/csrc/das_bilu_debug.hpp b/dafoam_amd/csrc/das_bilu_debug.hpp
--- a/dafoam_amd/csrc/das_bilu_debug.hpp
+++ b/dafoam_amd/csrc/das_bilu_debug.hpp
@@ -120,4 +120,19 @@
     info[0] = P.launchGrid; info[1] = P.launchSleep; info[2] = P.launchPerXcd; info[3] = bilu_xcd_probe(0);
 }
 
+static void debug_bilu_stab_max(long long n, long long nslots, const int* nodeUnk, const double* z, const double* e, double* est, long long* slot) {
+    const std::string who = "das_debug_bilu_stab_max";
+    DAS_CHECK(nodeUnk && z && e && est && slot, DAS_ERR_ARG, who + ": null pointer");
+    DAS_CHECK(n > 0 && nslots > 0 && n < (1LL << 31) && nslots < (1LL << 31), DAS_ERR_ARG, who + ": sizes out of range (0 < n, nslots < 2^31)");
+    for (long long q = 0; q < nslots; q++) DAS_CHECK(nodeUnk[q] >= -1 && nodeUnk[q] < n, DAS_ERR_ARG, who + ": nodeUnk out of range");
+    DAS_CHECK(das_device_count() > 0, DAS_ERR_NO_DEVICE, who + ": no HIP device visible");
+    DevBuf<int> d_nu((size_t)nslots);
+    DevBuf<double> d_z((size_t)n), d_e((size_t)n);
+    DevBuf<BiluStabPart> part;
+    d_nu.upload(nodeUnk, (size_t)nslots); d_z.upload(z, (size_t)n); d_e.upload(e, (size_t)n);
+    *est = 0.0;
+    *slot = -1;
+    bilu_stab_reduce(nslots, d_nu.p, d_z.p, d_e.p, part, 0, *est, *slot);
 }
+
+}
diff --git a/dafoam_amd/csrc/das_device.hip b/dafoam_amd/csrc/das_device.hip
--- a/dafoam_amd/csrc/das_device.hip
+++ b/dafoam_amd/csrc/das_device.hip
@@ -643,6 +643,7 @@
     int nSub = 1;
     std::vector<int> subOrder;
     std::vector<double> subEst;
+    struct PcSetupTimes { double structure = 0, scatter = 0, factor = 0, pack = 0, estimate = 0, merge = 0, gbPeak = 0; int factorisations = 0; } pcTimes;
     int pcOrder = -1;
     int pcOrderUsed = -1;
     double pcStability = -1.0;
@@ -1371,10 +1372,13 @@
     BiluInputs(das_solver* s, das_ksp* k)
         : A(k->pcmat->m), reach(pc_stencil_reach(s)), nthr(pc_setup_threads(s)), fp32(s->opt.geti("amd.pcFactorFP32") != 0), debug(s->opt.geti("debug") != 0) { pc_flow_direction(s, dir); }
 };
-static void factorise_node_ilu(das_solver* s, das_ksp* k, NodeILU& P, const std::vector<unsigned char>& mask, int order) {
+static void factorise_node_ilu(das_solver* s, das_ksp* k, NodeILU& P, const std::vector<unsigned char>& mask, int order, BiluSetupWork* W = nullptr) {
     const BiluInputs in(s, k);
     bilu_setup(s->mesh, s->st_full.states, s->n, mask, in.reach, in.fp32, in.A.n, in.A.rowptr.p, in.A.col.p, in.A.val.p, s->stream,
-               P, in.debug, in.nthr, order, k->pcTranspose, k->pcDiagScale, k->shiftExLo, k->shiftExHi, k->shiftEnd, in.dir);
+               P, in.debug, in.nthr, order, k->pcTranspose, k->pcDiagScale, k->shiftExLo, k->shiftExHi, k->shiftEnd, in.dir, W);
+    das_ksp::PcSetupTimes& T = k->pcTimes;
+    T.structure += P.t_struct; T.scatter += P.t_scatter; T.factor += P.t_factor; T.pack += P.t_pack; T.factorisations++;
+    T.gbPeak = std::max(T.gbPeak, P.gbPeak);
 }
 static void pc_finish_bilu(das_solver* s, das_ksp* k, double t0, int nBlocks, bool rasOverlap) {
     k->useBilu = true;
@@ -1386,35 +1390,23 @@
     k->pc.next = (long long)k->bilu.nNodes * BILU_NB;
 }
 
-static double pc_stability_estimate(das_solver* s, das_ksp* k, NodeILU& F, const std::vector<unsigned char>& mask) {
+static double pc_stability_estimate(das_solver* s, das_ksp* k, NodeILU& F, BiluSetupWork& W) {
+    const double t0 = wall_seconds();
     const long long n = s->n;
     const Mat& P = k->pcmat->m;
-    std::vector<double> e(n), z(n);
-    DevBuf<double> de(n), dw(n), dz(n);
+    if (W.e.n < (size_t)n) { W.e.alloc(n); W.w.alloc(n); W.z.alloc(n); }
     double est = 0.0;
     long long worst = -1;
     for (int trial = 0; trial < 2; trial++) {
-        for (long long i = 0; i < n; i++) {
-            const bool in = mask.empty() || mask[i];
-            unsigned long long hsh = (unsigned long long)i * 0x9E3779B97F4A7C15ull;
-            hsh ^= hsh >> 29;
-            e[i] = !in ? 0.0 : (trial == 0 ? 1.0 : ((hsh & 1ull) ? 1.0 : -1.0));
-        }
-        de.upload(e);
-        hipLaunchKernelGGL(k_spmv_wave, SPMV_GRID(P.n), dim3(256), 0, s->stream, P.n, P.rowptr.p, P.col.p, P.val.p, (const double*)de.p, dw.p);
-        dz.zero();
-        bilu_apply(F, dw.p, dz.p, s->stream);
-        DAS_HIP(hipStreamSynchronize(s->stream));
-        z = dz.to_host();
-        const int* nu = F.h_nodeUnk.data();
-        for (size_t q = 0; q < F.h_nodeUnk.size(); q++) {
-            const int gi = nu[q];
-            if (gi < 0) continue;
-            const double d = std::fabs(z[gi] - e[gi]);
-            if (d > est || d != d) worst = gi;
-            est = (d > est || d != d) ? (d != d ? 1e300 : d) : est;
-        }
-    }
+        hipLaunchKernelGGL(k_bilu_stab_trial, dim3((unsigned)std::min<long long>(4096, (n + 255) / 256)), dim3(256), 0, s->stream, n, (const unsigned char*)W.mask.p, trial, W.e.p);
+        hipLaunchKernelGGL(k_spmv_wave, SPMV_GRID(P.n), dim3(256), 0, s->stream, P.n, P.rowptr.p, P.col.p, P.val.p, (const double*)W.e.p, W.w.p);
+        DAS_HIP(hipMemsetAsync(W.z.p, 0, (size_t)n * sizeof(double), s->stream));
+        bilu_apply(F, W.w.p, W.z.p, s->stream);
+        long long slot = -1;
+        bilu_stab_reduce((long long)F.nNodes * BILU_NB, F.nodeUnk.p, W.z.p, W.e.p, W.part, s->stream, est, slot);
+        if (slot >= 0) worst = F.h_nodeUnk[(size_t)slot];
+    }
+    k->pcTimes.estimate += wall_seconds() - t0;
     if (worst >= 0 && getenv("DAS_PC_STAB")) {
         for (const StateDef& sd : s->st_full.states) {
             if (worst < sd.offset || worst >= sd.offset + sd.size) continue;
@@ -1426,6 +1418,8 @@
     }
     return est;
 }
+
+static bool pc_merge_rebuild() { const char* e = getenv("DAS_BILU_MERGE_REBUILD"); return e && atoi(e) != 0; }
 
 static void choose_order_and_factorise(das_solver* s, das_ksp* k, NodeILU& F, const std::vector<unsigned char>& mask, bool pickMin, int& orderUsed, double& estimate,
                                        bool earlyAccept = true) {
@@ -1449,12 +1443,29 @@
     const double good = s->opt.getd("amd.pcStabilityGood");
     struct Cand { int o; double est; int levels; };
     std::vector<Cand> seen;
-    int last = -1;
+    auto best_of_seen = [&](bool stoppedAtStable, double& bestEst) {
+        bool anyOk = false;
+        for (const Cand& c : seen) anyOk = anyOk || c.est <= limit;
+        int minLv = 1 << 30;
+        for (const Cand& c : seen) if (!anyOk || c.est <= limit) minLv = std::min(minLv, c.levels);
+        int best = seen.back().o;
+        bestEst = 1e300;
+        if (stoppedAtStable) bestEst = seen.back().est;
+        else
+            for (const Cand& c : seen)
+                if ((!anyOk || c.est <= limit) && (double)c.levels <= 1.5 * minLv && c.est < bestEst) { best = c.o; bestEst = c.est; }
+        return best;
+    };
+    const bool rebuild = pc_merge_rebuild();
+    BiluSetupWork W;
+    if (!mask.empty()) W.mask.upload(mask);
+    NodeILU kept;
+    int last = -1, keptOrder = -1;
     for (size_t attempt = 0; attempt < cand.size(); attempt++) {
         const int o = cand[attempt];
         F = NodeILU();
-        factorise_node_ilu(s, k, F, mask, o);
-        const double est = pc_stability_estimate(s, k, F, mask);
+        factorise_node_ilu(s, k, F, mask, o, &W);
+        const double est = pc_stability_estimate(s, k, F, W);
         last = o;
         seen.push_back({o, est, F.nLevels});
         if (s->opt.geti("debug") || getenv("DAS_PC_STAB") || (est > limit && !pickMin))
@@ -1462,20 +1473,22 @@
                     rank_label(), est, o, F.nLevels, limit, (est > limit && !pickMin) ? ": unstable, trying another order" : "");
         const bool deep = pc_order_is_deep(F.nLevels, F.nNodes);
         if (est <= limit && (!pickMin || (earlyAccept && est <= good && !deep))) break;
-    }
-    bool anyOk = false;
-    for (const Cand& c : seen) anyOk = anyOk || c.est <= limit;
-    int minLv = 1 << 30;
-    for (const Cand& c : seen) if (!anyOk || c.est <= limit) minLv = std::min(minLv, c.levels);
-    int best = seen.back().o;
-    double bestEst = 1e300;
-    if (!pickMin && seen.back().est <= limit) bestEst = seen.back().est;
-    else
-        for (const Cand& c : seen)
-            if ((!anyOk || c.est <= limit) && (double)c.levels <= 1.5 * minLv && c.est < bestEst) { best = c.o; bestEst = c.est; }
+        if (attempt + 1 < cand.size() && !rebuild) {
+            double e0;
+            const int b0 = best_of_seen(false, e0);
+            if (b0 == o) { kept = std::move(F); keptOrder = o; }
+            else if (b0 != keptOrder) { kept = NodeILU(); keptOrder = -1; }
+        }
+    }
+    double bestEst;
+    const int best = best_of_seen(!pickMin && seen.back().est <= limit, bestEst);
     if (last != best) {
-        F = NodeILU();
-        factorise_node_ilu(s, k, F, mask, best);
+        if (best == keptOrder) F = std::move(kept);
+        else {
+            F = NodeILU();
+            kept = NodeILU();
+            factorise_node_ilu(s, k, F, mask, best, &W);
+        }
     }
     if (bestEst > limit)
         fprintf(stderr, "[dafoam_amd] rank %s: no elimination order passes the stability limit; keeping order %d (estimate %.3e)\n", rank_label(), best, bestEst);
@@ -1514,6 +1527,9 @@
     const double t0 = wall_seconds();
     const Mesh& m = s->mesh;
     const long long N = m.nC, n = s->n;
+    k->pcTimes = das_ksp::PcSetupTimes();
+    const bool rebuild = pc_merge_rebuild() || k->pcTranspose || k->pcDiagScale != 1.0;
+    std::vector<NodeILU> kept(K);
     std::vector<int> cells(N), blockOf(N, 0);
     std::iota(cells.begin(), cells.end(), 0);
     rcb_parts(cells, [&](int c, int d) { return m.cg[c].C[d]; }, K, blockOf);
@@ -1533,7 +1549,7 @@
         }
         masks[b].assign(n, 0);
         for_each_unknown_with_cell(s, [&](long long g, int c) { masks[b][g] = cellIn[c]; });
-        NodeILU F;
+        NodeILU& F = kept[b];
         choose_order_and_factorise(s, k, F, masks[b], true, k->subOrder[b], k->subEst[b]);
         if (k->subOrder[b] < 0) k->subOrder[b] = pc_configured_order(s, k);
         if (s->opt.geti("debug") || getenv("DAS_PC_STAB"))
@@ -1544,14 +1560,21 @@
             k->subOrder.clear(); k->subEst.clear();
             return false;
         }
+        if (rebuild) F = NodeILU();
     }
     {
         const BiluInputs in(s, k);
         std::vector<const std::vector<unsigned char>*> mp;
         for (int b = 0; b < K; b++) mp.push_back(&masks[b]);
         k->bilu = NodeILU();
-        bilu_setup_multi(s->mesh, s->st_full.states, n, mp, k->subOrder, subOf, in.reach, in.fp32, in.A.n, in.A.rowptr.p, in.A.col.p, in.A.val.p, s->stream, k->bilu,
-                         in.debug, in.nthr, in.dir);
+        const double tm0 = wall_seconds();
+        if (rebuild)
+            bilu_setup_multi(s->mesh, s->st_full.states, n, mp, k->subOrder, subOf, in.reach, in.fp32, in.A.n, in.A.rowptr.p, in.A.col.p, in.A.val.p, s->stream, k->bilu,
+                             in.debug, in.nthr, in.dir);
+        else
+            bilu_merge_blocks(n, kept, subOf, in.fp32, s->stream, k->bilu, in.debug, in.nthr);
+        k->pcTimes.merge = wall_seconds() - tm0;
+        k->pcTimes.gbPeak = std::max(k->pcTimes.gbPeak, k->bilu.gbPeak);
     }
     k->nSub = K;
     k->pcOrderUsed = k->subOrder[0];
@@ -1560,6 +1583,13 @@
     pc_finish_bilu(s, k, t0, K, false);
     if (s->opt.geti("debug") || getenv("DAS_PC_STAB"))
         fprintf(stderr, "[dafoam_amd] %d sub-domains merged: %d nodes, %d levels (%.0f nodes per level)\n", K, k->bilu.nNodes, k->bilu.nLevels, (double)k->bilu.nNodes / std::max(1, k->bilu.nLevels));
+    if (s->opt.geti("debug") || getenv("DAS_PC_STAB")) {
+        const das_ksp::PcSetupTimes& T = k->pcTimes;
+        fprintf(stderr, "[dafoam_amd] sub-domain set-up %.3f s: %d block factorisations: structure %.3f s, scatter %.3f s, factorise %.3f s, pack %.3f s; estimates %.3f s; "
+                        "merge %.3f s (%s: structure %.3f s, scatter %.3f s, factorise %.3f s, %s %.3f s); device memory in use at the high-water point %.3f GB, after %.3f GB\n",
+                wall_seconds() - t0, T.factorisations, T.structure, T.scatter, T.factor, T.pack, T.estimate, T.merge, rebuild ? "rebuilt" : "kept factors copied", k->bilu.t_struct,
+                k->bilu.t_scatter, k->bilu.t_factor, rebuild ? "pack" : "copy", k->bilu.t_pack, T.gbPeak, bilu_device_gb_in_use());
+    }
     return true;
 }
 
@@ -6196,6 +6226,12 @@
     return DAS_OK;
     DAS_CATCH
 }
+int das_debug_bilu_stab_max(long long n, long long nslots, const int* nodeUnk, const double* z, const double* e, double* est, long long* slot) {
+    DAS_TRY
+    debug_bilu_stab_max(n, nslots, nodeUnk, z, e, est, slot);
+    return DAS_OK;
+    DAS_CATCH
+}
 
 #define DAS_GRAPH_DEVICE(who) DAS_CHECK(das_device_count() > 0, DAS_ERR_NO_DEVICE, std::string(who) + ": no HIP device visible")
 int das_debug_graph_scan(long long n, const int* cnt, long long* out, long long* total) {
diff --git a/include/dafoam_amd.h b/include/dafoam_amd.h
--- a/include/dafoam_amd.h
+++ b/include/dafoam_amd.h
@@ -321,6 +321,7 @@
                           int* nshift);
 int das_debug_bilu_apply(const das_bilu_debug_t* in, int nrhs, long long ld, const double* b, double* out, int twice, double* y, double* z,
                          int* abortFlag, int* info);
+int das_debug_bilu_stab_max(long long n, long long nslots, const int* nodeUnk, const double* z, const double* e, double* est, long long* slot);
 int das_debug_graph_scan(long long n, const int* cnt, long long* out, long long* total);
 int das_debug_graph_transpose(long long n, const long long* rowptr, const int* col, long long* trp, int* tcol);
 int das_debug_graph_nets(long long n, const long long* rowptr, const int* col, long long nKeep, const long long* keep, long long* cptr, int* crow, int* cpos,
```
